# zacharie12/Hypernet-image-captioning

Hardware: AMD Instinct MI355X
Metric: training images/sec at 1/2/4/8 MI355X, Flickr30k GRU+hypernet bs=128 (higher is better)
Workload: dtype f32; 1 GPU; Flickr30k-shaped GRU+additive-attention decoder + hypernet (3 style domains), full training step (fwd, CE, bwd, clip 5.0, Adam); per_gpu_batch=128, global_batch=128, T=20, P=49, D=2048, F=200, E=200, H=200, V=9684, hypernet_params=144906720, parallelism=dp1, launch=eager, next_theta_in_adam_pass=True, next_precompute_beside_adam=True, spinup_steps=0, deterministic_gradients=True

## Files before the change

hypernet-image-captioning_amd/caphn/_lib.py:

```python
import ctypes as C
import os

import torch

_HERE = os.path.dirname(os.path.abspath(__file__))
LIB_PATH = os.environ.get("CAPHN_LIB_PATH") or os.path.join(_HERE, "libcaphn.so")
MAX_HEADS = 8

c_fp = C.c_void_p


class HyperDesc(C.Structure):
    _fields_ = [("he", C.c_int), ("n_heads", C.c_int),
                ("k", C.c_int * MAX_HEADS), ("w", C.c_int * MAX_HEADS),
                ("base_w0", c_fp), ("base_b0", c_fp), ("base_w2", c_fp), ("base_b2", c_fp),
                ("w1", c_fp * MAX_HEADS), ("b1", c_fp * MAX_HEADS),
                ("w2", c_fp * MAX_HEADS), ("b2", c_fp * MAX_HEADS),
                ("d_in", C.c_int), ("d_mid", C.c_int)]


class HyperGrads(C.Structure):
    _fields_ = [("g_base_w0", c_fp), ("g_base_b0", c_fp), ("g_base_w2", c_fp), ("g_base_b2", c_fp),
                ("g_w1", c_fp * MAX_HEADS), ("g_b1", c_fp * MAX_HEADS),
                ("g_w2", c_fp * MAX_HEADS), ("g_b2", c_fp * MAX_HEADS),
# ... 31 lines not shown


class PairPack(C.Structure):
    _fields_ = [("wp", c_fp), ("H", C.c_int), ("HA", C.c_int), ("pitch", C.c_int), ("hrows", C.c_int)]


MAX_LAYERS = 4


class PlainDims(C.Structure):
    _fields_ = [(n, C.c_int) for n in ("B", "T", "E", "H", "V", "L", "cell")]


class AttnDims(C.Structure):
    _fields_ = [(n, C.c_int) for n in ("bs", "nh", "dh", "tq", "tk", "q_ldt", "q_ldb", "k_ldt", "k_ldb", "v_ldt", "v_ldb",
                                       "o_ldt", "o_ldb")] + [("scale", C.c_float), ("dropout_p", C.c_float),
                                                             ("seed", C.c_uint64)]


class PlainParams(C.Structure):
    _fields_ = [("embed_w", c_fp), ("out_w", c_fp), ("out_b", c_fp),
                ("w_ih", c_fp * MAX_LAYERS), ("w_hh", c_fp * MAX_LAYERS), ("b_ih", c_fp * MAX_LAYERS), ("b_hh", c_fp * MAX_LAYERS)]


class PlainGrads(C.Structure):
    _fields_ = [("embed_w", c_fp), ("out_w", c_fp), ("out_b", c_fp),
                ("w_ih", c_fp * MAX_LAYERS), ("w_hh", c_fp * MAX_LAYERS), ("b_ih", c_fp * MAX_LAYERS), ("b_hh", c_fp * MAX_LAYERS),
                ("features", c_fp)]


class SearchCfg(C.Structure):
    _fields_ = [("n_images", C.c_int), ("beam", C.c_int), ("max_steps", C.c_int), ("zero_pad_rule", C.c_int),
                ("lookup_first", C.c_int), ("first_token", C.c_int64), ("end_token", C.c_int64)]


SIGNATURES = {
    "caphn_abi_version": (C.c_int, []),
    "caphn_device_arch": (C.c_int, [C.c_char_p, C.c_int]),
    "caphn_device_error": (C.c_int, [C.c_int]),
    "caphn_gemm_f32": (C.c_int, [C.c_int, C.c_int, C.c_int, C.c_int, C.c_int, c_fp, C.c_int, c_fp, C.c_int,
                                 c_fp, C.c_int, c_fp, c_fp, C.c_int, C.c_int, C.c_int, c_fp]),
    "caphn_split3_bf16": (C.c_int, [c_fp, C.c_int, C.c_int, C.c_int, c_fp, C.c_int, C.c_size_t, C.c_int, c_fp]),
    "caphn_gemm_planes_f32": (C.c_int, [C.c_int, C.c_int, C.c_int, C.c_int, C.c_int, c_fp, C.c_int, c_fp, C.c_int, C.c_size_t,
                                        c_fp, C.c_int, c_fp, C.c_int, C.c_size_t, c_fp, C.c_int, c_fp, c_fp, C.c_int, C.c_int,
                                        C.c_int, C.c_int, c_fp]),
    "caphn_zero_f32": (C.c_int, [c_fp, C.c_size_t, c_fp]),
    "caphn_lrelu_bwd_f32": (C.c_int, [C.c_size_t, c_fp, c_fp, c_fp, c_fp]),
    "caphn_axpy_f32": (C.c_int, [C.c_size_t, C.c_float, c_fp, c_fp, c_fp]),
    "caphn_scale_f32": (C.c_int, [C.c_size_t, c_fp, c_fp, c_fp, c_fp]),
    "caphn_add_dropout_f32": (C.c_int, [C.c_size_t, c_fp, c_fp, C.c_float, C.c_uint64, C.c_uint64, c_fp, c_fp]),
    "caphn_dropout_f32": (C.c_int, [C.c_size_t, C.c_float, C.c_uint64, C.c_uint64, c_fp, c_fp, c_fp]),
    "caphn_colsum_workspace_bytes": (C.c_size_t, [C.c_int, C.c_int]),
    "caphn_linear_wgrad_f32": (C.c_int, [C.c_int, C.c_int, C.c_int, c_fp, C.c_int, c_fp, C.c_int, c_fp, C.c_int, c_fp, c_fp, c_fp]),
    "caphn_colsum_f32": (C.c_int, [C.c_int, C.c_int, c_fp, C.c_int, c_fp, c_fp, c_fp]),
    "caphn_hyper_acts_floats": (C.c_int, [C.POINTER(HyperDesc)]),
    "caphn_hyper_forward": (C.c_int, [C.POINTER(HyperDesc), c_fp, c_fp, c_fp, c_fp]),
    "caphn_hyper_backward_workspace_bytes": (C.c_size_t, [C.POINTER(HyperDesc)]),
    "caphn_hyper_backward": (C.c_int, [C.POINTER(HyperDesc), c_fp, c_fp, C.POINTER(HyperGrads), c_fp, c_fp]),
    "caphn_decoder_workspace_bytes": (C.c_size_t, [C.POINTER(DecoderDims)]),
    "caphn_decoder_forward": (C.c_int, [C.POINTER(DecoderDims), C.POINTER(DecoderParams), c_fp, c_fp,
                                        c_fp, c_fp, c_fp, c_fp]),
    "caphn_decoder_pair_prep": (C.c_int, [C.POINTER(DecoderDims), C.POINTER(DecoderParams), c_fp, c_fp]),
    "caphn_decoder_pair_pack_desc": (C.c_int, [C.POINTER(DecoderDims), c_fp, C.POINTER(PairPack)]),
    "caphn_decoder_precompute": (C.c_int, [C.POINTER(DecoderDims), C.POINTER(DecoderParams), c_fp, c_fp, c_fp, c_fp]),
    "caphn_decoder_inputs": (C.c_int, [C.POINTER(DecoderDims), C.POINTER(DecoderParams), c_fp, c_fp, c_fp]),
    "caphn_decoder_lookup": (C.c_int, [C.POINTER(DecoderDims), C.POINTER(DecoderParams), c_fp, c_fp, c_fp]),
    "caphn_decoder_prepare_rows": (C.c_int, [C.POINTER(DecoderDims), c_fp, C.c_int64, c_fp, c_fp]),
    "caphn_decoder_forward_sampled": (C.c_int, [C.POINTER(DecoderDims), C.POINTER(DecoderParams), c_fp, c_fp,
                                                C.c_char_p, c_fp, c_fp, c_fp, c_fp]),
    "caphn_decoder_forward_sampled_train": (C.c_int, [C.POINTER(DecoderDims), C.POINTER(DecoderParams), c_fp, c_fp,
                                                      C.c_char_p, c_fp, c_fp, c_fp, c_fp]),
    "caphn_decoder_backward": (C.c_int, [C.POINTER(DecoderDims), C.POINTER(DecoderParams), c_fp, c_fp,
                                         c_fp, c_fp, C.POINTER(DecoderGrads), c_fp, c_fp]),
    "caphn_decoder_hyper_backward": (C.c_int, [C.POINTER(DecoderDims), C.POINTER(DecoderParams), c_fp, c_fp,
                                               c_fp, c_fp, C.POINTER(DecoderGrads), c_fp,
                                               C.POINTER(HyperDesc), c_fp, C.POINTER(HyperGrads), c_fp, c_fp]),
    "caphn_decoder_backward_milestone": (C.c_int, [C.c_int, c_fp]),
    "caphn_decoder_search_workspace_bytes": (C.c_size_t, [C.POINTER(DecoderDims), C.POINTER(SearchCfg)]),
    "caphn_decoder_search_begin": (C.c_int, [C.POINTER(DecoderDims), C.POINTER(DecoderParams), C.POINTER(SearchCfg),
                                             c_fp, c_fp, c_fp, c_fp]),
    "caphn_decoder_search_steps": (C.c_int, [C.POINTER(DecoderDims), C.POINTER(DecoderParams), C.POINTER(SearchCfg),
                                             C.c_int, C.c_int, c_fp, c_fp, c_fp, c_fp]),
    "caphn_decoder_search_result": (C.c_int, [C.POINTER(DecoderDims), C.POINTER(SearchCfg), C.c_int, c_fp, c_fp,
                                              c_fp, c_fp, c_fp, c_fp, c_fp, c_fp]),
    "caphn_plain_workspace_bytes": (C.c_size_t, [C.POINTER(PlainDims)]),
    "caphn_plain_forward": (C.c_int, [C.POINTER(PlainDims), C.POINTER(PlainParams), c_fp, c_fp, c_fp, c_fp, c_fp, c_fp, c_fp]),
    "caphn_bahdanau_fwd": (C.c_int, [C.c_int] * 4 + [c_fp] * 8),
    "caphn_bahdanau_bwd": (C.c_int, [C.c_int] * 4 + [c_fp] * 12),
    "caphn_plain_forward_sampled": (C.c_int, [C.POINTER(PlainDims), C.POINTER(PlainParams), c_fp, c_fp, c_fp, C.c_uint64, c_fp, c_fp,
                                               c_fp, c_fp]),
    "caphn_plain_backward": (C.c_int, [C.POINTER(PlainDims), C.POINTER(PlainParams), c_fp, c_fp, c_fp, c_fp, c_fp,
                                       C.POINTER(PlainGrads), c_fp, c_fp]),
    "caphn_layernorm_fwd": (C.c_int, [C.c_int, C.c_int, c_fp, c_fp, c_fp, C.c_float, c_fp, c_fp, c_fp, c_fp]),
    "caphn_layernorm_bwd_workspace_bytes": (C.c_size_t, [C.c_int, C.c_int]),
    "caphn_layernorm_bwd": (C.c_int, [C.c_int, C.c_int, c_fp, c_fp, c_fp, c_fp, c_fp, c_fp, c_fp, c_fp, c_fp, c_fp]),
    "caphn_attention_supported": (C.c_int, [C.POINTER(AttnDims)]),
    "caphn_attention_fwd": (C.c_int, [C.POINTER(AttnDims), c_fp, c_fp, c_fp, c_fp, c_fp, c_fp, c_fp, c_fp]),
    "caphn_attention_bwd": (C.c_int, [C.POINTER(AttnDims), c_fp, c_fp, c_fp, c_fp, c_fp, c_fp, c_fp, c_fp, c_fp, c_fp, c_fp, c_fp]),
    "caphn_ce_workspace_bytes": (C.c_size_t, [C.c_int]),
    "caphn_cross_entropy_rows": (C.c_int, [C.c_int, C.c_int, c_fp, c_fp, C.c_int64, c_fp, C.c_int, c_fp, c_fp, c_fp]),
    "caphn_cross_entropy_rows_ld": (C.c_int, [C.c_int, C.c_int, C.c_int, c_fp, c_fp, C.c_int64, c_fp, C.c_int, c_fp, c_fp, c_fp]),
    "caphn_cross_entropy_finish": (C.c_int, [C.c_int, c_fp, c_fp, c_fp, c_fp]),
    "caphn_decoder_profile_ptr": (C.c_void_p, [C.POINTER(DecoderDims), c_fp]),
    "caphn_decoder_rowcount_ptr": (C.c_void_p, [C.POINTER(DecoderDims), c_fp]),
    "caphn_cross_entropy_fwd_bwd": (C.c_int, [C.c_int, C.c_int, c_fp, c_fp, C.c_int64, c_fp, c_fp, C.c_int, c_fp, c_fp]),
    "caphn_embedding_gather": (C.c_int, [C.c_int, C.c_int, c_fp, c_fp, c_fp, c_fp]),
# ... 85 lines not shown
```

hypernet-image-captioning_amd/caphn/ops.py:

```python
import ctypes as C
from dataclasses import dataclass
from typing import Dict, List, Optional, Sequence, Tuple

import torch

from . import _lib as L

GEMM_BIAS, GEMM_RELU, GEMM_ACCUM, GEMM_MASK, GEMM_LRELU = 1, 2, 4, 8, 16


def _f32(*shape, device):
    return torch.empty(*shape, dtype=torch.float32, device=device)


def gemm(a: torch.Tensor, b: torch.Tensor, ta: bool = False, tb: bool = False,
         bias: Optional[torch.Tensor] = None, relu: bool = False, out: Optional[torch.Tensor] = None,
         accumulate: bool = False, mask: Optional[torch.Tensor] = None, splitk: int = 1, lrelu: bool = False) -> torch.Tensor:
    lib = L.load()
    assert a.dim() == 2 and b.dim() == 2 and a.stride(1) == 1 and b.stride(1) == 1
    M, K = (a.shape[1], a.shape[0]) if ta else (a.shape[0], a.shape[1])
    N, Kb = (b.shape[0], b.shape[1]) if tb else (b.shape[1], b.shape[0])
    if K != Kb:
        raise L.CaphnError(f"gemm inner dims differ: {K} vs {Kb}")
    if out is None:
# ... 48 lines not shown
            "caphn_gemm_planes_f32")
    return out


def zero_(t: torch.Tensor) -> torch.Tensor:
    lib = L.load()
    L.check(lib.caphn_zero_f32(L.ptr(t), t.numel(), L.stream_ptr()), "caphn_zero_f32")
    return t


def add_dropout(x: torch.Tensor, branch: torch.Tensor, p: float = 0.0, seed: int = 0) -> torch.Tensor:
    lib = L.load()
    x, branch = x.contiguous(), branch.contiguous()
    assert x.shape == branch.shape
    out = torch.empty_like(x)
    L.check(lib.caphn_add_dropout_f32(x.numel(), L.ptr(x), L.ptr(branch), float(p), int(seed) & (2 ** 64 - 1), 0, L.ptr(out),
                                      L.stream_ptr()), "caphn_add_dropout_f32")
    return out


def scale_(x: torch.Tensor, scale_dev: torch.Tensor) -> torch.Tensor:
    lib = L.load()
    L.check(lib.caphn_scale_f32(x.numel(), L.ptr(x), L.ptr(scale_dev.reshape(-1)[:1].contiguous()), L.ptr(x), L.stream_ptr()),
            "caphn_scale_f32")
    return x


def lrelu_bwd(dy: torch.Tensor, post: torch.Tensor, out: Optional[torch.Tensor] = None) -> torch.Tensor:
    lib = L.load()
    assert dy.numel() == post.numel() and dy.is_contiguous() and post.is_contiguous()
    if out is None:
        out = torch.empty_like(dy)
    L.check(lib.caphn_lrelu_bwd_f32(dy.numel(), L.ptr(dy), L.ptr(post), L.ptr(out), L.stream_ptr()), "caphn_lrelu_bwd_f32")
    return out


def axpy_(y: torch.Tensor, x: torch.Tensor, alpha: float = 1.0) -> torch.Tensor:
    lib = L.load()
    assert x.numel() == y.numel() and x.is_contiguous() and y.is_contiguous()
    L.check(lib.caphn_axpy_f32(y.numel(), float(alpha), L.ptr(x), L.ptr(y), L.stream_ptr()), "caphn_axpy_f32")
    return y


def linear_wgrad(dy: torch.Tensor, x: torch.Tensor):
    lib = L.load()
    K, M = dy.shape
    N = x.shape[1]
    assert x.shape[0] == K and dy.stride(1) == 1 and x.stride(1) == 1
    dw, db = _f32(M, N, device=dy.device), _f32(M, device=dy.device)
    ws = torch.empty(lib.caphn_colsum_workspace_bytes(K, M), dtype=torch.uint8, device=dy.device)
    L.check(lib.caphn_linear_wgrad_f32(M, N, K, L.ptr(dy), dy.stride(0), L.ptr(x), x.stride(0), L.ptr(dw), N, L.ptr(db),
                                       C.c_void_p(ws.data_ptr()), L.stream_ptr()), "caphn_linear_wgrad_f32")
    return dw, db


def bahdanau_fwd(f: torch.Tensor, waf: torch.Tensor, uah: torch.Tensor, v_a: torch.Tensor, b_va: torch.Tensor):
    lib = L.load()
    B, P, Fd = f.shape
    H = uah.shape[1]
    ctx, alpha = _f32(B, Fd, device=f.device), _f32(B, P, device=f.device)
    L.check(lib.caphn_bahdanau_fwd(B, P, Fd, H, L.ptr(f), L.ptr(waf), L.ptr(uah), L.ptr(v_a), L.ptr(b_va), L.ptr(ctx), L.ptr(alpha),
                                   L.stream_ptr()), "caphn_bahdanau_fwd")
    return ctx, alpha


def bahdanau_bwd(f, waf, uah, v_a, alpha, dctx, dalpha, want_df: bool):
    lib = L.load()
    B, P, Fd = f.shape
    H = uah.shape[1]
    dwaf, duah, part = _f32(B, P, H, device=f.device), _f32(B, H, device=f.device), _f32(B, H + 1, device=f.device)
    df = _f32(B, P, Fd, device=f.device) if want_df else None
    L.check(lib.caphn_bahdanau_bwd(B, P, Fd, H, L.ptr(f), L.ptr(waf), L.ptr(uah), L.ptr(v_a), L.ptr(alpha), L.ptr(dctx),
                                   L.ptr(dalpha, allow_none=True), L.ptr(dwaf), L.ptr(duah), L.ptr(part),
                                   L.ptr(df, allow_none=True), L.stream_ptr()), "caphn_bahdanau_bwd")
    return dwaf, duah, part, df


def colsum(a: torch.Tensor, out: Optional[torch.Tensor] = None) -> torch.Tensor:
    lib = L.load()
    M, N = a.shape
    ws = torch.empty(lib.caphn_colsum_workspace_bytes(M, N), dtype=torch.uint8, device=a.device)
    if out is None:
        out = _f32(N, device=a.device)
    L.check(lib.caphn_colsum_f32(M, N, L.ptr(a), a.stride(0), L.ptr(out), C.c_void_p(ws.data_ptr()), L.stream_ptr()),
            "caphn_colsum_f32")
    return out


HYPER_NAMES = ("hn_base.0.weight", "hn_base.0.bias", "hn_base.2.weight", "hn_base.2.bias")


@dataclass
class HyperShape:
    he: int
    heads: List[Tuple[int, int]]
    d_in: int = 0
    d_mid: int = 0

    @property
    def din(self) -> int:
        return self.d_in or self.he

    @property
    def dmid(self) -> int:
        return self.d_mid or self.he

# ... 883 lines not shown
```

hypernet-image-captioning_amd/csrc/decoder.hip:

```cpp
#include "common.h"
#include "decoder_internal.h"
#include "gemm_internal.h"
#include <algorithm>
#include <initializer_list>
#include <mutex>

int g_tune_deterministic = 0;
int g_tune_rec_pair = 1;
int g_tune_rec_rotate = 1;
int g_tune_vocab_order = 1;
int g_tune_branch_mask = 7;
int g_tune_splitk_target = 1280;
int g_tune_chain_main = 0;
int g_tune_hops = 0;
int g_tune_fork = 4;
int g_tune_join_chain = 0;
int g_tune_sk_dhs = 0, g_tune_sk_vocab_w = 0;
#define RUN(x) do { int _rc = (x); if (_rc != CAPHN_OK) return _rc; } while (0)

namespace {

struct Side {
    hipStream_t st[3];
    enum { D_FORK = 0, D_JOIN = 1, D_X = 4, D_MS = 10, D_PRE_F = 14, D_PRE_ALL = 15, D_COUNT = 16 };
    struct Dep { hipEvent_t ev; unsigned seq = 0; bool by_value = false; };
    Dep deps[D_COUNT];
    unsigned* vals = nullptr;
    unsigned counter = 0;
    bool values = false;
    bool pre_valid = false;
    const void* pre_ws = nullptr;
    bool ready = false, on = false;
    bool forked[3] = {false, false, false};
    hipStream_t main = nullptr;
    int init() {
        if (ready) return CAPHN_OK;
        static std::mutex mu;
        std::lock_guard<std::mutex> lock(mu);
        if (ready) return CAPHN_OK;
        for (auto& s : st) if (hipStreamCreateWithFlags(&s, hipStreamNonBlocking) != hipSuccess) return CAPHN_ELAUNCH;
        for (auto& d : deps) if (hipEventCreateWithFlags(&d.ev, hipEventDisableTiming) != hipSuccess) return CAPHN_ELAUNCH;
        void* p = nullptr;
        if (hipMalloc(&p, sizeof(unsigned) * D_COUNT) == hipSuccess && hipMemset(p, 0, sizeof(unsigned) * D_COUNT) == hipSuccess)
            vals = static_cast<unsigned*>(p);
        else (void)hipGetLastError();
        ready = true;
        return CAPHN_OK;
    }
    int post(int slot, hipStream_t from) {
        Dep& d = deps[slot];
        if (values) {
            d.seq = ++counter; d.by_value = true;
            return hipStreamWriteValue32(from, vals + slot, d.seq, 0) == hipSuccess ? CAPHN_OK : CAPHN_ELAUNCH;
        }
        d.by_value = false;
        return hipEventRecord(d.ev, from) == hipSuccess ? CAPHN_OK : CAPHN_ELAUNCH;
    }
    int await(int slot, hipStream_t to) {
        Dep& d = deps[slot];
        if (d.by_value)
            return hipStreamWaitValue32(to, vals + slot, d.seq, hipStreamWaitValueGte, 0xffffffffu) == hipSuccess ? CAPHN_OK : CAPHN_ELAUNCH;
        return hipStreamWaitEvent(to, d.ev, 0) == hipSuccess ? CAPHN_OK : CAPHN_ELAUNCH;
    }
    int milestone(int k, hipStream_t from) {
        if (init() != CAPHN_OK) return CAPHN_ELAUNCH;
        return post(D_MS + k, from);
    }
    int begin(hipStream_t m, bool enable) {
        main = m; on = enable;
// ... 14 lines not shown
        if (!on) return CAPHN_OK;
        if (post(D_FORK, main) != CAPHN_OK) return CAPHN_ELAUNCH;
        for (int i : ids) {
            if (!((g_tune_branch_mask >> i) & 1)) continue;
            if (await(D_FORK, st[i]) != CAPHN_OK) return CAPHN_ELAUNCH;
            forked[i] = true;
        }
        return CAPHN_OK;
    }
    int jointo(int i) {
        if (!on || !((g_tune_branch_mask >> i) & 1)) return CAPHN_OK;
        forked[i] = false;
        if (post(D_JOIN + i, st[i]) != CAPHN_OK) return CAPHN_ELAUNCH;
        return await(D_JOIN + i, main);
    }
    int join_into(int i, int j) {
        if (!on || !((g_tune_branch_mask >> i) & 1)) return CAPHN_OK;
        if (!((g_tune_branch_mask >> j) & 1)) return jointo(i);
        forked[i] = false;
        if (post(D_JOIN + i, st[i]) != CAPHN_OK) return CAPHN_ELAUNCH;
        return await(D_JOIN + i, st[j]);
    }
    struct Scope {
        Side& s;
        explicit Scope(Side& side) : s(side) {}
        ~Scope() { for (int i = 0; i < 3; ++i) if (s.on && s.forked[i]) (void)s.jointo(i); }
    };
    hipStream_t xfrom[6] = {nullptr, nullptr, nullptr, nullptr, nullptr, nullptr};
    int record(int k, hipStream_t from) {
        if (!on) return CAPHN_OK;
        xfrom[k] = from;
        return post(D_X + k, from);
    }
    int wait(int k, hipStream_t to) {
        if (!on || xfrom[k] == to) return CAPHN_OK;
        return await(D_X + k, to);
    }
    int dep(hipStream_t from, hipStream_t to, int k) {
        if (!on || from == to) return CAPHN_OK;
        if (post(D_X + k, from) != CAPHN_OK) return CAPHN_ELAUNCH;
        return await(D_X + k, to);
    }
};
constexpr int MAX_DEVICES = 64;
Side g_sides[MAX_DEVICES];
inline Side* side_here() {
    int dev = 0;
    if (hipGetDevice(&dev) != hipSuccess || dev < 0 || dev >= MAX_DEVICES) return nullptr;
    return &g_sides[dev];
}

struct Ws {
    size_t Y1, f, meanf, h0, c0, Waf, G, Xe, Xg, Hs, Hprev, gates, hn, Cs, Cprev, uah, alphas, idx;
    size_t dHs, dgi, dgh, duah, de, dh0, dc0, ctx, dctx, dXe, dWaf, dmeanf, df, dY1, apart, vtmp, colws, colws_s[3], prof, rowmap;
    size_t xch, xch_floats;
    size_t wp;
    size_t H0s, dH0, h0L, dcarry, tgi, tgh, tmpA, tmpB;
    size_t Lin[CAPHN_MAX_DEC_LAYERS - 1], Lgates[CAPHN_MAX_DEC_LAYERS - 1], Lhn[CAPHN_MAX_DEC_LAYERS - 1],
           Ldgi[CAPHN_MAX_DEC_LAYERS - 1], Ldgh[CAPHN_MAX_DEC_LAYERS - 1];
    int L1;
    size_t total;
    int npc, pchunk, NG, arows;
};
inline bool use_pair(const caphn_decoder_dims* d) {
    const int NG = d->cell == CAPHN_CELL_LSTM ? 4 : 3;
    return g_tune_rec_pair && d->T > 1 && d->layers <= 1 && caphn_rec_pair_resident_gates(d->P, d->H, NG) >= 0;
}

inline size_t up4(size_t v) { return (v + 3) & ~(size_t)3; }

inline Ws layout(const caphn_decoder_dims* d) {
    Ws w;
    const size_t B = d->B, T = d->T, P = d->P, F = d->F, E = d->E, H = d->H, V = d->V, D = d->D;
    const bool lstm = d->cell == CAPHN_CELL_LSTM, raw = d->raw_features != 0;
    const size_t NG = lstm ? 4 : 3;
    w.NG = (int)NG;
    size_t o = 0;
    auto take = [&](size_t n) { size_t r = o; o += up4(n); return r; };
    w.Y1 = take(raw ? 0 : B * P * F); w.f = take(raw ? 0 : B * P * F); w.meanf = take(B * F); w.h0 = take(B * H);
    w.c0 = take(lstm ? B * H : 0);
    w.Waf = take(B * P * H); w.G = take(B * P * NG * H); w.Xe = take(B * T * (E + F)); w.Xg = take(B * T * NG * H);
    w.Hs = take(B * T * H); w.Hprev = take(B * T * H); w.gates = take(B * T * NG * H); w.hn = take(lstm ? 0 : B * T * H);
    w.Cs = take(lstm ? B * T * H : 0); w.Cprev = take(lstm ? B * T * H : 0);
    w.uah = take(B * T * H); w.alphas = take(B * T * P); w.idx = take(2 * B * T);
    w.dHs = take(B * T * H); w.dgi = take(B * T * NG * H); w.dgh = take(lstm ? 0 : B * T * NG * H); w.duah = take(B * T * H);
    w.de = take(B * T * P); w.dh0 = take(B * H); w.dc0 = take(lstm ? B * H : 0);
    w.ctx = w.Xe + E; w.dctx = take(raw ? 0 : B * T * F);
    w.dXe = take(B * T * E); w.dWaf = take(B * P * H); w.dmeanf = take(raw ? 0 : 2 * B * F); w.df = take(raw ? 0 : B * P * F);
    w.dY1 = take(raw ? 0 : B * P * F);
    w.pchunk = 1; w.npc = (int)((P + w.pchunk - 1) / w.pchunk);
    const size_t arows = std::max<size_t>(std::max<size_t>(w.npc, (size_t)caphn_rec_bwd_groups((int)P, (int)H)),
                                          (size_t)caphn_rec_pair_bwd_groups((int)P, (int)H));
    w.arows = (int)arows;
    w.apart = take(B * arows * (H + 1)); w.vtmp = take(H + 1);
    size_t cs = 0;
    auto need = [&](size_t M, size_t N) { cs = std::max(cs, caphn_colsum_workspace_bytes((int)M, (int)N) / sizeof(float)); };
    need(B * T, V); need(B * T, NG * H); need(B * T, H); need(B * P, H); need(B * P, F); need(B, H);
    need(B * arows, H + 1);
    if (d->layers > 1) need(B * (T + 1), 3 * H);
    w.colws = take(cs);
    {
        size_t c2 = 0;
        auto need2 = [&](size_t M, size_t N) { c2 = std::max(c2, caphn_colsum_workspace_bytes((int)M, (int)N) / sizeof(float)); };
        need2(B * T, NG * H); need2(B * T, H); need2(B * P, H); need2(B * P, F); need2(B, H); need2(B * arows, H + 1);
        if (d->layers > 1) need2(B * (T + 1), 3 * H);
        for (int i = 0; i < 3; ++i) w.colws_s[i] = take(c2);
    }
    w.prof = take(64);
    w.rowmap = take(B * T + 4);
    w.xch_floats = caphn_rec_pair_xch_bytes((int)B, (int)P, (int)H) / sizeof(float);
    w.xch = take(2 * w.xch_floats);
    o = (o + 31) & ~(size_t)31;
    w.wp = take(caphn_rec_pair_wp_floats((int)H, (int)NG));
    w.L1 = d->layers > 1 ? d->layers - 1 : 0;
    {
        const size_t on = w.L1 > 0 ? 1 : 0, S = T + 1;
        w.H0s = take(on * B * T * H); w.dH0 = take(on * B * T * H); w.h0L = take(on * B * H); w.dcarry = take(on * B * H);
        w.tgi = take(on * B * 3 * H); w.tgh = take(on * B * 3 * H); w.tmpA = take(on * B * H); w.tmpB = take(on * B * H);
        for (int l = 0; l < CAPHN_MAX_DEC_LAYERS - 1; ++l) {
            const size_t u = l < w.L1 ? 1 : 0;
            w.Lin[l] = take(u * B * S * H); w.Lgates[l] = take(u * B * S * 3 * H); w.Lhn[l] = take(u * B * S * H);
            w.Ldgi[l] = take(u * B * S * 3 * H); w.Ldgh[l] = take(u * B * S * 3 * H);
        }
    }
    w.total = o;
    (void)D;
    return w;
}

__global__ __launch_bounds__(1024) void valid_rows_kernel(int n, const int64_t* __restrict__ tgt, int64_t ignore, int* __restrict__ map) {
    __shared__ int wsum[16];
    __shared__ int base_s;
    const int tid = threadIdx.x, lane = tid & 63, wave = tid >> 6;
    if (tid == 0) base_s = 0;
    __syncthreads();
    for (int c0 = 0; c0 < n; c0 += 1024) {
        const int i = c0 + tid;
        const int v = (i < n && tgt[i] != ignore) ? 1 : 0;
        const unsigned long long ball = __ballot(v);
        const int before = __popcll(ball & ((1ull << lane) - 1ull));
        if (lane == 0) wsum[wave] = __popcll(ball);
// ... 419 lines not shown
    if (!late && !wg_first) {
        if (!(d->precomputed & 32) && sd.s(0) != s && sd.s(2) != s) {
            RUN(sd.fork_many({0, 2}));
            RUN(caphn_launch_ctx(B, T, P, F, ws + w.alphas, f, ws + w.ctx, EF, sd.s(2)));
            RUN(sd.record(5, sd.s(2)));
            ctx_side = true;
        } else
        RUN(sd.forkto(0));
        RUN(wgrad_bias(V, H, BT, dlogits, LV, ws + w.Hs, H, g->out_w, H, g->out_b, rmap, cws, sd.s(0), gz));
        RUN(sd.milestone(CAPHN_MS_VOCAB, sd.s(0)));
    }

    RecBwdArgs a;
    a.B = B; a.T = T; a.P = P; a.H = H; a.RG = RG;
    a.Waf = ws + w.Waf; a.G = ws + w.G; a.W_hh = p->w_hh; a.U_a = p->Ua_w; a.v_a = p->va_w;
    a.Hprev = ws + w.Hprev; a.alphas = ws + w.alphas; a.gates = ws + w.gates; a.hn = ws + w.hn; a.uah = ws + w.uah;
    a.Cs = ws + w.Cs; a.Cprev = ws + w.Cprev;
    a.dHs = ws + w.dHs; a.dalphas = dalphas;
    a.dgi = dgi; a.dgh = dgh; a.duah = ws + w.duah; a.de = ws + w.de; a.dh0 = ws + w.dh0; a.dc0 = ws + w.dc0;
    a.vecW = (H % 4 == 0) && caphn_aligned16(p->w_hh) && caphn_aligned16(p->Ua_w);
    a.vecS = (H % 4 == 0) && caphn_aligned16(ws);
    a.prof = reinterpret_cast<unsigned long long*>(ws + w.prof) + 8;
    a.rotate = g_tune_rec_rotate;
    a.drop_p = d->dropout_p; a.drop_seed = d->dropout_seed;
    const int ang = w.L1 > 0 ? 0 : pair ? caphn_rec_pair_bwd_groups(P, H) : caphn_rec_bwd_groups(P, H);
    if (ang > 0) { a.dWaf = ws + w.dWaf; a.apart = ws + w.apart; }
    if (w.L1 > 0) {
        RUN(caphn_zero_f32(ws + w.dcarry, (size_t)B * H, s));
        a.dHs = ws + w.dH0; a.dh0 = ws + w.dcarry; a.drop_p = 0.f;
        for (int t = T - 1; t >= 0; --t) {
            RUN(layers_backward(d, p, w, ws, t + 1, ws + w.dHs + (size_t)t * H, T * H, ws + w.dcarry, ws + w.dH0 + (size_t)t * H, T * H, s));
            a.t0 = t; a.t1 = t + 1;
            RUN(caphn_launch_rec_bwd(a, lstm, s));
        }
        RUN(layers_backward(d, p, w, ws, 0, ws + w.dcarry, H, nullptr, ws + w.dh0, H, s));
    } else if (pair) {
        a.xch = reinterpret_cast<unsigned long long*>(ws + w.xch) + w.xch_floats * sizeof(float) / sizeof(unsigned long long);
        a.apart_rows = ang;
        a.WP = ws + w.wp; a.wp_pitch = caphn_rec_pair_pitch(H);
        if (!raw) { a.inith_w = p->inith_w; a.initc_w = lstm ? p->initc_w : nullptr; a.dmean_part = ws + w.dmeanf; a.F = F; }
        RUN(caphn_launch_rec_pair_bwd(a, lstm, s));
    } else
    RUN(caphn_launch_rec_bwd(a, lstm, s));

    hipStream_t b0 = sd.s(0), b1 = sd.s(1), b2 = sd.s(2);
    const bool t_main = hook != nullptr && g_tune_chain_main != 0;
    hipStream_t sT = t_main ? s : b1, sF = t_main ? b1 : s;
    const bool hold_big = late && !raw && fork_mode == 3;
    RUN(sd.fork_many({0, 1, 2}));
    if (late && !hold_big) {
        RUN(wgrad_bias(V, H, BT, dlogits, LV, ws + w.Hs, H, g->out_w, H, g->out_b, rmap, cws, b0, gz));
        RUN(sd.milestone(CAPHN_MS_VOCAB, b0));
    }
    if (ctx_side) RUN(sd.wait(5, sT));
    else if (!(d->precomputed & 32)) RUN(caphn_launch_ctx(B, T, P, F, ws + w.alphas, f, ws + w.ctx, EF, sT));
    if (lstm) RUN(gemm_auto(1, 0, GH, EF, BT, dgi, GH, ws + w.Xe, EF, g->w_ih, EF, nullptr, 0, sT, nullptr, 0, gz));
    else RUN(wgrad_bias(GH, EF, BT, dgi, GH, ws + w.Xe, EF, g->w_ih, EF, g->b_ih, nullptr, cw1, sT, gz));
    RUN(wgrad_bias(GH, H, BT, dgh, GH, ws + w.Hprev, H, g->w_hh, H, g->b_hh, nullptr, cw2, b2, gz));
    if (lstm) RUN(caphn_colsum_f32(BT, GH, dgi, GH, g->b_ih, cw2, b2));
    RUN(sd.record(3, b2));
    hipStream_t se = late ? b2 : b0;
    RUN(caphn_gemm_f32(0, 0, BT, E, GH, dgi, GH, p->w_ih, EF, ws + w.dXe, E, nullptr, nullptr, 0, 0, 1, se));
    if (!gz) RUN(caphn_zero_f32(g->embed_w, (size_t)V * E, se));
    RUN(caphn_embedding_scatter_add_v(BT, E, V, ws + w.dXe, idx, g->embed_w, se));
    RUN(sd.milestone(CAPHN_MS_EMBED, se));
    RUN(sd.wait(3, sT));
    RUN(sd.milestone(CAPHN_MS_DTHETA, sT));
    if (hook && !hold_big) {
        RUN(caphn_hyper_backward(hook->hd, g->w_ih, hook->acts, hook->hg, hook->ws, sT));
    }
    if (!hold_big) RUN(sd.milestone(CAPHN_MS_HYPER, sT));
    if (!raw) {
        RUN(caphn_gemm_f32(0, 0, BT, F, GH, dgi, GH, p->w_ih + E, EF, ws + w.dctx, F, nullptr, nullptr, 0, 0, 1, sF));
        if (!pair)
            RUN(caphn_launch_dmean(B, H, F, ws + w.dh0, p->inith_w, lstm ? ws + w.dc0 : nullptr, lstm ? p->initc_w : nullptr,
                                   ws + w.dmeanf, sF));
    }
    AttnGradArgs ag;
    ag.T = T; ag.P = P; ag.H = H; ag.pchunk = w.pchunk;
    ag.Waf = ws + w.Waf; ag.uah = ws + w.uah; ag.de = ws + w.de; ag.v_a = p->va_w;
    ag.dWaf = ws + w.dWaf; ag.part = ws + w.apart;
    if (ang == 0) RUN(caphn_launch_attn_param_grads(ag, B, w.npc, sF));
    RUN(sd.record(2, sF));
    RUN(wgrad_bias(H, H, BT, ws + w.duah, H, ws + w.Hprev, H, g->Ua_w, H, g->Ua_b, nullptr, cws, b0, gz));
    for (int l = 0; l < w.L1; ++l) {
        const int BS = B * (T + 1), G3 = 3 * H;
        RUN(wgrad_bias(G3, H, BS, ws + w.Ldgi[l], G3, ws + w.Lin[l], H, g->lw_ih[l], H, g->lb_ih[l], nullptr, cws, b0, gz));
        RUN(wgrad_bias(G3, H, BS, ws + w.Ldgh[l], G3, ws + w.Lin[l], H, g->lw_hh[l], H, g->lb_hh[l], nullptr, cws, b0, gz));
    }
    RUN(wgrad_bias(H, F, B, ws + w.dh0, H, ws + w.meanf, F, g->inith_w, F, g->inith_b, nullptr, cws, b0, gz));
    if (lstm) RUN(wgrad_bias(H, F, B, ws + w.dc0, H, ws + w.meanf, F, g->initc_w, F, g->initc_b, nullptr, cws, b0, gz));
    if (!raw) {
        RUN(caphn_launch_df(B, T, P, F, ws + w.alphas, ws + w.dctx, ws + w.dmeanf, ws + w.df, sF, pair ? ws + w.dmeanf + (size_t)B * F : nullptr));
        RUN(caphn_gemm_f32(0, 0, BP, F, H, ws + w.dWaf, H, p->Wa_w, F, ws + w.df, F, nullptr, nullptr, 0, CAPHN_GEMM_ACCUM, 1, sF));
        RUN(sd.record(4, sF));
        if (hold_big) {
            RUN(sd.wait(4, b0));
            RUN(wgrad_bias(V, H, BT, dlogits, LV, ws + w.Hs, H, g->out_w, H, g->out_b, rmap, cws, b0, gz));
            RUN(sd.milestone(CAPHN_MS_VOCAB, b0));
            if (hook) {
                RUN(sd.wait(4, sT));
                RUN(caphn_hyper_backward(hook->hd, g->w_ih, hook->acts, hook->hg, hook->ws, sT));
            }
            RUN(sd.milestone(CAPHN_MS_HYPER, sT));
        }
        RUN(caphn_gemm_f32(0, 0, BP, F, F, ws + w.df, F, p->fc2_w, F, ws + w.dY1, F, nullptr, ws + w.Y1, F, CAPHN_GEMM_MASK, 1, sF));
        RUN(wgrad_bias(F, D, BP, ws + w.dY1, F, features, D, g->fc0_w, D, g->fc0_b, nullptr, cw0, sF, gz));
    }
    RUN(sd.wait(2, b2));
    RUN(caphn_colsum_f32(B * (ang > 0 ? ang : w.npc), H + 1, ws + w.apart, H + 1, ws + w.vtmp, cw2, b2));
    hipLaunchKernelGGL(copy2_kernel, dim3((H + 256) / 256), dim3(256), 0, b2, ws + w.vtmp, H, g->va_w, g->va_b);
    RUN(wgrad_bias(H, F, BP, ws + w.dWaf, H, f, F, g->Wa_w, F, g->Wa_b, nullptr, cw2, b2, gz));
    if (!raw) {
        RUN(sd.wait(4, b2));
        RUN(wgrad_bias(F, F, BP, ws + w.df, F, ws + w.Y1, F, g->fc2_w, F, g->fc2_b, nullptr, cw2, b2, gz));
    }
    if (g_tune_join_chain) { RUN(sd.join_into(0, 1)); RUN(sd.join_into(2, 1)); RUN(sd.jointo(1)); }
    else { RUN(sd.jointo(0)); RUN(sd.jointo(1)); RUN(sd.jointo(2)); }
    (void)captions;
    return caphn_launch_status();
}

extern "C" int caphn_decoder_backward_milestone(int which, caphn_stream_t waiter) {
    if (which < 0 || which >= CAPHN_MS_COUNT) return CAPHN_EINVAL;
    Side* sd = side_here();
    if (!sd) return CAPHN_ELAUNCH;
    if (!sd->ready) return CAPHN_OK;
    return sd->await(Side::D_MS + which, static_cast<hipStream_t>(waiter));
}

extern "C" int caphn_decoder_forward_sampled(const caphn_decoder_dims* d, const caphn_decoder_params* p,
                                             const float* features, const int64_t* captions,
                                             const unsigned char* use_sampling,
                                             float* logits, float* alphas, void* ws_, caphn_stream_t stream) {
    if (!dims_ok(d) || !p || !features || !captions || !use_sampling || !logits || !ws_ || d->logits_ld != 0) return CAPHN_EINVAL;
    if (d->dropout_p > 0.f) return CAPHN_EINVAL;
    hipStream_t s = static_cast<hipStream_t>(stream);
    const Ws w = layout(d);
    float* ws = static_cast<float*>(ws_);
    const int B = d->B, T = d->T, P = d->P, E = d->E, F = d->F, H = d->H, V = d->V;
    const bool lstm = d->cell == CAPHN_CELL_LSTM;
    const int GH = w.NG * H, EF = E + F;
    const int RG = caphn_rec_resident_gates(P, H, w.NG);
    if (RG < 0) return CAPHN_ELIMIT;
    if (lstm && (!p->initc_w || !p->initc_b)) return CAPHN_EINVAL;
    const float* f = nullptr;
    if (!layer_params_ok(d, p)) return CAPHN_EINVAL;
    RUN(decoder_precompute(d, p, w, ws, features, &f, s));
    if (w.L1 > 0) RUN(layers_forward(d, p, w, ws, 0, ws + w.h0, H, ws + w.h0L, H, s));
    int64_t* idx = reinterpret_cast<int64_t*>(ws + w.idx);
    int src_mode = 0, src_col = 0;
    for (int t = 0; t < T; ++t) {
        const bool samp = t > 0 && use_sampling[t] != 0;
        if (!samp) {
            if (t < 2) { src_mode = 0; } else { src_mode = 1; src_col = t - 1; }
// ... 146 lines not shown
    const SearchArgs a = search_args(d, c, w, ws, static_cast<char*>(sws_));
    return caphn_launch_search_init(a, ws + (w.L1 > 0 ? w.h0L : w.h0), c->first_token, c->lookup_first, s);
}

extern "C" int caphn_decoder_search_steps(const caphn_decoder_dims* d, const caphn_decoder_params* p, const caphn_search_cfg* c,
                                          int step0, int nsteps, float* alphas, void* ws_, void* sws_, caphn_stream_t stream) {
    if (!search_ok(d, c) || !p || !ws_ || !sws_ || step0 < 1 || nsteps < 0 || step0 + nsteps - 1 > c->max_steps) return CAPHN_EINVAL;
    if (!layer_params_ok(d, p)) return CAPHN_EINVAL;
    if (alphas && c->beam != 1) return CAPHN_EINVAL;
    hipStream_t s = static_cast<hipStream_t>(stream);
    const Ws w = layout(d);
    float* ws = static_cast<float*>(ws_);
    char* sw = static_cast<char*>(sws_);
    const SearchWs q = search_layout(d, c);
    const SearchArgs sa = search_args(d, c, w, ws, sw);
    const int R = d->B, P = d->P, E = d->E, F = d->F, H = d->H, V = d->V, GH = w.NG * H, EF = E + F;
    const int RG = caphn_rec_resident_gates(P, H, w.NG);
    if (RG < 0) return CAPHN_ELIMIT;
    float* logits = reinterpret_cast<float*>(sw + q.logits);
    for (int step = step0; step < step0 + nsteps; ++step) {
        RUN(caphn_embedding_gather(R, E, p->embed_w, sa.idx, ws + w.Xe, s));
        RUN(caphn_gemm_f32(0, 1, R, GH, E, ws + w.Xe, E, p->w_ih, EF, ws + w.Xg, GH, p->b_ih, nullptr, 0, CAPHN_GEMM_BIAS, 1, s));
        RecFwdArgs a;
        a.B = R; a.T = 1; a.P = P; a.H = H; a.RG = RG; a.slab_div = c->beam;
        a.Waf = ws + w.Waf; a.G = ws + w.G; a.Xg = ws + w.Xg; a.h0 = sa.h_cur; a.c0 = nullptr;
        a.W_hh = p->w_hh; a.b_hh = p->b_hh; a.U_a = p->Ua_w; a.b_Ua = p->Ua_b; a.v_a = p->va_w; a.b_va = p->va_b;
        a.Hs = ws + w.Hs; a.Hprev = ws + w.Hprev; a.alphas = ws + w.alphas; a.gates = ws + w.gates; a.hn = ws + w.hn;
        a.Cs = nullptr; a.Cprev = nullptr; a.uah = ws + w.uah; a.prof = nullptr; a.rotate = 0;
        a.vecW = (H % 4 == 0) && caphn_aligned16(p->w_hh) && caphn_aligned16(p->Ua_w);
        a.vecS = (H % 4 == 0) && caphn_aligned16(ws);
        if (w.L1 > 0) a.Hs = ws + w.H0s;
        RUN(caphn_launch_rec_fwd(a, false, s));
        if (w.L1 > 0) RUN(layers_forward(d, p, w, ws, 1, ws + w.H0s, H, ws + w.Hs, H, s));
        RUN(caphn_gemm_f32(0, 1, R, V, H, ws + w.Hs, H, p->out_w, H, logits, V, p->out_b, nullptr, 0, CAPHN_GEMM_BIAS, 1, s));
        if (alphas)
            if (hipMemcpy2DAsync(alphas + (size_t)(step - 1) * P, sizeof(float) * (size_t)c->max_steps * P, ws + w.alphas,
                                 sizeof(float) * P, sizeof(float) * P, R, hipMemcpyDeviceToDevice, s) != hipSuccess) return CAPHN_ELAUNCH;
        RUN(caphn_launch_row_topk(R, V, c->beam, logits, sa.score, const_cast<float*>(sa.cand_val), const_cast<int*>(sa.cand_idx), s));
        RUN(caphn_launch_beam_merge(sa, step, s));
    }
    return caphn_launch_status();
}

extern "C" int caphn_decoder_search_result(const caphn_decoder_dims* d, const caphn_search_cfg* c, int steps_done, void* ws_, void* sws_,
                                           int64_t* seqs, int* lengths, float* scores, int* finished, int* n_active,
                                           caphn_stream_t stream) {
    if (!search_ok(d, c) || !ws_ || !sws_ || !seqs || !lengths || !scores || !finished || !n_active || steps_done < 0 ||
        steps_done > c->max_steps) return CAPHN_EINVAL;
    const Ws w = layout(d);
    const SearchArgs sa = search_args(d, c, w, static_cast<float*>(ws_), static_cast<char*>(sws_));
    return caphn_launch_search_result(sa, steps_done, seqs, lengths, scores, finished, n_active, static_cast<hipStream_t>(stream));
}

extern "C" int caphn_linear_wgrad_f32(int M, int N, int K, const float* dY, int ldy, const float* X, int ldx, float* dW, int ldw,
                                      float* db, void* ws, caphn_stream_t stream) {
    if (M <= 0 || N <= 0 || K <= 0 || !dY || !X || !dW || !db || !ws) return CAPHN_EINVAL;
    return caphn_gemm_tn_colsum(M, N, K, dY, ldy, X, ldx, dW, ldw, db, pick_splitk(M, N, K), nullptr, ws, false,
                                static_cast<hipStream_t>(stream));
}
```

hypernet-image-captioning_amd/csrc/decoder_internal.h:

```cpp
#pragma once
#include "common.h"

struct RecFwdArgs {
    int B, T, P, H;
    int RG;
    const float* Waf;
    const float* G;
    const float* Xg;
    const float* h0;
    const float* c0;
    const float* W_hh; const float* b_hh;
    const float* U_a; const float* b_Ua;
    const float* v_a; const float* b_va;
    float* Hs; float* Hprev;
    float* alphas;
    float* gates;
    float* hn;
    float* Cs; float* Cprev;
    float* uah;
    unsigned long long* prof;
    int vecW, vecS, rotate;
    int slab_div = 1;
    unsigned long long* xch = nullptr;
    const float* WP = nullptr; int wp_pitch = 0;
// ... 25 lines not shown
    const float* WP = nullptr; int wp_pitch = 0;
    int apart_rows = 0;
    float drop_p = 0.f; unsigned long long drop_seed = 0;
    unsigned epoch = 0; int* err = nullptr; long long xlimit = 0;
    const float* inith_w = nullptr; const float* initc_w = nullptr; float* dmean_part = nullptr; int F = 0;
    int part_rows = 0, wc_rows = 0;
    int t0 = 0, t1 = 0;
};
struct AttnGradArgs {
    int T, P, H, pchunk;
    const float* Waf; const float* uah; const float* de; const float* v_a;
    float* dWaf;
    float* part;
};

struct LayerFwdArgs {
    int B, H, S, slot;
    const float* gi; const float* gh;
    const float* hin; int hin_ld;
    float* hout; int hout_ld;
    float* sin; float* sgates; float* shn;
    float drop_p = 0.f; unsigned long long drop_seed = 0; int T = 1, t = 0;
};
struct LayerBwdArgs {
    int B, H, S, slot;
    const float* d1; int d1_ld; const float* d2;
    const float* sin; const float* sgates; const float* shn;
    float* dgi; float* dgh;
    float* dout; int dout_ld;
    float drop_p = 0.f; unsigned long long drop_seed = 0; int T = 1, t = 0;
};
int caphn_launch_layer_gru_fwd(const LayerFwdArgs& a, hipStream_t s);
int caphn_launch_layer_gru_bwd(const LayerBwdArgs& a, hipStream_t s);

size_t caphn_rec_fwd_lds_bytes(int P, int H, int NG, int RG);
size_t caphn_rec_bwd_lds_bytes(int P, int H, int NG, int RG);
int caphn_rec_resident_gates(int P, int H, int NG);
int caphn_launch_rec_fwd(const RecFwdArgs& a, bool lstm, hipStream_t s);
int caphn_launch_rec_bwd(const RecBwdArgs& a, bool lstm, hipStream_t s);
bool caphn_rec_pair_ok(int P, int H, int NG, int RG);
int caphn_rec_pair_resident_gates(int P, int H, int NG);
size_t caphn_rec_pair_xch_bytes(int B, int P, int H);
int caphn_rec_pair_bwd_groups(int P, int H);
int caphn_rec_pair_pitch(int H);
int caphn_rec_pair_half_a(int H);
size_t caphn_rec_pair_wp_floats(int H, int NG);
int caphn_launch_rec_pair_prep(unsigned long long* xch, size_t nxch, const float* U_a, const float* W_hh, int H, int NG, float* WP,
                               float* zbuf, size_t nz, hipStream_t s);
int caphn_launch_rec_pair_fwd(const RecFwdArgs& a, bool lstm, hipStream_t s);
int caphn_launch_rec_pair_bwd(const RecBwdArgs& a, bool lstm, hipStream_t s);
int caphn_rec_bwd_groups(int P, int H);
int caphn_launch_attn_param_grads(const AttnGradArgs& a, int B, int npc, hipStream_t s);
int caphn_launch_ctx(int B, int T, int P, int F, const float* alphas, const float* f, float* ctx, int ldc, hipStream_t s);
int caphn_launch_df(int B, int T, int P, int F, const float* alphas, const float* dctx, const float* dmean, float* df, hipStream_t s,
                    const float* dmean2 = nullptr);
int caphn_launch_dmean(int B, int H, int F, const float* dh0, const float* Wh, const float* dc0, const float* Wc, float* out, hipStream_t s);
int caphn_launch_init_state(int B, int P, int F, int H, const float* f, const float* Wh, const float* bh, const float* Wc,
                            const float* bc, float* meanf, float* h0, float* c0, hipStream_t s);
int caphn_embedding_gather_strided(int rows, int E, const float* table, const int64_t* idx, int istride, float* out, int ostride, hipStream_t s);
int caphn_launch_mean_p(int B, int P, int F, const float* f, float* out, hipStream_t s);

constexpr int SEARCH_MAX_BEAM = 8;
struct SearchArgs {
    int n_images, beam, max_steps, H;
    int zero_pad_rule;
    int64_t end_token;
    float* h_cur; const float* h_new;
    float* score;
    int64_t* idx;
    const float* cand_val; const int* cand_idx;
    int* k_alive; int* n_comp;
    int64_t* seqs[2];
    int64_t* comp_seqs; int* comp_len; float* comp_score;
};
int caphn_launch_row_topk(int R, int V, int k, const float* logits, const float* score, float* cand_val, int* cand_idx, hipStream_t s);
int caphn_launch_beam_merge(const SearchArgs& a, int step, hipStream_t s);
int caphn_launch_search_init(const SearchArgs& a, const float* h0, int64_t first_token, int lookup_first, hipStream_t s);
int caphn_launch_search_result(const SearchArgs& a, int steps_done, int64_t* out_seq, int* out_len, float* out_score, int* finished,
                               int* n_active, hipStream_t s);
```

hypernet-image-captioning_amd/csrc/gemm_bf16x3.hip:

```cpp
#include "common.h"
#include "gemm_internal.h"
#include "split3.h"
#include <type_traits>

#ifdef CAPHN_GEMM_PROFILE
__device__ unsigned long long d_gemm_prof[10];
__device__ unsigned long long d_gemm_wgt[2 * 8192];
extern "C" int caphn_debug_gemm_wgtimes(unsigned long long* out, int n) {
    return hipMemcpyFromSymbol(out, HIP_SYMBOL(d_gemm_wgt), sizeof(unsigned long long) * 2 * (n < 8192 ? n : 8192)) == hipSuccess ? 0 : -1;
}
#define GSTAMP(i) do { if (gprof) { unsigned long long _n = clock64(); gpc[i] += _n - glast; glast = _n; } } while (0)
extern "C" int caphn_debug_gemm_prof(unsigned long long* out, int reset) {
    if (out && hipMemcpyFromSymbol(out, HIP_SYMBOL(d_gemm_prof), sizeof(unsigned long long) * 10) != hipSuccess) return -1;
    if (reset) { unsigned long long z[10] = {0, 0, 0, 0, 0, 0, 0, 0, 0, 0}; if (hipMemcpyToSymbol(HIP_SYMBOL(d_gemm_prof), z, sizeof(z)) != hipSuccess) return -1; }
    return 0;
}
#else
#define GSTAMP(i) do { } while (0)
#endif

extern int g_tune_gemm_waves;
namespace {

constexpr int BK = 32;
constexpr int PITCH = 32;
__device__ __forceinline__ int kc_off(int row, int k) { return row * PITCH + ((((k >> 3) ^ (row >> 2)) & 3) << 3) + (k & 7); }

template <int BMN, bool KC>
struct TileS {
    static constexpr int NV = BMN / 32;
    static constexpr int PITCHM = BMN + 32;
    static constexpr int PLANE = KC ? BMN * PITCH : BK * PITCHM;
    static constexpr int ELEMS = 3 * PLANE;

    __device__ static __forceinline__ void phys_rows(int (&pr)[NV], int rows, int r0, int tid, const int* __restrict__ rmap,
                                                     bool clamp) {
#pragma unroll
        for (int i = 0; i < NV; ++i) {
            int row = r0 + ((tid + 256 * i) >> 3);
            if (clamp) row = min(row, rows - 1);
            pr[i] = (rmap && row < rows) ? rmap[row] : row;
        }
    }
    __device__ static __forceinline__ void load(f32x4 (&r)[NV], const float* __restrict__ G, int ld,
                                                int rows, int K, int r0, int k0, int vec, int tid,
                                                const int (&pr)[NV], const int* __restrict__ kmap) {
#pragma unroll
        for (int i = 0; i < NV; ++i) {
            f32x4 v = {0.f, 0.f, 0.f, 0.f};
            const int idx = tid + 256 * i;
            if (KC) {
                const int row = r0 + (idx >> 3);
                const int k = k0 + (idx & 7) * 4;
                if (row < rows) {
                    const float* p = G + (size_t)pr[i] * ld + k;
// ... 159 lines not shown
    __device__ static __forceinline__ bf16x8 frag(const __bf16* __restrict__ S, int plane, int row0, int ks, int lane) {
        if (KC) {
            return *reinterpret_cast<const bf16x8*>(S + plane * PLANE + kc_off(row0 + (lane & 31), ks * 16 + (lane >> 5) * 8));
        } else {
            const int g = lane >> 4, i = lane & 15;
            const int col = row0 + 16 * (g & 1) + 4 * (i & 3);
            const int kb = 16 * ks + 8 * (g >> 1) + (i >> 2);
            typedef __attribute__((address_space(3))) bf16x4 lds_bf16x4;
            const __bf16* p = S + plane * PLANE + kb * PITCHM + col;
            const bf16x4 lo4 = __builtin_amdgcn_ds_read_tr16_b64_v4bf16((lds_bf16x4*)(p));
            const bf16x4 hi4 = __builtin_amdgcn_ds_read_tr16_b64_v4bf16((lds_bf16x4*)(p + 4 * PITCHM));
            return __builtin_shufflevector(lo4, hi4, 0, 1, 2, 3, 4, 5, 6, 7);
        }
    }
};

__device__ __forceinline__ float bf16_bits_to_f32(unsigned short b) { return __uint_as_float((unsigned)b << 16); }

template <int BM, int BN, bool TA, bool TB, int MODE>
__device__ __forceinline__ void gemm_bf16x3_body(GemmArgs g) {
    constexpr bool PL = MODE == 1;
    constexpr bool SINGLE = MODE == 2;
    constexpr bool WS = MODE == 5;
    constexpr bool DB = MODE == 3 || WS;
    constexpr bool TWO = MODE == 4;
    using TileA = TileS<BM, !TA>;
    using TileB = TileS<BN, TB>;
    constexpr int WM = BM / 2, WN = BN / 2, TM = WM / 32, TN = WN / 32;
    constexpr int TILE_ELEMS = TileA::ELEMS + TileB::ELEMS;
    extern __shared__ __attribute__((aligned(16))) __bf16 lds[];
    __bf16* As = lds;
    __bf16* Bs = lds + TileA::ELEMS;
    __bf16* As1 = DB ? lds + TILE_ELEMS : As;
    __bf16* Bs1 = DB ? lds + TILE_ELEMS + TileA::ELEMS : Bs;

    const bool producer = WS && threadIdx.x >= 256;
    const int tid = WS ? (threadIdx.x & 255) : threadIdx.x, lane = tid & 63, wave = tid >> 6;
    const int wm = wave >> 1, wn = wave & 1;
    const int li = lane & 31, kh = lane >> 5;
#ifdef CAPHN_GEMM_PROFILE
    const unsigned long long gstart = clock64();
    const unsigned gwg = blockIdx.x + gridDim.x * (blockIdx.y + gridDim.y * blockIdx.z);
    if (tid == 0 && gwg < 8192) d_gemm_wgt[2 * gwg] = wall_clock64();
#endif
    int bx = blockIdx.x, by = blockIdx.y, bz = blockIdx.z;
    if (g.flags & (1 << 20)) {
        const int nx = gridDim.x, ny = gridDim.y, nwg = nx * ny * (int)gridDim.z;
        const int orig = bx + nx * (by + ny * bz);
        const int xcd = orig & 7, q = nwg >> 3, r = nwg & 7;
        const int wgid = (xcd < r ? xcd * (q + 1) : r * (q + 1) + (xcd - r) * q) + (orig >> 3);
        if (g.flags & (1 << 22)) { by = wgid % ny; bx = (wgid / ny) % nx; }
        else { bx = wgid % nx; by = (wgid / nx) % ny; }
        bz = wgid / (nx * ny);
    }
    const int m0 = by * BM, n0 = bx * BN;
    const int* rmapA = nullptr; const int* kmap = nullptr;
    if (g.map_mode == 1) { g.M = min(g.M, g.dev_count[0]); rmapA = g.row_map; if (m0 >= g.M) return; }
    if (g.map_mode == 2) { g.K = min(g.K, g.dev_count[0]); kmap = g.row_map; }

    const int nslab_total = (g.K + BK - 1) / BK;
    int slab0 = 0, slab1 = nslab_total;
    if (g.splitk > 1) {
        const int sps = g.map_mode == 2 ? (nslab_total + g.splitk - 1) / g.splitk : g.slabs_per_split;
        slab0 = bz * sps;
        slab1 = min(nslab_total, slab0 + sps);
        if (slab0 >= slab1) return;
    }

    constexpr bool DUAL = TM * TN == 1;
    f32x16 acc[TM][TN], acc2[DUAL ? TM : 1][DUAL ? TN : 1];
#pragma unroll
    for (int a = 0; a < TM; ++a)
#pragma unroll
        for (int b = 0; b < TN; ++b)
#pragma unroll
            for (int r = 0; r < 16; ++r) { acc[a][b][r] = 0.f; if (DUAL) acc2[a][b][r] = 0.f; }

    f32x4 ra0[TileA::NV], rb0[TileB::NV], ra1[TileA::NV], rb1[TileB::NV];
    int pra[TileA::NV], prb[TileB::NV];
    const int* kl = nullptr;
    const int kbase = slab0 * BK;
    bool fast = !(g.flags & (1 << 21)) && g.vecA && g.vecB && g.M >= 4 && g.N >= 4 && g.K >= 4 && (g.K & 3) == 0 &&
                (!TA || (g.M & 3) == 0) && (TB || (g.N & 3) == 0);
    if (kmap) {
        const int need = (slab1 - slab0) * BK;
        if (fast && TA && !TB && g.kmap_lds >= need) {
            int* kls = reinterpret_cast<int*>(lds + (DB ? 2 : 1) * TILE_ELEMS);
            for (int i = tid; i < need; i += 256) kls[i] = kmap[min(kbase + i, g.K - 1)];
            __syncthreads();
            kl = kls;
        } else fast = false;
    }
    TileA::phys_rows(pra, g.M, m0, tid, rmapA, fast);
    TileB::phys_rows(prb, g.N, n0, tid, nullptr, fast);
    unsigned boa[TileA::NV], bob[TileB::NV];
    if (fast) { TileA::fast_bases(boa, g.lda, g.M, m0, tid, pra); TileB::fast_bases(bob, g.ldb, g.N, n0, tid, prb); }
    else {
#pragma unroll
        for (int i = 0; i < TileA::NV; ++i) boa[i] = 0;
#pragma unroll
        for (int i = 0; i < TileB::NV; ++i) bob[i] = 0;
    }
    auto gload = [&](f32x4 (&ra)[TileA::NV], f32x4 (&rb)[TileB::NV], int slab, auto fast_c) {
        if constexpr (decltype(fast_c)::value) {
            TileA::load_fast_b(ra, g.A, boa, g.lda, g.K, slab * BK, tid, kl, kbase);
            TileB::load_fast_b(rb, g.B, bob, g.ldb, g.K, slab * BK, tid, kl, kbase);
// ... 330 lines not shown
        for (int b = 0; b < TN; ++b) {
            const int col = n0 + wn * WN + b * 32 + li;
            if (col >= g.N) continue;
            const float bv = add_bias ? g.bias[col] : 0.f;
#pragma unroll
            for (int r = 0; r < 16; ++r) {
                const int row = m0 + wm * WM + a * 32 + (r & 3) + 8 * (r >> 2) + 4 * kh;
                if (row >= g.M) continue;
                float v = acc[a][b][r] + bv;
                float* c = g.C + (size_t)(rmapA ? rmapA[row] : row) * g.ldc + col;
                if (atomic) { atomicAdd(c, v); continue; }
                if (g.flags & CAPHN_GEMM_ACCUM) v += *c;
                if (g.flags & CAPHN_GEMM_RELU) v = fmaxf(v, 0.f);
                if (g.flags & CAPHN_GEMM_LRELU) v = v > 0.f ? v : 0.01f * v;
                if (g.flags & CAPHN_GEMM_MASK) v = (g.mask[(size_t)row * g.ldmask + col] > 0.f) ? v : 0.f;
                *c = v;
            }
        }
#ifdef CAPHN_GEMM_PROFILE
    if (tid == 0) {
        __builtin_amdgcn_s_waitcnt(0);
        if (gwg < 8192) d_gemm_wgt[2 * gwg + 1] = wall_clock64();
        if (gwg == 0) atomicAdd(&d_gemm_prof[8], clock64() - gstart);
    }
#endif
}

template <int BM, int BN, bool TA, bool TB, int MODE>
__global__ __launch_bounds__(256) void gemm_bf16x3_kernel(GemmArgs g) { gemm_bf16x3_body<BM, BN, TA, TB, MODE>(g); }
template <int BM, int BN, bool TA, bool TB, int MODE>
__global__ __launch_bounds__(256) __attribute__((amdgpu_waves_per_eu(5, 5))) void gemm_bf16x3_kernel_w5(GemmArgs g) { gemm_bf16x3_body<BM, BN, TA, TB, MODE>(g); }
template <int BM, int BN, bool TA, bool TB, int MODE>
__global__ __launch_bounds__(256) __attribute__((amdgpu_waves_per_eu(6, 6))) void gemm_bf16x3_kernel_w6(GemmArgs g) { gemm_bf16x3_body<BM, BN, TA, TB, MODE>(g); }

template <int BM, int BN, bool TA, bool TB>
__global__ __launch_bounds__(512) void gemm_bf16x3_kernel_ws(GemmArgs g) { gemm_bf16x3_body<BM, BN, TA, TB, 5>(g); }

template <int BM, int BN, bool TA, bool TB, int PL>
int launch_one(const GemmArgs& g, hipStream_t s) {
    using TileA = TileS<BM, !TA>;
    using TileB = TileS<BN, TB>;
    constexpr size_t lds_tiles = sizeof(__bf16) * (TileA::ELEMS + TileB::ELEMS) * ((PL == 3 || PL == 5) ? 2 : 1);
    size_t lds = lds_tiles;
    if (g.kmap_lds > 0) lds += sizeof(int) * (size_t)g.kmap_lds;
    static bool attr_set[64];
    int dev = 0;
    if (hipGetDevice(&dev) != hipSuccess || dev < 0 || dev >= 64) return CAPHN_ELAUNCH;
    if (lds_tiles + 16384 > 48 * 1024 && !attr_set[dev]) {
        const void* fn = PL == 5 ? reinterpret_cast<const void*>(gemm_bf16x3_kernel_ws<BM, BN, TA, TB>)
                                 : reinterpret_cast<const void*>(gemm_bf16x3_kernel<BM, BN, TA, TB, PL == 5 ? 0 : PL>);
        if (hipFuncSetAttribute(fn, hipFuncAttributeMaxDynamicSharedMemorySize, (int)(lds_tiles + 16384)) != hipSuccess) return CAPHN_ELAUNCH;
        attr_set[dev] = true;
    }
    dim3 grid((g.N + BN - 1) / BN, (g.M + BM - 1) / BM, g.splitk > 1 ? g.splitk : 1);
    if constexpr (PL == 5) {
        hipLaunchKernelGGL((gemm_bf16x3_kernel_ws<BM, BN, TA, TB>), grid, dim3(512), lds, s, g);
        return caphn_launch_status();
    } else {
    if constexpr (BM == 64 && PL == 0) {
        if (g_tune_gemm_waves == 5) { hipLaunchKernelGGL((gemm_bf16x3_kernel_w5<BM, BN, TA, TB, PL>), grid, dim3(256), lds, s, g); return caphn_launch_status(); }
        if (g_tune_gemm_waves == 6) { hipLaunchKernelGGL((gemm_bf16x3_kernel_w6<BM, BN, TA, TB, PL>), grid, dim3(256), lds, s, g); return caphn_launch_status(); }
    }
    hipLaunchKernelGGL((gemm_bf16x3_kernel<BM, BN, TA, TB, PL>), grid, dim3(256), lds, s, g);
    return caphn_launch_status();
    }
}
template <int BM, int BN, int PL>
int launch_cfg(const GemmArgs& g, int ta, int tb, hipStream_t s) {
    if (!ta && tb) return launch_one<BM, BN, false, true, PL>(g, s);
    if (!ta && !tb) return launch_one<BM, BN, false, false, PL>(g, s);
    if (ta && !tb) return launch_one<BM, BN, true, false, PL>(g, s);
    if constexpr (PL != 0) return CAPHN_EINVAL;
    else return launch_one<BM, BN, true, true, 0>(g, s);
}

}

extern int g_tune_gemm_planes;
int g_tune_gemm_tile = 0;
int g_tune_gemm_single = 0;
int g_tune_gemm_order = 1;
int g_tune_gemm_xcd = 1;
int g_tune_gemm_waves = 0;
int g_tune_gemm_ws = 0;
int g_tune_gemm_db = 0;
int g_tune_gemm_fast = 1;
bool caphn_gemm_planes_ok(const GemmArgs& g, int ta, int tb) {
    bool pl = g_tune_gemm_planes && g.Ap && g.Bp && !(ta && tb) && (g.K % 8) == 0 && g.K >= 8 && (g.ldap % 8) == 0 && (g.ldbp % 8) == 0 &&
              (g.psa % 8) == 0 && (g.psb % 8) == 0 && caphn_aligned16(g.Ap) && caphn_aligned16(g.Bp);
    if (pl && ta && (((g.M + 7) & ~7) > g.ldap || g.M < 8)) pl = false;
    if (pl && !tb && (((g.N + 7) & ~7) > g.ldbp || g.N < 8)) pl = false;
    if (pl && g.map_mode == 2) {
        const int nslab = (g.K + 31) / 32, sk = g.splitk > 1 ? g.splitk : 1;
        if (!(ta && !tb) || ((nslab + sk - 1) / sk) * 32 > 4096) pl = false;
    }
    return pl;
}
template <int BM, int BN, bool TA, bool TB>
static int occ_one() {
    using TileA = TileS<BM, !TA>;
    using TileB = TileS<BN, TB>;
    int n = 0;
    if (hipOccupancyMaxActiveBlocksPerMultiprocessor(&n, reinterpret_cast<const void*>(gemm_bf16x3_kernel<BM, BN, TA, TB, 0>), 256,
                                                     sizeof(__bf16) * (TileA::ELEMS + TileB::ELEMS)) != hipSuccess) return -1;
    return n;
}
extern "C" int caphn_debug_gemm_occupancy(int ta, int tb, int tile) {
    if (tile == 128) return !ta && tb ? occ_one<128, 128, false, true>() : !ta ? occ_one<128, 128, false, false>() : !tb ? occ_one<128, 128, true, false>() : occ_one<128, 128, true, true>();
    return !ta && tb ? occ_one<64, 64, false, true>() : !ta ? occ_one<64, 64, false, false>() : !tb ? occ_one<64, 64, true, false>() : occ_one<64, 64, true, true>();
}
int caphn_gemm_bf16x3_launch(GemmArgs g, int ta, int tb, hipStream_t s) {
    if (g_tune_gemm_xcd) g.flags |= 1 << 20;
    g.kmap_lds = 0;
    if (g.map_mode == 2 && ta && !tb) {
        const int nslab = (g.K + 31) / 32, sk = g.splitk > 1 ? g.splitk : 1;
        const int ints = ((nslab + sk - 1) / sk) * 32;
        if (ints <= 4096) g.kmap_lds = ints;
    }
    if (!g_tune_gemm_fast) g.flags |= 1 << 21;
    {
        const double ea = ta ? (double)g.K * g.lda : (double)g.M * g.lda, eb = tb ? (double)g.N * g.ldb : (double)g.K * g.ldb;
        if (ea * 4.0 >= 4.0e9 || eb * 4.0 >= 4.0e9) g.flags |= 1 << 21;
    }
    if (g_tune_gemm_order != 0 && g.splitk <= 1) {
        const double abytes = 4.0 * (double)g.M * g.K, bbytes = 4.0 * (double)g.N * g.K, l2 = 3.0 * 1024 * 1024;
        if (g_tune_gemm_order == 2 || (bbytes > l2 && abytes < bbytes)) g.flags |= 1 << 22;
    }
    long tiles128 = (long)((g.M + 127) / 128) * ((g.N + 127) / 128) * g.splitk;
    if (g.K < 512) tiles128 = 0;
    if (g_tune_gemm_tile == 64) tiles128 = 0; else if (g_tune_gemm_tile == 128) tiles128 = 1 << 20;
    const bool pl = caphn_gemm_planes_ok(g, ta, tb);
    if (!pl && g_tune_gemm_single == 0 && g_tune_gemm_tile == 0 && g_tune_gemm_ws == 0) {
        const int rc = caphn_gemm_kres_launch(g, ta, tb, s);
        if (rc != 1) return rc;
    }
    if (pl) {
        if (tiles128 >= 512) return launch_cfg<128, 128, 1>(g, ta, tb, s);
        return launch_cfg<64, 64, 1>(g, ta, tb, s);
    }
    if (g_tune_gemm_single == 1 && !(ta && tb)) {
        if (tiles128 >= 512) return launch_cfg<128, 128, 2>(g, ta, tb, s);
        return launch_cfg<64, 64, 2>(g, ta, tb, s);
    }
    if (g_tune_gemm_single == 2 && !(ta && tb)) {
        if (tiles128 >= 512) return launch_cfg<128, 128, 4>(g, ta, tb, s);
        return launch_cfg<64, 64, 4>(g, ta, tb, s);
    }
    if (g_tune_gemm_ws == 128 && !(ta && tb)) return launch_cfg<128, 128, 5>(g, ta, tb, s);
    if (g_tune_gemm_ws == 64 && !(ta && tb)) return launch_cfg<64, 64, 5>(g, ta, tb, s);
    if (tiles128 >= 512) return launch_cfg<128, 128, 0>(g, ta, tb, s);
    const int lay = (!ta && tb) ? 1 : (!ta && !tb) ? 2 : (ta && !tb) ? 4 : 0;
    if (g_tune_gemm_db & lay) return launch_cfg<64, 64, 3>(g, ta, tb, s);
    return launch_cfg<64, 64, 0>(g, ta, tb, s);
}

namespace {
struct SplitJobs { SplitJob j[8]; int n; long block0[9]; };
__global__ __launch_bounds__(256) void split3_kernel(SplitJobs jobs) {
    int ji = 0;
    for (int i = 1; i < jobs.n; ++i) if ((long)blockIdx.x >= jobs.block0[i]) ji = i;
    const SplitJob& J = jobs.j[ji];
    const int cpr = (J.cols + 7) >> 3;
    const long nchunk = (long)(J.rows + J.zero_rows) * cpr;
    const long stride = (jobs.block0[ji + 1] - jobs.block0[ji]) * 256;
    __bf16* dst = static_cast<__bf16*>(J.dst);
    const bool vec = (J.ld & 3) == 0 && caphn_aligned16_dev(J.src);
    for (long c = ((long)blockIdx.x - jobs.block0[ji]) * 256 + threadIdx.x; c < nchunk; c += stride) {
        const int row = (int)(c / cpr), col = (int)(c % cpr) * 8;
        const float* sp = J.src + (size_t)row * J.ld + col;
        f32x4 v0 = {0.f, 0.f, 0.f, 0.f}, v1 = {0.f, 0.f, 0.f, 0.f};
        if (row >= J.rows) { }
        else if (vec && col + 8 <= J.cols) { v0 = *reinterpret_cast<const f32x4*>(sp); v1 = *reinterpret_cast<const f32x4*>(sp + 4); }
        else {
#pragma unroll
            for (int e = 0; e < 4; ++e) { if (col + e < J.cols) v0[e] = sp[e]; if (col + 4 + e < J.cols) v1[e] = sp[4 + e]; }
        }
        const Split4 a = split3(v0), b = split3(v1);
        __bf16* dp = dst + (size_t)row * J.ldp + col;
        *reinterpret_cast<bf16x8*>(dp) = __builtin_shufflevector(a.hi, b.hi, 0, 1, 2, 3, 4, 5, 6, 7);
        *reinterpret_cast<bf16x8*>(dp + J.ps) = __builtin_shufflevector(a.mid, b.mid, 0, 1, 2, 3, 4, 5, 6, 7);
        *reinterpret_cast<bf16x8*>(dp + 2 * J.ps) = __builtin_shufflevector(a.lo, b.lo, 0, 1, 2, 3, 4, 5, 6, 7);
    }
}
// ... 22 lines not shown
```

hypernet-image-captioning_amd/csrc/gemm_f32.hip:

```cpp
#include "common.h"
#include "gemm_internal.h"

int g_tune_gemm = 1;

namespace {

template <int BMN, bool KC, int BK>
struct Tile {
    static constexpr int KPAD = BK + 4;
    static constexpr int K4 = BK / 4;
    static constexpr int TOTAL = BMN * K4;
    static constexpr int NV = (TOTAL + 255) / 256;
    static constexpr int LDM = BMN + 4;
    static constexpr int FLOATS = KC ? BMN * KPAD : BK * LDM;

    __device__ static __forceinline__ void load(f32x4 (&r)[NV], const float* __restrict__ G, int ld,
                                                int rows, int K, int r0, int k0, int vec, int tid) {
#pragma unroll
        for (int i = 0; i < NV; ++i) {
            f32x4 v = {0.f, 0.f, 0.f, 0.f};
            const int idx = tid + 256 * i;
            if (TOTAL % 256 != 0 && idx >= TOTAL) { r[i] = v; continue; }
            if (KC) {
                int row = r0 + idx / K4;
                int k = k0 + (idx % K4) * 4;
                if (row < rows) {
                    const float* p = G + (size_t)row * ld + k;
                    if (vec && k + 3 < K) v = *reinterpret_cast<const f32x4*>(p);
                    else {
#pragma unroll
                        for (int e = 0; e < 4; ++e) if (k + e < K) v[e] = p[e];
                    }
                }
            } else {
                int m = r0 + (idx % (BMN / 4)) * 4;
                int k = k0 + idx / (BMN / 4);
                if (k < K) {
                    const float* p = G + (size_t)k * ld + m;
                    if (vec && m + 3 < rows) v = *reinterpret_cast<const f32x4*>(p);
                    else {
#pragma unroll
                        for (int e = 0; e < 4; ++e) if (m + e < rows) v[e] = p[e];
                    }
                }
            }
            r[i] = v;
        }
    }
    __device__ static __forceinline__ void store(const f32x4 (&r)[NV], float* __restrict__ S, int tid) {
#pragma unroll
        for (int i = 0; i < NV; ++i) {
            const int idx = tid + 256 * i;
            if (TOTAL % 256 != 0 && idx >= TOTAL) continue;
            if (KC) *reinterpret_cast<f32x4*>(S + (idx / K4) * KPAD + (idx % K4) * 4) = r[i];
            else *reinterpret_cast<f32x4*>(S + (idx / (BMN / 4)) * LDM + (idx % (BMN / 4)) * 4) = r[i];
        }
    }
    __device__ static __forceinline__ f32x4 frag(const float* __restrict__ S, int row, int kq, int kh) {
        if (KC) return *reinterpret_cast<const f32x4*>(S + row * KPAD + kq * 8 + kh * 4);
        f32x4 v;
#pragma unroll
        for (int s = 0; s < 4; ++s) v[s] = S[(kq * 8 + kh * 4 + s) * LDM + row];
        return v;
    }
};

template <int BM, int BN, bool TA, bool TB, int BK>
__global__ __launch_bounds__(256) void gemm_f32_kernel(GemmArgs g) {
    using TileA = Tile<BM, !TA, BK>;
    using TileB = Tile<BN, TB, BK>;
    constexpr int WM = BM / 2, WN = BN / 2, TM = WM / 32, TN = WN / 32;
    __shared__ __attribute__((aligned(16))) float lds[TileA::FLOATS + TileB::FLOATS];
    float* As = lds;
    float* Bs = lds + TileA::FLOATS;

    const int tid = threadIdx.x, lane = tid & 63, wave = tid >> 6;
    const int wm = wave >> 1, wn = wave & 1;
    const int li = lane & 31, kh = lane >> 5;
    const int m0 = blockIdx.y * BM, n0 = blockIdx.x * BN;

    const int nslab_total = (g.K + BK - 1) / BK;
    int slab0 = 0, slab1 = nslab_total;
    if (g.splitk > 1) {
        slab0 = blockIdx.z * g.slabs_per_split;
        slab1 = min(nslab_total, slab0 + g.slabs_per_split);
        if (slab0 >= slab1) return;
    }

    f32x16 acc[TM][TN];
#pragma unroll
    for (int a = 0; a < TM; ++a)
#pragma unroll
        for (int b = 0; b < TN; ++b)
#pragma unroll
            for (int r = 0; r < 16; ++r) acc[a][b][r] = 0.f;

    f32x4 ra[TileA::NV], rb[TileB::NV];
    TileA::load(ra, g.A, g.lda, g.M, g.K, m0, slab0 * BK, g.vecA, tid);
    TileB::load(rb, g.B, g.ldb, g.N, g.K, n0, slab0 * BK, g.vecB, tid);
    TileA::store(ra, As, tid);
    TileB::store(rb, Bs, tid);
    __syncthreads();

    for (int slab = slab0; slab < slab1; ++slab) {
        const bool more = slab + 1 < slab1;
        if (more) {
            TileA::load(ra, g.A, g.lda, g.M, g.K, m0, (slab + 1) * BK, g.vecA, tid);
            TileB::load(rb, g.B, g.ldb, g.N, g.K, n0, (slab + 1) * BK, g.vecB, tid);
        }
#pragma unroll
        for (int kq = 0; kq < BK / 8; ++kq) {
            f32x4 fa[TM], fb[TN];
#pragma unroll
            for (int a = 0; a < TM; ++a) fa[a] = TileA::frag(As, wm * WM + a * 32 + li, kq, kh);
#pragma unroll
            for (int b = 0; b < TN; ++b) fb[b] = TileB::frag(Bs, wn * WN + b * 32 + li, kq, kh);
#pragma unroll
            for (int s = 0; s < 4; ++s)
#pragma unroll
                for (int a = 0; a < TM; ++a)
#pragma unroll
                    for (int b = 0; b < TN; ++b)
                        acc[a][b] = __builtin_amdgcn_mfma_f32_32x32x2f32(fa[a][s], fb[b][s], acc[a][b], 0, 0, 0);
        }
        __syncthreads();
        if (more) {
            TileA::store(ra, As, tid);
            TileB::store(rb, Bs, tid);
            __syncthreads();
        }
    }

    const bool atomic = g.splitk > 1;
    const bool add_bias = (g.flags & CAPHN_GEMM_BIAS) && (!atomic || blockIdx.z == 0);
#pragma unroll
    for (int a = 0; a < TM; ++a)
#pragma unroll
        for (int b = 0; b < TN; ++b) {
            const int col = n0 + wn * WN + b * 32 + li;
            if (col >= g.N) continue;
            const float bv = add_bias ? g.bias[col] : 0.f;
#pragma unroll
            for (int r = 0; r < 16; ++r) {
                const int row = m0 + wm * WM + a * 32 + (r & 3) + 8 * (r >> 2) + 4 * kh;
                if (row >= g.M) continue;
                float v = acc[a][b][r] + bv;
                float* c = g.C + (size_t)row * g.ldc + col;
                if (atomic) { atomicAdd(c, v); continue; }
                if (g.flags & CAPHN_GEMM_ACCUM) v += *c;
                if (g.flags & CAPHN_GEMM_RELU) v = fmaxf(v, 0.f);
                if (g.flags & CAPHN_GEMM_LRELU) v = v > 0.f ? v : 0.01f * v;
                if (g.flags & CAPHN_GEMM_MASK) v = (g.mask[(size_t)row * g.ldmask + col] > 0.f) ? v : 0.f;
                *c = v;
            }
        }
}

template <int BM, int BN, int BK>
int launch_cfg(const GemmArgs& g, int ta, int tb, hipStream_t s) {
    dim3 grid((g.N + BN - 1) / BN, (g.M + BM - 1) / BM, g.splitk > 1 ? g.splitk : 1);
    dim3 block(256);
    if (!ta && tb) hipLaunchKernelGGL((gemm_f32_kernel<BM, BN, false, true, BK>), grid, block, 0, s, g);
    else if (!ta && !tb) hipLaunchKernelGGL((gemm_f32_kernel<BM, BN, false, false, BK>), grid, block, 0, s, g);
    else if (ta && !tb) hipLaunchKernelGGL((gemm_f32_kernel<BM, BN, true, false, BK>), grid, block, 0, s, g);
    else hipLaunchKernelGGL((gemm_f32_kernel<BM, BN, true, true, BK>), grid, block, 0, s, g);
    return caphn_launch_status();
}

}

int caphn_gemm_mapped(int ta, int tb, int M, int N, int K, const float* A, int lda, const float* B, int ldb,
                      float* C, int ldc, const float* bias, int flags, int splitk,
                      const int* row_map, const int* dev_count, int map_mode, hipStream_t s) {
    if (M <= 0 || N <= 0 || K <= 0 || !A || !B || !C || !row_map || !dev_count) return CAPHN_EINVAL;
    if ((flags & CAPHN_GEMM_BIAS) && !bias) return CAPHN_EINVAL;
    if (splitk > 1 && (flags & 0xFFFF & ~CAPHN_GEMM_BIAS)) return CAPHN_EINVAL;
    GemmArgs g;
    g.M = M; g.N = N; g.K = K; g.A = A; g.lda = lda; g.B = B; g.ldb = ldb; g.C = C; g.ldc = ldc;
    g.bias = bias; g.mask = nullptr; g.ldmask = 0; g.flags = flags;
    const int nslab = (K + 31) / 32;
    if (splitk > nslab) splitk = nslab;
    g.splitk = splitk > 1 ? splitk : 1;
    g.slabs_per_split = (nslab + g.splitk - 1) / g.splitk;
    g.vecA = caphn_aligned16(A) && (lda % 4 == 0);
    g.vecB = caphn_aligned16(B) && (ldb % 4 == 0);
    g.row_map = row_map; g.dev_count = dev_count; g.map_mode = map_mode; g.colsum_a = nullptr; g.kmap_lds = 0;
    g.Ap = nullptr; g.Bp = nullptr; g.ldap = g.ldbp = 0; g.psa = g.psb = 0;
    return caphn_gemm_bf16x3_launch(g, ta, tb, s);
}

int caphn_gemm_tn_colsum(int M, int N, int K, const float* A, int lda, const float* B, int ldb, float* C, int ldc,
                         float* colsum_out, int splitk, const int* rowmap, void* cws, bool prezeroed, hipStream_t s) {
    if (M <= 0 || N <= 0 || K <= 0 || !A || !B || !C || !colsum_out) return CAPHN_EINVAL;
    const int nslab = (K + 31) / 32;
    if (splitk > nslab) splitk = nslab;
    if (splitk < 1) splitk = 1;
    if ((splitk > 1 || rowmap) && !prezeroed) {
        if (ldc == N) { int rc = caphn_zero_f32(C, (size_t)M * N, s); if (rc) return rc; }
        else if (hipMemset2DAsync(C, sizeof(float) * ldc, 0, sizeof(float) * N, M, s) != hipSuccess) return CAPHN_ELAUNCH;
    }
    if (g_tune_gemm != 1 && !rowmap) {
        int rc = caphn_gemm_f32(1, 0, M, N, K, A, lda, B, ldb, C, ldc, nullptr, nullptr, 0, 0, splitk, s);
        if (rc) return rc;
        return caphn_colsum_f32(K, M, A, lda, colsum_out, cws, s);
    }
    if (!prezeroed) { int rc = caphn_zero_f32(colsum_out, (size_t)M, s); if (rc) return rc; }
    GemmArgs g;
    g.M = M; g.N = N; g.K = K; g.A = A; g.lda = lda; g.B = B; g.ldb = ldb; g.C = C; g.ldc = ldc;
    g.bias = nullptr; g.mask = nullptr; g.ldmask = 0; g.flags = 0;
    g.splitk = splitk; g.slabs_per_split = (nslab + splitk - 1) / splitk;
    g.vecA = caphn_aligned16(A) && (lda % 4 == 0);
    g.vecB = caphn_aligned16(B) && (ldb % 4 == 0);
    g.row_map = rowmap ? rowmap + 4 : nullptr; g.dev_count = rowmap; g.map_mode = rowmap ? 2 : 0;
    g.colsum_a = colsum_out; g.kmap_lds = 0;
    g.Ap = nullptr; g.Bp = nullptr; g.ldap = g.ldbp = 0; g.psa = g.psb = 0;
    return caphn_gemm_bf16x3_launch(g, 1, 0, s);
}

int caphn_gemm_x(int ta, int tb, int M, int N, int K, const Opnd& A, const Opnd& B, float* C, int ldc, const GemmX& x, hipStream_t s) {
    if (M <= 0 || N <= 0 || K <= 0 || !A.f || !B.f || !C) return CAPHN_EINVAL;
    if ((x.flags & CAPHN_GEMM_BIAS) && !x.bias) return CAPHN_EINVAL;
    if ((x.flags & CAPHN_GEMM_MASK) && !x.mask) return CAPHN_EINVAL;
    if (g_tune_gemm != 1) {
        if (x.rowmap || x.colsum) return CAPHN_EINVAL;
        return caphn_gemm_f32(ta, tb, M, N, K, A.f, A.ld, B.f, B.ld, C, ldc, x.bias, x.mask, x.ldmask, x.flags, x.splitk, s);
    }
    int splitk = x.splitk;
    if (splitk > 1 && (x.flags & 0xFFFF & ~CAPHN_GEMM_BIAS)) return CAPHN_EINVAL;
    GemmArgs g;
    g.M = M; g.N = N; g.K = K; g.A = A.f; g.lda = A.ld; g.B = B.f; g.ldb = B.ld; g.C = C; g.ldc = ldc;
    g.bias = x.bias; g.mask = x.mask; g.ldmask = x.ldmask; g.flags = x.flags;
    const int nslab = (K + 31) / 32;
    if (splitk > nslab) splitk = nslab;
    g.splitk = splitk > 1 ? splitk : 1;
    g.slabs_per_split = (nslab + g.splitk - 1) / g.splitk;
    g.vecA = caphn_aligned16(A.f) && (A.ld % 4 == 0);
    g.vecB = caphn_aligned16(B.f) && (B.ld % 4 == 0);
    g.row_map = x.rowmap ? x.rowmap + 4 : nullptr; g.dev_count = x.rowmap; g.map_mode = x.rowmap ? x.map_mode : 0;
    g.colsum_a = ta ? x.colsum : nullptr; g.kmap_lds = 0;
    const bool both = A.p && B.p;
    g.Ap = both ? A.p : nullptr; g.ldap = A.ldp; g.psa = A.ps;
    g.Bp = both ? B.p : nullptr; g.ldbp = B.ldp; g.psb = B.ps;
    if (both && x.Kp > K) {
        g.K = x.Kp;
        if (!caphn_gemm_planes_ok(g, ta, tb)) g.K = K;
        else {
            const int ns = (g.K + 31) / 32;
            g.slabs_per_split = (ns + g.splitk - 1) / g.splitk;
        }
    }
    if (g.K == K && (K % 8) != 0) { g.Ap = nullptr; g.Bp = nullptr; }
    return caphn_gemm_bf16x3_launch(g, ta, tb, s);
}

extern "C" int caphn_split3_bf16(const float* src, int rows, int cols, int ld, void* planes, int ldp, size_t plane_stride,
                                 int zero_rows, caphn_stream_t stream) {
    if (!src || !planes || rows <= 0 || cols <= 0 || ld < cols || zero_rows < 0) return CAPHN_EINVAL;
    SplitJob j{src, ld, planes, ldp, plane_stride, rows, cols, zero_rows};
    return caphn_split3_launch(&j, 1, static_cast<hipStream_t>(stream));
}
extern "C" int caphn_gemm_planes_f32(int ta, int tb, int M, int N, int K,
                                     const float* A, int lda, const void* Ap, int ldap, size_t psa,
                                     const float* B, int ldb, const void* Bp, int ldbp, size_t psb,
                                     float* C, int ldc, const float* bias, const float* mask, int ldmask, int flags, int splitk,
                                     int Kp, caphn_stream_t stream) {
    GemmX x;
    x.bias = bias; x.mask = mask; x.ldmask = ldmask; x.flags = flags; x.splitk = splitk; x.Kp = Kp;
    return caphn_gemm_x(ta, tb, M, N, K, Opnd(A, lda, Ap, ldap, psa), Opnd(B, ldb, Bp, ldbp, psb), C, ldc, x,
// ... 39 lines not shown
```

hypernet-image-captioning_amd/csrc/gemm_internal.h:

```cpp
#pragma once
#include "common.h"

struct GemmArgs {
    int M, N, K;
    const float* A; int lda;
    const float* B; int ldb;
    float* C; int ldc;
    const float* bias;
    const float* mask; int ldmask;
    int flags;
    int splitk, slabs_per_split;
    int vecA, vecB;
    const int* row_map; const int* dev_count; int map_mode;
    float* colsum_a;
    int kmap_lds;
    const void* Ap; int ldap; size_t psa;
    const void* Bp; int ldbp; size_t psb;
};

struct Opnd {
    const float* f; int ld;
    const void* p; int ldp; size_t ps;
    Opnd() : f(nullptr), ld(0), p(nullptr), ldp(0), ps(0) {}
    Opnd(const float* f_, int ld_) : f(f_), ld(ld_), p(nullptr), ldp(0), ps(0) {}
    Opnd(const float* f_, int ld_, const void* p_, int ldp_, size_t ps_) : f(f_), ld(ld_), p(p_), ldp(ldp_), ps(ps_) {}
    Opnd at(size_t rows, size_t cols) const {
        Opnd o = *this;
        o.f = f + rows * ld + cols;
        if (p) o.p = static_cast<const char*>(p) + 2 * (rows * ldp + cols);
        return o;
    }
};
struct GemmX {
    const float* bias = nullptr; const float* mask = nullptr; int ldmask = 0; int flags = 0; int splitk = 1;
    const int* rowmap = nullptr;
    int map_mode = 0;
    float* colsum = nullptr;
    int Kp = 0;
};
int caphn_gemm_x(int ta, int tb, int M, int N, int K, const Opnd& A, const Opnd& B, float* C, int ldc, const GemmX& x, hipStream_t s);

struct SplitJob { const float* src; int ld; void* dst; int ldp; size_t ps; int rows, cols; int zero_rows; };
int caphn_split3_launch(const SplitJob* jobs, int n, hipStream_t s);

int caphn_gemm_mapped(int ta, int tb, int M, int N, int K, const float* A, int lda, const float* B, int ldb,
                      float* C, int ldc, const float* bias, int flags, int splitk,
                      const int* row_map, const int* dev_count, int map_mode, hipStream_t s);

int caphn_gemm_tn_colsum(int M, int N, int K, const float* A, int lda, const float* B, int ldb, float* C, int ldc,
                         float* colsum_out, int splitk, const int* rowmap, void* cws, bool prezeroed, hipStream_t s);

bool caphn_gemm_planes_ok(const GemmArgs& g, int ta, int tb);
int caphn_gemm_bf16x3_launch(GemmArgs g, int ta, int tb, hipStream_t s);
int caphn_gemm_kres_launch(const GemmArgs& g, int ta, int tb, hipStream_t s);
extern int g_tune_gemm;
```

hypernet-image-captioning_amd/csrc/hyper.hip:

```cpp
#include "common.h"
#include <algorithm>

namespace {

constexpr float LRELU = 0.01f;
__device__ __forceinline__ float lrelu(float v) { return v > 0.f ? v : LRELU * v; }
__device__ __forceinline__ float lrelu_grad(float post) { return post > 0.f ? 1.f : LRELU; }

struct GemvJob {
    const float* W; const float* b; const float* x; float* y;
    int rows, k, act, vec;
    int block0, nblocks;
    float* xcopy;
};
struct GemvJobs { GemvJob j[CAPHN_MAX_HEADS]; int n; };

template <int QMAX, int RB, bool NTL>
__device__ __forceinline__ void gemv_rows_wave(const GemvJob& J, int wave_g, int nwaves, int lane) {
    const int k4 = J.k >> 2;
    const f32x4* x4 = reinterpret_cast<const f32x4*>(J.x);
    f32x4 xr[QMAX];
#pragma unroll
    for (int q = 0; q < QMAX; ++q) {
        int c = lane + 64 * q;
        xr[q] = c < k4 ? x4[c] : f32x4{0.f, 0.f, 0.f, 0.f};
    }
    const int myrow = RB == 8 ? ((lane >> 5) & 1) * 4 + ((lane >> 4) & 1) * 2 + ((lane >> 3) & 1) : lane;
    for (int r0 = wave_g * RB; r0 < J.rows; r0 += nwaves * RB) {
        f32x4 w[RB][QMAX];
#pragma unroll
        for (int i = 0; i < RB; ++i) {
            const f32x4* row = reinterpret_cast<const f32x4*>(J.W + (size_t)(r0 + i) * J.k);
#pragma unroll
            for (int q = 0; q < QMAX; ++q) {
                int c = lane + 64 * q;
                if (r0 + i < J.rows && c < k4) w[i][q] = NTL ? __builtin_nontemporal_load(row + c) : row[c];
                else w[i][q] = f32x4{0.f, 0.f, 0.f, 0.f};
            }
        }
        float v[RB];
#pragma unroll
        for (int i = 0; i < RB; ++i) {
            float s = 0.f;
#pragma unroll
            for (int q = 0; q < QMAX; ++q)
                s += w[i][q][0] * xr[q][0] + w[i][q][1] * xr[q][1] + w[i][q][2] * xr[q][2] + w[i][q][3] * xr[q][3];
            v[i] = s;
        }
        float mine = 0.f;
        if (RB == 8) {
#pragma unroll
            for (int st = 0; st < 3; ++st) {
                const int mask = 32 >> st, half = RB >> (st + 1);
// ... 132 lines not shown
            if (lane == 0) {
                const RowRef rr = locate(r);
                const float v = lrelu(t + rr.b[rr.r]);
                if (out_s) out_s[r] = v;
                if (rr.og) rr.og[rr.r] = v;
            }
        }
    }
}
template <int QMAX>
__global__ __launch_bounds__(1024) void hyper_acts_fused_kernel(ActsFusedArgs a) {
    extern __shared__ __attribute__((aligned(16))) float sm[];
    float* xs = sm;
    float* a0s = xs + ((a.d_in + 3) & ~3);
    float* bs = a0s + ((a.d_mid + 3) & ~3);
    const int tid = threadIdx.x, lane = tid & 63, wave = __builtin_amdgcn_readfirstlane(tid >> 6), wg = blockIdx.x;
    const bool w0g = wg == 0;
    for (int i = tid; i < a.d_in; i += 1024) {
        const float v = a.x[i];
        xs[i] = v;
        if (w0g && a.a_x != a.x) a.a_x[i] = v;
    }
    __syncthreads();
    fused_rows<QMAX>([&](int r) { return RowRef{a.w0, a.b0, w0g ? a.a_a0 : nullptr, r}; }, a.d_mid, a.d_in, xs, wave, 16, a0s, lane);
    __syncthreads();
    fused_rows<QMAX>([&](int r) { return RowRef{a.w2, a.b2, w0g ? a.a_base : nullptr, r}; }, a.he, a.d_mid, a0s, wave, 16, bs, lane);
    __syncthreads();
    fused_rows<QMAX>([&](int r) {
        int i = 0;
        while (i + 1 < a.nh && r >= a.k[i]) { r -= a.k[i]; ++i; }
        return RowRef{a.w1[i], a.b1[i], a.out[i], r};
    }, a.rtot, a.he, bs, wg * 16 + wave, (int)gridDim.x * 16, nullptr, lane);
}
}
int g_tune_gemv = 1;
namespace {
template <int QMAX>
static void launch_gemv_fwd_q(const GemvJobs& jobs, int nblocks, hipStream_t s) {
    if (g_tune_gemv == 0) hipLaunchKernelGGL((gemv_fwd_kernel<4, false, QMAX>), dim3(nblocks), dim3(256), 0, s, jobs);
    else hipLaunchKernelGGL((gemv_fwd_kernel<4, true, QMAX>), dim3(nblocks), dim3(256), 0, s, jobs);
}
static void launch_gemv_fwd(const GemvJobs& jobs, int nblocks, hipStream_t s) {
    int kmax = 0;
    for (int i = 0; i < jobs.n; ++i) if (jobs.j[i].vec && jobs.j[i].k <= 2048) kmax = std::max(kmax, jobs.j[i].k);
    if (kmax <= 256) launch_gemv_fwd_q<1>(jobs, nblocks, s);
    else if (kmax <= 512) launch_gemv_fwd_q<2>(jobs, nblocks, s);
    else if (kmax <= 1024) launch_gemv_fwd_q<4>(jobs, nblocks, s);
    else launch_gemv_fwd_q<8>(jobs, nblocks, s);
}

struct GemvTJob {
    const float* W; const float* d; float* partial;
    int rows, k, vec, block0, nblocks;
};
struct GemvTJobs { GemvTJob j[CAPHN_MAX_HEADS]; int n; unsigned* bar = nullptr; };

template <int QMAX>
__device__ __forceinline__ void gemv_t_wave(const GemvTJob& J, int lb, int tid, float* red ) {
    const int lane = tid & 63, wave = tid >> 6;
    const int k4 = J.k >> 2;
    f32x4 acc[QMAX];
#pragma unroll
    for (int q = 0; q < QMAX; ++q) acc[q] = f32x4{0.f, 0.f, 0.f, 0.f};
    constexpr int RB = 4;
    const int wave_g = lb * 4 + wave, nwaves = J.nblocks * 4;
    for (int r0 = wave_g * RB; r0 < J.rows; r0 += nwaves * RB) {
        f32x4 w[RB][QMAX];
        float dv[RB];
#pragma unroll
        for (int i = 0; i < RB; ++i) {
            const bool ok = r0 + i < J.rows;
            dv[i] = ok ? J.d[r0 + i] : 0.f;
            const f32x4* row = reinterpret_cast<const f32x4*>(J.W + (size_t)(r0 + i) * J.k);
#pragma unroll
            for (int q = 0; q < QMAX; ++q) {
                int c = lane + 64 * q;
                w[i][q] = (ok && c < k4) ? __builtin_nontemporal_load(row + c) : f32x4{0.f, 0.f, 0.f, 0.f};
            }
        }
#pragma unroll
        for (int i = 0; i < RB; ++i)
#pragma unroll
            for (int q = 0; q < QMAX; ++q) acc[q] += w[i][q] * dv[i];
    }
#pragma unroll
    for (int q = 0; q < QMAX; ++q) {
        int c = lane + 64 * q;
        if (c < k4) *reinterpret_cast<f32x4*>(red + wave * J.k + c * 4) = acc[q];
    }
    __syncthreads();
    for (int c = tid; c < J.k; c += 256)
        J.partial[(size_t)lb * J.k + c] = red[c] + red[J.k + c] + red[2 * J.k + c] + red[3 * J.k + c];
}

template <int QMAX>
__global__ __launch_bounds__(256) void gemv_t_partial_kernel(GemvTJobs jobs) {
    extern __shared__ __attribute__((aligned(16))) float red[];
    int ji = 0;
    for (int i = 1; i < jobs.n; ++i) if ((int)blockIdx.x >= jobs.j[i].block0) ji = i;
    const GemvTJob& J = jobs.j[ji];
    const int lb = blockIdx.x - J.block0, tid = threadIdx.x;
    if (jobs.bar && blockIdx.x == 0 && tid < 4) jobs.bar[tid] = 0u;
    if (J.vec && J.k <= 256 * QMAX) {
        gemv_t_wave<QMAX>(J, lb, tid, red);
    } else {
        const int per = (J.rows + J.nblocks - 1) / J.nblocks;
        const int ra = lb * per, rb = min(J.rows, ra + per);
        constexpr int CJ = 8;
        for (int c0 = tid; c0 < J.k; c0 += 256 * CJ) {
            float s[CJ];
#pragma unroll
            for (int j = 0; j < CJ; ++j) s[j] = 0.f;
            const bool full = c0 + 256 * (CJ - 1) < J.k;
            if (full) {
                for (int r = ra; r < rb; ++r) {
                    const float dr = J.d[r];
                    const float* row = J.W + (size_t)r * J.k + c0;
#pragma unroll
                    for (int j = 0; j < CJ; ++j) s[j] += row[256 * j] * dr;
                }
            } else {
                for (int r = ra; r < rb; ++r) {
                    const float dr = J.d[r];
                    const float* row = J.W + (size_t)r * J.k + c0;
#pragma unroll
                    for (int j = 0; j < CJ; ++j) if (c0 + 256 * j < J.k) s[j] += row[256 * j] * dr;
                }
            }
#pragma unroll
            for (int j = 0; j < CJ; ++j) if (c0 + 256 * j < J.k) J.partial[(size_t)lb * J.k + c0 + 256 * j] = s[j];
        }
    }
}

constexpr int RL = 16;
__device__ __forceinline__ float col_reduce_finish(float acc, float (*red)[65]) {
    const int c = threadIdx.x & 63, rl = threadIdx.x >> 6;
    red[rl][c] = acc;
    __syncthreads();
    float s = 0.f;
    if (rl == 0) {
#pragma unroll
        for (int i = 0; i < RL; ++i) s += red[i][c];
    }
    return s;
}

struct ReduceJob { const float* partial; const float* post; float* out0; float* out1; int k, nblocks; };
struct ReduceJobs { ReduceJob j[CAPHN_MAX_HEADS]; int n; };
__global__ __launch_bounds__(1024) void gemv_t_reduce_kernel(ReduceJobs jobs) {
    __shared__ float red[RL][65];
    const ReduceJob& J = jobs.j[blockIdx.y];
    const int c = blockIdx.x * 64 + (threadIdx.x & 63), rl = threadIdx.x >> 6;
    if (blockIdx.x * 64 >= J.k) return;
    float acc = 0.f;
    if (c < J.k)
        for (int b = rl; b < J.nblocks; b += RL) acc += J.partial[(size_t)b * J.k + c];
    float s = col_reduce_finish(acc, red);
    if (rl == 0 && c < J.k) {
        if (J.post) s *= lrelu_grad(J.post[c]);
        if (J.out0) J.out0[c] = s;
        if (J.out1) J.out1[c] = s;
    }
}

struct SmallTJob { const float* W; const float* d; int rows; };
struct SmallTArgs { SmallTJob j[CAPHN_MAX_HEADS]; int n; int k; const float* post; float* out0; float* out1; int acc0 = 0; };
constexpr int STC = 8, STR = 128;
__global__ __launch_bounds__(1024) void gemv_t_small_kernel(SmallTArgs a) {
    __shared__ float red[STR][STC + 1];
    const int cl = threadIdx.x & (STC - 1), rl = threadIdx.x / STC;
    const int c = blockIdx.x * STC + cl;
    float acc = 0.f;
    if (c < a.k)
        for (int i = 0; i < a.n; ++i) {
            const SmallTJob& J = a.j[i];
            for (int r = rl; r < J.rows; r += STR) acc += J.W[(size_t)r * a.k + c] * J.d[r];
        }
    red[rl][cl] = acc;
    __syncthreads();
    if (threadIdx.x < 64 * STC) {
        const int col = threadIdx.x >> 6, lane = threadIdx.x & 63;
        float s = wave_sum(red[lane][col] + red[lane + 64][col]);
        const int cc = blockIdx.x * STC + col;
        if (lane == 0 && cc < a.k) {
            if (a.post) s *= lrelu_grad(a.post[cc]);
            if (a.out0) { if (a.acc0) atomicAdd(a.out0 + cc, s); else a.out0[cc] = s; }
            if (a.out1) a.out1[cc] = s;
        }
    }
}

struct OuterJob { const float* g; const float* a; float* out; int rows, k; long block0; };
struct OuterJobs { OuterJob j[2 * CAPHN_MAX_HEADS]; int n; };
__global__ __launch_bounds__(256) void outer_kernel(OuterJobs jobs) {
    int ji = 0;
    for (int i = 1; i < jobs.n; ++i) if ((long)blockIdx.x >= jobs.j[i].block0) ji = i;
    const OuterJob& J = jobs.j[ji];
    const size_t n = (size_t)J.rows * J.k;
    size_t idx = ((size_t)blockIdx.x - J.block0) * 1024 + threadIdx.x;
#pragma unroll
    for (int i = 0; i < 4; ++i, idx += 256)
        if (idx < n) J.out[idx] = J.g[idx / J.k] * J.a[idx % J.k];
}


int g_tune_vjp_blocks = 512;
int g_tune_hyper_tail = 0;
struct TailHead { const float* partial; const float* post; const float* w1; float* g_b1; float* g_w1; int k, nblocks, dzo; };
struct TailArgs {
    TailHead h[CAPHN_MAX_HEADS]; int nh;
    int he, d_mid, d_in;
    const float* base_act;
    const float* a0_act;
    const float* x_in;
    const float* base_w2; const float* base_w0;
    float* g_base_b2; float* g_base_b0; float* g_base_w2; float* g_base_w0; float* g_x; int x_acc;
    float* dz; float* dzb2; float* dzb0;
    unsigned* bar;
    int* err; long long limit;
};
__device__ __forceinline__ float ld_x(const float* p) {
    return __uint_as_float(__hip_atomic_load(reinterpret_cast<const unsigned*>(p), __ATOMIC_RELAXED, __HIP_MEMORY_SCOPE_AGENT));
}
__device__ __forceinline__ void st_x(float* p, float v) {
    __hip_atomic_store(reinterpret_cast<unsigned*>(p), __float_as_uint(v), __ATOMIC_RELAXED, __HIP_MEMORY_SCOPE_AGENT);
}
__device__ __forceinline__ void tail_barrier(unsigned* cnt, unsigned target, int* err, long long limit) {
    asm volatile("s_waitcnt vmcnt(0)" ::: "memory");
    __syncthreads();
    if (threadIdx.x == 0) {
        __hip_atomic_fetch_add(cnt, 1u, __ATOMIC_RELAXED, __HIP_MEMORY_SCOPE_AGENT);
        const long long t0 = wall_clock64();
        for (int spin = 1; __hip_atomic_load(cnt, __ATOMIC_RELAXED, __HIP_MEMORY_SCOPE_AGENT) < target; ++spin) {
            __builtin_amdgcn_s_sleep(1);
            if ((spin & 255) == 0 && wall_clock64() - t0 > limit) {
                if (err) __hip_atomic_store(err, 1, __ATOMIC_RELAXED, __HIP_MEMORY_SCOPE_SYSTEM);
                break;
            }
        }
    }
    __syncthreads();
}
__device__ __forceinline__ void tail_stage(const float* src, int n, float* dst) {
    for (int i = threadIdx.x; i < n; i += 1024) dst[i] = ld_x(src + i);
    __syncthreads();
}
__device__ __forceinline__ void tail_smallt(const float* W, const float* ds, int rows, int k, const float* post, float* out_x, float* out_g,
                                            int acc_g, int unit, float (*red)[STC + 1]) {
    const int cl = threadIdx.x & (STC - 1), rl = threadIdx.x / STC;
    const int c = unit * STC + cl;
    float acc = 0.f;
    if (c < k) {
        int r = rl;
        for (; r + 3 * STR < rows; r += 4 * STR) {
            const float w0 = W[(size_t)r * k + c], w1 = W[(size_t)(r + STR) * k + c], w2 = W[(size_t)(r + 2 * STR) * k + c],
                        w3 = W[(size_t)(r + 3 * STR) * k + c];
            acc += w0 * ds[r]; acc += w1 * ds[r + STR]; acc += w2 * ds[r + 2 * STR]; acc += w3 * ds[r + 3 * STR];
        }
// ... 184 lines not shown
        GemvJob& J = jobs.j[0];
        J.W = W; J.b = b; J.x = in; J.y = out; J.rows = rows; J.k = k; J.act = act; J.xcopy = xcopy;
        J.vec = vec_ok(W, in, k); J.block0 = 0; J.nblocks = gemv_blocks(rows, k, J.vec);
        launch_gemv_fwd(jobs, J.nblocks, s);
    };
    bool fused = g_tune_acts_fused != 0;
    {
        const int widths[3] = {d_in(d), d_mid(d), d->he};
        for (int wdt : widths) fused = fused && wdt % 4 == 0 && wdt >= 128 && wdt <= 512;
        fused = fused && (long)d_mid(d) * d_in(d) + (long)d->he * d_mid(d) <= 262144 && caphn_aligned16(x) && caphn_aligned16(acts) &&
                caphn_aligned16(d->base_w0) && caphn_aligned16(d->base_w2);
        for (int i = 0; i < d->n_heads; ++i) fused = fused && caphn_aligned16(d->w1[i]);
    }
    if (fused) {
        ActsFusedArgs a;
        a.x = x; a.d_in = d_in(d); a.d_mid = d_mid(d); a.he = d->he; a.nh = d->n_heads; a.rtot = 0;
        a.w0 = d->base_w0; a.b0 = d->base_b0; a.w2 = d->base_w2; a.b2 = d->base_b2;
        for (int i = 0; i < d->n_heads; ++i) { a.w1[i] = d->w1[i]; a.b1[i] = d->b1[i]; a.out[i] = acts + L.a[i]; a.k[i] = d->k[i]; a.rtot += d->k[i]; }
        a.a_x = acts + L.x; a.a_a0 = acts + L.a0; a.a_base = acts + L.base;
        const int nb = std::max(1, std::min(64, (a.rtot + 15) / 16));
        const size_t shm = sizeof(float) * (size_t)(((a.d_in + 3) & ~3) + ((a.d_mid + 3) & ~3) + ((a.he + 3) & ~3));
        const int wmax = std::max(a.d_in, std::max(a.d_mid, a.he));
        if (wmax <= 256) hipLaunchKernelGGL(hyper_acts_fused_kernel<1>, dim3(nb), dim3(1024), shm, s, a);
        else hipLaunchKernelGGL(hyper_acts_fused_kernel<2>, dim3(nb), dim3(1024), shm, s, a);
    } else {
    one(d->base_w0, d->base_b0, x, acts + L.a0, d_mid(d), d_in(d), 1, x == acts + L.x ? nullptr : acts + L.x);
    one(d->base_w2, d->base_b2, acts + L.a0, acts + L.base, d->he, d_mid(d), 1, nullptr);
    {
        GemvJobs jobs; jobs.n = d->n_heads; int b0 = 0;
        for (int i = 0; i < d->n_heads; ++i) {
            GemvJob& J = jobs.j[i];
            J.W = d->w1[i]; J.b = d->b1[i]; J.x = acts + L.base; J.y = acts + L.a[i];
            J.rows = d->k[i]; J.k = d->he; J.act = 1; J.vec = vec_ok(J.W, J.x, J.k); J.xcopy = nullptr;
            J.block0 = b0; J.nblocks = gemv_blocks(J.rows, J.k, J.vec); b0 += J.nblocks;
        }
        launch_gemv_fwd(jobs, b0, s);
    }
    }
    if (theta) {
        GemvJobs jobs; jobs.n = d->n_heads; int b0 = 0; size_t off = 0;
        for (int i = 0; i < d->n_heads; ++i) {
            GemvJob& J = jobs.j[i];
            J.W = d->w2[i]; J.b = d->b2[i]; J.x = acts + L.a[i]; J.y = theta + off; off += d->w[i];
            J.rows = d->w[i]; J.k = d->k[i]; J.act = 0; J.vec = vec_ok(J.W, J.x, J.k); J.xcopy = nullptr;
            J.block0 = b0; J.nblocks = gemv_blocks(J.rows, J.k, J.vec); b0 += J.nblocks;
        }
        launch_gemv_fwd(jobs, b0, s);
    }
    return caphn_launch_status();
}

namespace {
struct BwdWs { size_t partial[CAPHN_MAX_HEADS]; int nblocks[CAPHN_MAX_HEADS]; size_t dz[CAPHN_MAX_HEADS];
               size_t dzb2, dzb0, bar, total; };
constexpr int VJP_BLOCKS_MAX = 4096;
inline BwdWs bwd_ws(const caphn_hyper_desc* d) {
    BwdWs w; size_t o = 0;
    for (int i = 0; i < d->n_heads; ++i) {
        const long want = ((long)d->w[i] + 15) / 16;
        int nb = (int)std::min<long>(g_tune_vjp_blocks, want);
        if (nb < 1) nb = 1;
        w.nblocks[i] = nb;
        w.partial[i] = o; o += caphn_align_up((size_t)std::max<long>(1, std::min<long>(VJP_BLOCKS_MAX, want)) * d->k[i], 4);
    }
    for (int i = 0; i < d->n_heads; ++i) { w.dz[i] = o; o += caphn_align_up(d->k[i], 4); }
    w.dzb2 = o; o += caphn_align_up(d->he, 4);
    w.dzb0 = o; o += caphn_align_up(d_mid(d), 4);
    o = caphn_align_up(o, 32);
    w.bar = o; o += 32;
    w.total = o;
    return w;
}
}

extern "C" size_t caphn_hyper_backward_workspace_bytes(const caphn_hyper_desc* d) {
    if (!d || d->n_heads <= 0 || d->n_heads > CAPHN_MAX_HEADS) return 0;
    return bwd_ws(d).total * sizeof(float);
}

extern "C" int caphn_hyper_backward(const caphn_hyper_desc* d, const float* dtheta, const float* acts,
                                    const caphn_hyper_grads* g, void* ws_, caphn_stream_t stream) {
    if (!desc_ok(d) || !dtheta || !acts || !g || !ws_) return CAPHN_EINVAL;
    hipStream_t s = static_cast<hipStream_t>(stream);
    const ActsLayout L = acts_layout(d);
    const BwdWs W = bwd_ws(d);
    float* ws = static_cast<float*>(ws_);
    const int nh = d->n_heads;
    size_t toff[CAPHN_MAX_HEADS]; { size_t o = 0; for (int i = 0; i < nh; ++i) { toff[i] = o; o += d->w[i]; } }

    for (int i = 0; i < nh; ++i)
        if (g->g_b2[i] && g->g_b2[i] != dtheta + toff[i])
            if (hipMemcpyAsync(g->g_b2[i], dtheta + toff[i], sizeof(float) * d->w[i], hipMemcpyDeviceToDevice, s) != hipSuccess)
                return CAPHN_ELAUNCH;

    {
        GemvTJobs jobs; jobs.n = nh; int b0 = 0; int kmax = 0;
        for (int i = 0; i < nh; ++i) {
            GemvTJob& J = jobs.j[i];
            J.W = d->w2[i]; J.d = dtheta + toff[i]; J.partial = ws + W.partial[i];
            J.rows = d->w[i]; J.k = d->k[i]; J.vec = (J.k % 4 == 0) && caphn_aligned16(J.W);
            J.block0 = b0; J.nblocks = W.nblocks[i]; b0 += J.nblocks;
            kmax = std::max(kmax, J.k);
        }
        size_t vec_floats = std::max(d->he, d_mid(d));
        { size_t kt = 0; for (int i = 0; i < nh; ++i) kt += caphn_align_up(d->k[i], 4); vec_floats = std::max(vec_floats, kt); }
        const bool fused_tail = g_tune_hyper_tail != 0 && vec_floats * sizeof(float) <= 64 * 1024;
        if (fused_tail) jobs.bar = reinterpret_cast<unsigned*>(ws + W.bar);
        int kv = 0;
        for (int i = 0; i < nh; ++i) if (jobs.j[i].vec && jobs.j[i].k <= 2048) kv = std::max(kv, jobs.j[i].k);
        const size_t shm = sizeof(float) * 4 * (kv > 0 ? kv : 1);
        if (kv <= 256) hipLaunchKernelGGL(gemv_t_partial_kernel<1>, dim3(b0), dim3(256), shm, s, jobs);
        else if (kv <= 512) hipLaunchKernelGGL(gemv_t_partial_kernel<2>, dim3(b0), dim3(256), shm, s, jobs);
        else if (kv <= 1024) hipLaunchKernelGGL(gemv_t_partial_kernel<4>, dim3(b0), dim3(256), shm, s, jobs);
        else hipLaunchKernelGGL(gemv_t_partial_kernel<8>, dim3(b0), dim3(256), shm, s, jobs);
        if (fused_tail) {
            TailArgs a;
            a.nh = nh; a.he = d->he; a.d_mid = d_mid(d); a.d_in = d_in(d);
            a.base_act = acts + L.base; a.a0_act = acts + L.a0; a.x_in = acts + L.x;
            a.base_w2 = d->base_w2; a.base_w0 = d->base_w0;
            a.g_base_b2 = g->g_base_b2; a.g_base_b0 = g->g_base_b0; a.g_base_w2 = g->g_base_w2; a.g_base_w0 = g->g_base_w0;
            a.g_x = g->g_x; a.x_acc = g->x_accumulate;
            a.dz = ws + W.dz[0]; a.dzb2 = ws + W.dzb2; a.dzb0 = ws + W.dzb0;
            a.bar = reinterpret_cast<unsigned*>(ws + W.bar);
            a.err = caphn_errword(); a.limit = g_tune_xch_timeout;
            int units = (d->he + STC - 1) / STC, p1 = 0, outer = 0;
            for (int i = 0; i < nh; ++i) {
                TailHead& H = a.h[i];
                H.partial = ws + W.partial[i]; H.post = acts + L.a[i]; H.w1 = d->w1[i]; H.g_b1 = g->g_b1[i]; H.g_w1 = g->g_w1[i];
                H.k = d->k[i]; H.nblocks = W.nblocks[i]; H.dzo = (int)(W.dz[i] - W.dz[0]);
                p1 += (H.k + 63) / 64;
                if (H.g_w1) outer += (int)(((size_t)H.k * d->he + 4095) / 4096);
            }
            units = std::max(units + outer, std::max(p1, std::max((d_mid(d) + STC - 1) / STC, (d_in(d) + STC - 1) / STC)));
            const int nb = std::max(1, std::min(64, units));
            hipLaunchKernelGGL(hyper_tail_kernel, dim3(nb), dim3(1024), vec_floats * sizeof(float), s, a);
            for (int i = 0; i < nh; ++i)
                if (g->g_w2[i]) {
                    OuterJobs o2; o2.n = 1;
                    OuterJob& J = o2.j[0];
                    J.g = dtheta + toff[i]; J.a = acts + L.a[i]; J.out = g->g_w2[i]; J.rows = d->w[i]; J.k = d->k[i]; J.block0 = 0;
                    long nbo = ((long)J.rows * J.k + 1023) / 1024;
                    hipLaunchKernelGGL(outer_kernel, dim3((unsigned)nbo), dim3(256), 0, s, o2);
                }
            return caphn_launch_status();
        }
        ReduceJobs rj; rj.n = nh;
        for (int i = 0; i < nh; ++i) {
            ReduceJob& R = rj.j[i];
            R.partial = ws + W.partial[i]; R.post = acts + L.a[i]; R.out0 = ws + W.dz[i]; R.out1 = g->g_b1[i];
            R.k = d->k[i]; R.nblocks = W.nblocks[i];
        }
        hipLaunchKernelGGL(gemv_t_reduce_kernel, dim3((kmax + 63) / 64, nh), dim3(1024), 0, s, rj);
    }
    {
        SmallTArgs a; a.n = nh; a.k = d->he; a.post = acts + L.base; a.out0 = ws + W.dzb2; a.out1 = g->g_base_b2;
        for (int i = 0; i < nh; ++i) { a.j[i].W = d->w1[i]; a.j[i].d = ws + W.dz[i]; a.j[i].rows = d->k[i]; }
        hipLaunchKernelGGL(gemv_t_small_kernel, dim3((d->he + STC - 1) / STC), dim3(1024), 0, s, a);
    }
    {
        SmallTArgs a; a.n = 1; a.k = d_mid(d); a.post = acts + L.a0; a.out0 = ws + W.dzb0; a.out1 = g->g_base_b0;
        a.j[0].W = d->base_w2; a.j[0].d = ws + W.dzb2; a.j[0].rows = d->he;
        hipLaunchKernelGGL(gemv_t_small_kernel, dim3((d_mid(d) + STC - 1) / STC), dim3(1024), 0, s, a);
    }
    if (g->g_x) {
        SmallTArgs a; a.n = 1; a.k = d_in(d); a.post = nullptr; a.out0 = g->g_x; a.out1 = nullptr; a.acc0 = g->x_accumulate;
        a.j[0].W = d->base_w0; a.j[0].d = ws + W.dzb0; a.j[0].rows = d_mid(d);
        hipLaunchKernelGGL(gemv_t_small_kernel, dim3((d_in(d) + STC - 1) / STC), dim3(1024), 0, s, a);
    }
    {
        OuterJobs oj; oj.n = 0; long b0 = 0;
        auto add = [&](const float* gv, const float* av, float* out, int rows, int k) {
            if (!out) return;
            OuterJob& J = oj.j[oj.n++];
            J.g = gv; J.a = av; J.out = out; J.rows = rows; J.k = k; J.block0 = b0;
            b0 += ((long)rows * k + 1023) / 1024;
        };
        add(ws + W.dzb0, acts + L.x, g->g_base_w0, d_mid(d), d_in(d));
        add(ws + W.dzb2, acts + L.a0, g->g_base_w2, d->he, d_mid(d));
        for (int i = 0; i < nh; ++i) add(ws + W.dz[i], acts + L.base, g->g_w1[i], d->k[i], d->he);
        if (oj.n) hipLaunchKernelGGL(outer_kernel, dim3((unsigned)b0), dim3(256), 0, s, oj);
        for (int i = 0; i < nh; ++i)
            if (g->g_w2[i]) {
                OuterJobs o2; o2.n = 1;
                OuterJob& J = o2.j[0];
                J.g = dtheta + toff[i]; J.a = acts + L.a[i]; J.out = g->g_w2[i]; J.rows = d->w[i]; J.k = d->k[i]; J.block0 = 0;
                long nb = ((long)J.rows * J.k + 1023) / 1024;
                hipLaunchKernelGGL(outer_kernel, dim3((unsigned)nb), dim3(256), 0, s, o2);
            }
    }
    return caphn_launch_status();
}

extern "C" int caphn_outer_f32(int rows, int k, const float* gv, const float* av, float* out, caphn_stream_t stream) {
    if (rows <= 0 || k <= 0 || !gv || !av || !out) return CAPHN_EINVAL;
    OuterJobs o2; o2.n = 1;
    OuterJob& J = o2.j[0];
    J.g = gv; J.a = av; J.out = out; J.rows = rows; J.k = k; J.block0 = 0;
    long nb = ((long)rows * k + 1023) / 1024;
    hipLaunchKernelGGL(outer_kernel, dim3((unsigned)nb), dim3(256), 0, static_cast<hipStream_t>(stream), o2);
    return caphn_launch_status();
}

extern int g_tune_adam;
extern int g_tune_gemm;
extern int g_tune_rec_rotate;
extern int g_tune_fork;
extern int g_tune_gemm_xcd;
extern int g_tune_gemm_fast;
extern int g_tune_gemm_planes;
extern int g_tune_rec_pair;
extern int g_tune_gemm_single;
extern int g_tune_gemm_tile;
extern int g_tune_deterministic;
extern int g_tune_adam_cap;
extern int g_tune_chain_main;
extern int g_tune_rec_cache;
extern int g_tune_splitk_target;
extern int g_tune_gemm_order;
extern int g_tune_branch_mask;
extern int g_tune_gemm_db;
extern int g_tune_gemm_ws;
extern int g_tune_adam_dense_cap;
extern int g_tune_sk_dhs, g_tune_sk_vocab_w;
extern int g_tune_join_chain;
extern int g_tune_gemm_kres;
extern int g_tune_gemm_waves;
extern int g_tune_hops;
extern int g_tune_vocab_order;
extern int g_det_vocab;
int caphn_rec_pair_debug_skip(int v);
int caphn_rec_pair_debug_opts(int v);
extern "C" int caphn_tune(int key, int value) {
    if (key == 0) { g_tune_gemv = value; return CAPHN_OK; }
    if (key == 1) { g_tune_adam = value; return CAPHN_OK; }
    if (key == 2) { g_tune_gemm = value; return CAPHN_OK; }
    if (key == 3) { g_tune_rec_rotate = value; return CAPHN_OK; }
    if (key == 4) { g_tune_fork = value; return CAPHN_OK; }
    if (key == 6) { g_tune_gemm_xcd = value; return CAPHN_OK; }
    if (key == 7) { g_tune_gemm_fast = value; return CAPHN_OK; }
    if (key == 8) { g_tune_gemm_planes = value; return CAPHN_OK; }
    if (key == 9) { g_tune_rec_pair = value; return CAPHN_OK; }
    if (key == 10) return caphn_rec_pair_debug_skip(value);
    if (key == 11) { g_tune_gemm_single = value; return CAPHN_OK; }
    if (key == 12) { g_tune_gemm_tile = value; return CAPHN_OK; }
    if (key == 13) { g_tune_deterministic = value > 0; g_det_vocab = value; return CAPHN_OK; }
    if (key == 21) { g_tune_vocab_order = value != 0; return CAPHN_OK; }
    if (key == 20) { if (value < 0 || value > 7) return CAPHN_EINVAL; g_tune_branch_mask = value; return CAPHN_OK; }
    if (key == 18) { if (value < 0 || value > 2) return CAPHN_EINVAL; g_tune_gemm_order = value; return CAPHN_OK; }
    if (key == 17) { if (value < 1 || value > 65536) return CAPHN_EINVAL; g_tune_splitk_target = value; return CAPHN_OK; }
    if (key == 16) { if (value < 0 || value > 2) return CAPHN_EINVAL; g_tune_rec_cache = value; return CAPHN_OK; }
    if (key == 15) { g_tune_chain_main = value != 0; return CAPHN_OK; }
    if (key == 26) { g_tune_hops = value != 0; return CAPHN_OK; }
    if (key == 27) { g_tune_hyper_tail = value != 0; return CAPHN_OK; }
    if (key == 28) { g_tune_acts_fused = value != 0; return CAPHN_OK; }
    if (key == 36) { g_tune_gemm_kres = value != 0; return CAPHN_OK; }
    if (key == 35) { g_tune_join_chain = value != 0; return CAPHN_OK; }
    if (key == 33) { if (value < 0 || value > 64) return CAPHN_EINVAL; g_tune_sk_dhs = value; return CAPHN_OK; }
    if (key == 34) { if (value < 0 || value > 64) return CAPHN_EINVAL; g_tune_sk_vocab_w = value; return CAPHN_OK; }
    if (key == 30) { if (value < 64 || value > 4096) return CAPHN_EINVAL; g_tune_vjp_blocks = value; return CAPHN_OK; }
    if (key == 31) { if (value < 64 || value > 65535) return CAPHN_EINVAL; g_tune_adam_dense_cap = value; return CAPHN_OK; }
    if (key == 29) { if (value != 0 && value != 64 && value != 128) return CAPHN_EINVAL; g_tune_gemm_ws = value; return CAPHN_OK; }
    if (key == 25) { if (value != 0 && value != 5 && value != 6) return CAPHN_EINVAL; g_tune_gemm_waves = value; return CAPHN_OK; }
    if (key == 24) return caphn_rec_pair_debug_opts(value);
    if (key == 23) { if (value < 0 || value > 7) return CAPHN_EINVAL; g_tune_gemm_db = value; return CAPHN_OK; }
    if (key == 22) { if (value < 1) return CAPHN_EINVAL; g_tune_xch_timeout = 100ll * value; return CAPHN_OK; }
    if (key == 14) { if (value < 64 || value > 65535) return CAPHN_EINVAL; g_tune_adam_cap = value; return CAPHN_OK; }
    return CAPHN_EINVAL;
}
```

hypernet-image-captioning_amd/csrc/misc.hip:

```cpp
#include "common.h"
#include "gemm_internal.h"
#include <math.h>

namespace {
constexpr int RMAX = 8;


__global__ __launch_bounds__(256) void ce_count_kernel(int rows, const int64_t* __restrict__ tgt, int64_t ignore, float* nvalid) {
    __shared__ int cnt[4];
    int c = 0;
    for (int i = threadIdx.x; i < rows; i += 256) c += (tgt[i] != ignore);
    float cf = wave_sum((float)c);
    if ((threadIdx.x & 63) == 0) cnt[threadIdx.x >> 6] = (int)cf;
    __syncthreads();
    if (threadIdx.x == 0) nvalid[0] = (float)(cnt[0] + cnt[1] + cnt[2] + cnt[3]);
}

__global__ __launch_bounds__(256) void ce_row_kernel(int V, int ld, const float* logits, const int64_t* __restrict__ tgt,
                                                     int64_t ignore, const float* __restrict__ nvalid, const int* __restrict__ nvi,
                                                     float* dlogits, float* __restrict__ row_loss, int vec) {
    __shared__ float red[4];
    __shared__ float bc[2];
    const int row = blockIdx.x, tid = threadIdx.x;
    const float* x = logits + (size_t)row * ld;
// ... 142 lines not shown
        out[i] = x[i] + branch[i] * (p > 0.f ? caphn_keep_scale(seed, offset + i, p, inv_keep) : 1.f);
}

__global__ __launch_bounds__(256) void scale_kernel(size_t n, const float* __restrict__ x, const float* __restrict__ scale, float* __restrict__ out) {
    const float c = scale[0];
    const size_t stride = (size_t)gridDim.x * 256;
    for (size_t i = (size_t)blockIdx.x * 256 + threadIdx.x; i < n; i += stride) out[i] = x[i] * c;
}

__global__ __launch_bounds__(256) void lrelu_bwd_kernel(size_t n, const float* __restrict__ dy, const float* __restrict__ post, float* __restrict__ dx) {
    for (size_t i = (size_t)blockIdx.x * 256 + threadIdx.x; i < n; i += (size_t)gridDim.x * 256) dx[i] = dy[i] * (post[i] > 0.f ? 1.f : 0.01f);
}
__global__ __launch_bounds__(256) void axpy_kernel(size_t n, float alpha, const float* __restrict__ x, float* __restrict__ y) {
    const size_t stride = (size_t)gridDim.x * 256;
    for (size_t i = (size_t)blockIdx.x * 256 + threadIdx.x; i < n; i += stride) y[i] = fmaf(alpha, x[i], y[i]);
}

__global__ __launch_bounds__(256) void colsum_kernel(int M, int N, const float* __restrict__ A, int lda,
                                                     float* __restrict__ out, int rows_per) {
    __shared__ float red[4][65];
    const int c = threadIdx.x & 63, rl = threadIdx.x >> 6;
    const int n = blockIdx.x * 64 + c;
    const int m0 = blockIdx.y * rows_per, m1 = min(M, m0 + rows_per);
    float s0 = 0.f, s1 = 0.f;
    if (n < N) {
        int m = m0 + rl;
        for (; m + 4 < m1; m += 8) { s0 += A[(size_t)m * lda + n]; s1 += A[(size_t)(m + 4) * lda + n]; }
        if (m < m1) s0 += A[(size_t)m * lda + n];
    }
    red[rl][c] = s0 + s1;
    __syncthreads();
    if (rl == 0 && n < N) out[(size_t)blockIdx.y * N + n] = (red[0][c] + red[1][c]) + (red[2][c] + red[3][c]);
}
inline int colsum_slices(int M, int N) {
    const int colblocks = (N + 63) / 64;
    int S = 2048 / colblocks;
    if (S > (M + 31) / 32) S = (M + 31) / 32;
    if (S > 256) S = 256;
    if (S < 1) S = 1;
    return S;
}

__global__ __launch_bounds__(256) void embed_gather_kernel(int rows, int E, const float* __restrict__ table, const int64_t* __restrict__ idx, float* __restrict__ out) {
    const int r = blockIdx.x;
    const int64_t id = idx[r];
    for (int e = threadIdx.x; e < E; e += 256) out[(size_t)r * E + e] = id < 0 ? 0.f : table[(size_t)id * E + e];
}
__global__ __launch_bounds__(256) void embed_gather_strided_kernel(int rows, int E, const float* __restrict__ table, const int64_t* __restrict__ idx,
                                                                   int istride, float* __restrict__ out, int ostride) {
    const int r = blockIdx.x;
    const int64_t id = idx[(size_t)r * istride];
    for (int e = threadIdx.x; e < E; e += 256) out[(size_t)r * ostride + e] = id < 0 ? 0.f : table[(size_t)id * E + e];
}
__global__ __launch_bounds__(256) void embed_scatter_det_kernel(int rows, int E, int V, const float* __restrict__ g, const int64_t* __restrict__ idx,
                                                                float* __restrict__ tg) {
    const int v = blockIdx.x * 4 + (threadIdx.x >> 6), lane = threadIdx.x & 63;
    if (v >= V) return;
    bool any = false;
    for (int r0 = 0; r0 < rows; r0 += 64) {
        const int r = r0 + lane;
        const bool hit = r < rows && idx[r] == (int64_t)v;
        unsigned long long ball = __ballot(hit);
        while (ball) {
            const int b = __ffsll((long long)ball) - 1;
            ball &= ball - 1;
            const float* src = g + (size_t)(r0 + b) * E;
            for (int e = lane; e < E; e += 64) tg[(size_t)v * E + e] += src[e];
            any = true;
        }
    }
    (void)any;
}
__global__ __launch_bounds__(256) void embed_scatter_kernel(int rows, int E, const float* __restrict__ g, const int64_t* __restrict__ idx, float* __restrict__ tg) {
    const int r = blockIdx.x;
    const int64_t id = idx[r];
    if (id < 0) return;
    for (int e = threadIdx.x; e < E; e += 256) atomicAdd(&tg[(size_t)id * E + e], g[(size_t)r * E + e]);
}

constexpr int SUMSQ_CHUNK = 256 * 4 * 8;
__global__ __launch_bounds__(256) void sumsq_kernel(size_t n, const float* __restrict__ x, double* __restrict__ partial, int vec) {
    __shared__ double red[4];
    const size_t base = (size_t)blockIdx.x * SUMSQ_CHUNK;
    float s = 0.f;
    if (vec && base + SUMSQ_CHUNK <= n) {
        const f32x4* x4 = reinterpret_cast<const f32x4*>(x + base);
#pragma unroll
        for (int i = 0; i < 8; ++i) { f32x4 v = x4[threadIdx.x + 256 * i]; s += v[0] * v[0] + v[1] * v[1] + v[2] * v[2] + v[3] * v[3]; }
    } else {
        for (size_t i = base + threadIdx.x; i < n && i < base + SUMSQ_CHUNK; i += 256) s += x[i] * x[i];
    }
    double d = wave_sum_d((double)s);
    if ((threadIdx.x & 63) == 0) red[threadIdx.x >> 6] = d;
    __syncthreads();
    if (threadIdx.x == 0) partial[blockIdx.x] = red[0] + red[1] + red[2] + red[3];
}

constexpr int GRAM_CHUNKS = 64;
struct GramJob { const float* gfac; size_t ldg; const float* afac; size_t lda; int rows, k; };
struct GramJobs { GramJob j[CAPHN_MAX_HEADS]; int n; };
__global__ __launch_bounds__(256) void rank_gram_kernel(int R, GramJobs jobs, double* __restrict__ ws) {
    __shared__ double red[4];
    const int pair = blockIdx.x, job = blockIdx.y >> 1, which = blockIdx.y & 1;
    const GramJob& J = jobs.j[job];
    const int r = pair / R, s = pair % R;
    const float* u = which ? J.afac + (size_t)r * J.lda : J.gfac + (size_t)r * J.ldg;
    const float* v = which ? J.afac + (size_t)s * J.lda : J.gfac + (size_t)s * J.ldg;
    const int n = which ? J.k : J.rows;
    const int per = (n + GRAM_CHUNKS - 1) / GRAM_CHUNKS;
    const int i0 = blockIdx.z * per, i1 = min(n, i0 + per);
    if (i0 >= i1) return;
    double acc = 0.0;
    for (int i = i0 + threadIdx.x; i < i1; i += 256) acc += (double)u[i] * (double)v[i];
    acc = wave_sum_d(acc);
    if ((threadIdx.x & 63) == 0) red[threadIdx.x >> 6] = acc;
    __syncthreads();
    if (threadIdx.x == 0) atomicAdd(&ws[((size_t)job * 2 + which) * R * R + pair], red[0] + red[1] + red[2] + red[3]);
}
__global__ void rank_gram_finish_kernel(int R, int njobs, const double* __restrict__ ws, double* acc) {
    if (threadIdx.x == 0 && blockIdx.x == 0) {
        double t = 0.0;
        for (int j = 0; j < njobs; ++j)
            for (int i = 0; i < R * R; ++i) t += ws[((size_t)j * 2) * R * R + i] * ws[((size_t)j * 2 + 1) * R * R + i];
        acc[0] += t;
    }
}
__global__ __launch_bounds__(256) void clip_coef_kernel(int nparts, const double* __restrict__ partial, const double* extra,
                                                        double max_norm, double scale, float* coef_out) {
    __shared__ double red[4];
    double s = 0.0;
// ... 596 lines not shown
    if (!in || !out || !(p >= 0.f) || !(p < 1.f)) return CAPHN_EINVAL;
    size_t blocks = (n + 255) / 256;
    if (blocks > 4096) blocks = 4096;
    hipLaunchKernelGGL(dropout_kernel, dim3((unsigned)blocks), dim3(256), 0, static_cast<hipStream_t>(stream), n, p, 1.0f / (1.0f - p), seed,
                       offset, in, out);
    return caphn_launch_status();
}
extern "C" int caphn_add_dropout_f32(size_t n, const float* x, const float* branch, float p, unsigned long long seed,
                                     unsigned long long offset, float* out, caphn_stream_t stream) {
    if (n == 0) return CAPHN_OK;
    if (!x || !branch || !out || !(p >= 0.f) || !(p < 1.f)) return CAPHN_EINVAL;
    size_t blocks = (n + 255) / 256;
    if (blocks > 4096) blocks = 4096;
    hipLaunchKernelGGL(add_dropout_kernel, dim3((unsigned)blocks), dim3(256), 0, static_cast<hipStream_t>(stream), n, p, 1.0f / (1.0f - p), seed,
                       offset, x, branch, out);
    return caphn_launch_status();
}
extern "C" int caphn_scale_f32(size_t n, const float* x, const float* scale_dev, float* out, caphn_stream_t stream) {
    if (n == 0) return CAPHN_OK;
    if (!x || !scale_dev || !out) return CAPHN_EINVAL;
    size_t blocks = (n + 255) / 256;
    if (blocks > 4096) blocks = 4096;
    hipLaunchKernelGGL(scale_kernel, dim3((unsigned)blocks), dim3(256), 0, static_cast<hipStream_t>(stream), n, x, scale_dev, out);
    return caphn_launch_status();
}
extern "C" int caphn_lrelu_bwd_f32(size_t n, const float* dy, const float* post, float* dx, caphn_stream_t stream) {
    if (n == 0) return CAPHN_OK;
    if (!dy || !post || !dx) return CAPHN_EINVAL;
    size_t blocks = (n + 255) / 256;
    if (blocks > 1024) blocks = 1024;
    hipLaunchKernelGGL(lrelu_bwd_kernel, dim3((unsigned)blocks), dim3(256), 0, static_cast<hipStream_t>(stream), n, dy, post, dx);
    return caphn_launch_status();
}
extern "C" int caphn_axpy_f32(size_t n, float alpha, const float* x, float* y, caphn_stream_t stream) {
    if (n == 0) return CAPHN_OK;
    if (!x || !y) return CAPHN_EINVAL;
    size_t blocks = (n + 255) / 256;
    if (blocks > 2048) blocks = 2048;
    hipLaunchKernelGGL(axpy_kernel, dim3((unsigned)blocks), dim3(256), 0, static_cast<hipStream_t>(stream), n, alpha, x, y);
    return caphn_launch_status();
}
extern "C" int caphn_embedding_gather(int rows, int E, const float* table, const int64_t* idx, float* out, caphn_stream_t stream) {
    if (rows <= 0 || E <= 0 || !table || !idx || !out) return CAPHN_EINVAL;
    hipLaunchKernelGGL(embed_gather_kernel, dim3(rows), dim3(256), 0, static_cast<hipStream_t>(stream), rows, E, table, idx, out);
    return caphn_launch_status();
}
int caphn_embedding_gather_strided(int rows, int E, const float* table, const int64_t* idx, int istride, float* out, int ostride, hipStream_t s) {
    if (rows <= 0 || E <= 0 || !table || !idx || !out) return CAPHN_EINVAL;
    hipLaunchKernelGGL(embed_gather_strided_kernel, dim3(rows), dim3(256), 0, s, rows, E, table, idx, istride, out, ostride);
    return caphn_launch_status();
}
extern int g_tune_deterministic;
int g_det_vocab = 0;
extern "C" int caphn_embedding_scatter_add_v(int rows, int E, int V, const float* g, const int64_t* idx, float* table_grad,
                                             caphn_stream_t stream) {
    if (rows <= 0 || E <= 0 || V <= 0 || !g || !idx || !table_grad) return CAPHN_EINVAL;
    if (g_tune_deterministic && rows > 1) {
        hipLaunchKernelGGL(embed_scatter_det_kernel, dim3((V + 3) / 4), dim3(256), 0, static_cast<hipStream_t>(stream), rows, E,
                           V, g, idx, table_grad);
        return caphn_launch_status();
    }
    hipLaunchKernelGGL(embed_scatter_kernel, dim3(rows), dim3(256), 0, static_cast<hipStream_t>(stream), rows, E, g, idx, table_grad);
    return caphn_launch_status();
}
extern "C" int caphn_embedding_scatter_add(int rows, int E, const float* g, const int64_t* idx, float* table_grad, caphn_stream_t stream) {
    if (rows <= 0 || E <= 0 || !g || !idx || !table_grad) return CAPHN_EINVAL;
    if (g_tune_deterministic && g_det_vocab > 0 && rows > 1) return caphn_embedding_scatter_add_v(rows, E, g_det_vocab, g, idx, table_grad, stream);
    hipLaunchKernelGGL(embed_scatter_kernel, dim3(rows), dim3(256), 0, static_cast<hipStream_t>(stream), rows, E, g, idx, table_grad);
    return caphn_launch_status();
}

extern "C" int caphn_sumsq_blocks(size_t n) { return (int)((n + SUMSQ_CHUNK - 1) / SUMSQ_CHUNK); }
extern "C" int caphn_sumsq_f32(size_t n, const float* x, double* partial, caphn_stream_t stream) {
    if (n == 0 || !x || !partial) return CAPHN_EINVAL;
    const int nb = caphn_sumsq_blocks(n);
    hipLaunchKernelGGL(sumsq_kernel, dim3(nb), dim3(256), 0, static_cast<hipStream_t>(stream), n, x, partial, (int)caphn_aligned16(x));
    return caphn_launch_status();
}
extern "C" int caphn_rank_sumsq_f32(int R, int rows, int k, const float* gfac, size_t ldg, const float* afac, size_t lda,
                                    double* acc, double* ws, caphn_stream_t stream) {
    if (R <= 0 || R > RMAX || rows <= 0 || k <= 0 || !gfac || !afac || !acc || !ws) return CAPHN_EINVAL;
    hipStream_t s = static_cast<hipStream_t>(stream);
    GramJobs jobs; jobs.n = 1;
    jobs.j[0] = GramJob{gfac, ldg, afac, lda, rows, k};
    if (hipMemsetAsync(ws, 0, sizeof(double) * 2 * R * R, s) != hipSuccess) return CAPHN_ELAUNCH;
    hipLaunchKernelGGL(rank_gram_kernel, dim3(R * R, 2, GRAM_CHUNKS), dim3(256), 0, s, R, jobs, ws);
    hipLaunchKernelGGL(rank_gram_finish_kernel, dim3(1), dim3(64), 0, s, R, 1, ws, acc);
    return caphn_launch_status();
}
extern "C" int caphn_rank_sumsq_multi_f32(int R, int n, const int* rows, const int* k, const float* const* gfac, const size_t* ldg,
                                          const float* const* afac, const size_t* lda, double* acc, double* ws,
                                          caphn_stream_t stream) {
    if (R <= 0 || R > RMAX || n <= 0 || n > CAPHN_MAX_HEADS || !rows || !k || !gfac || !ldg || !afac || !lda || !acc || !ws)
        return CAPHN_EINVAL;
    hipStream_t s = static_cast<hipStream_t>(stream);
    GramJobs jobs; jobs.n = n;
    for (int i = 0; i < n; ++i) {
        if (rows[i] <= 0 || k[i] <= 0 || !gfac[i] || !afac[i]) return CAPHN_EINVAL;
        jobs.j[i] = GramJob{gfac[i], ldg[i], afac[i], lda[i], rows[i], k[i]};
    }
    if (hipMemsetAsync(ws, 0, sizeof(double) * 2 * R * R * n, s) != hipSuccess) return CAPHN_ELAUNCH;
    hipLaunchKernelGGL(rank_gram_kernel, dim3(R * R, 2 * n, GRAM_CHUNKS), dim3(256), 0, s, R, jobs, ws);
    hipLaunchKernelGGL(rank_gram_finish_kernel, dim3(1), dim3(64), 0, s, R, n, ws, acc);
    return caphn_launch_status();
}
extern "C" size_t caphn_grad_norm_workspace_bytes(size_t n, int R, int njobs) {
    if (R <= 0 || R > RMAX || njobs < 0 || njobs > CAPHN_MAX_HEADS) return 0;
    return sizeof(double) * ((size_t)caphn_sumsq_blocks(n) + (size_t)njobs * 2 * R * R * NORM_CHUNKS);
}
extern "C" int caphn_grad_norm_coef(size_t n, const float* x, int R, int njobs, const int* rows, const int* k,
                                    const float* const* gfac, const size_t* ldg, const float* const* afac, const size_t* lda,
                                    double max_norm, double scale, float* coef_out, void* ws, caphn_stream_t stream) {
    if (n == 0 || !x || R <= 0 || R > RMAX || njobs < 0 || njobs > CAPHN_MAX_HEADS || !coef_out || !ws) return CAPHN_EINVAL;
    GramJobs jobs; jobs.n = njobs;
    for (int i = 0; i < njobs; ++i) {
        if (!rows || !k || !gfac || !ldg || !afac || !lda || rows[i] <= 0 || k[i] <= 0 || !gfac[i] || !afac[i]) return CAPHN_EINVAL;
        jobs.j[i] = GramJob{gfac[i], ldg[i], afac[i], lda[i], rows[i], k[i]};
    }
    const int nb_s = caphn_sumsq_blocks(n);
    const unsigned nb = (unsigned)nb_s + (unsigned)(njobs * 2 * R * R * NORM_CHUNKS);
    hipStream_t s = static_cast<hipStream_t>(stream);
// ... 259 lines not shown
```

hypernet-image-captioning_amd/csrc/recurrent_gru.hip:

```cpp
#include "common.h"
#include "decoder_internal.h"

namespace {

constexpr int NT = 1024;
#ifdef CAPHN_REC_PROFILE
#define PSTAMP(i) do { if (prof_on) { unsigned long long _n = clock64(); pc[i] += _n - plast; plast = _n; } } while (0)
#define PDECL const bool prof_on = (b == 0 && tid == 0 && a.prof != nullptr); \
    unsigned long long pc[8] = {0, 0, 0, 0, 0, 0, 0, 0}, plast = prof_on ? clock64() : 0
#define PFLUSH do { if (prof_on) for (int i = 0; i < 8; ++i) a.prof[i] = pc[i]; } while (0)
#else
#define PSTAMP(i) do { } while (0)
#define PDECL do { } while (0)
#define PFLUSH do { } while (0)
#endif

__device__ __forceinline__ void copy_to_lds(float* dst, const float* __restrict__ src, int n, int vec, int tid) {
    if (vec) {
        const f32x4* s4 = reinterpret_cast<const f32x4*>(src);
        f32x4* d4 = reinterpret_cast<f32x4*>(dst);
        for (int i = tid; i < (n >> 2); i += NT) d4[i] = s4[i];
    } else {
        for (int i = tid; i < n; i += NT) dst[i] = src[i];
    }
// ... 421 lines not shown
                dv += de * tv;
            }
            a.dWaf[((size_t)b * P + p) * H + k] = s * vk;
        }
        a.part[blk * (H + 1) + k] = dv;
    }
    if (threadIdx.x == 0) {
        float s = 0.f;
        for (int p = p0; p < p1; ++p)
            for (int t = 0; t < T; ++t) s += a.de[((size_t)b * T + t) * P + p];
        a.part[blk * (H + 1) + H] = s;
    }
}

__global__ __launch_bounds__(256) void dmean_kernel(int H, int F, const float* __restrict__ dh0, const float* __restrict__ Wh,
                                                    const float* __restrict__ dc0, const float* __restrict__ Wc, float* __restrict__ out) {
    extern __shared__ float dv[];
    const int b = blockIdx.x;
    for (int j = threadIdx.x; j < H; j += 256) { dv[j] = dh0[(size_t)b * H + j]; dv[H + j] = dc0 ? dc0[(size_t)b * H + j] : 0.f; }
    __syncthreads();
    for (int k = threadIdx.x; k < F; k += 256) {
        float s0 = 0.f, s1 = 0.f;
        int j = 0;
        for (; j + 8 <= H; j += 8) {
            float w[8], c[8];
#pragma unroll
            for (int u = 0; u < 8; ++u) { w[u] = Wh[(size_t)(j + u) * F + k]; c[u] = dc0 ? Wc[(size_t)(j + u) * F + k] : 0.f; }
#pragma unroll
            for (int u = 0; u < 8; ++u) { s0 += dv[j + u] * w[u]; s1 += dv[H + j + u] * c[u]; }
        }
        for (; j < H; ++j) { s0 += dv[j] * Wh[(size_t)j * F + k]; if (dc0) s1 += dv[H + j] * Wc[(size_t)j * F + k]; }
        out[(size_t)b * F + k] = s0 + s1;
    }
}

__global__ void ctx_kernel(int P, int F, int T, const float* __restrict__ alphas, const float* __restrict__ f, float* __restrict__ ctx,
                           int ldc) {
    const int b = blockIdx.x, t = blockIdx.y;
    const float* al = alphas + ((size_t)b * T + t) * P;
    for (int k = threadIdx.x; k < F; k += blockDim.x) {
        float s = 0.f;
        int p = 0;
        for (; p + 8 <= P; p += 8) {
            float v[8];
#pragma unroll
            for (int u = 0; u < 8; ++u) v[u] = f[((size_t)b * P + p + u) * F + k];
#pragma unroll
            for (int u = 0; u < 8; ++u) s += al[p + u] * v[u];
        }
        for (; p < P; ++p) s += al[p] * f[((size_t)b * P + p) * F + k];
        ctx[((size_t)b * T + t) * ldc + k] = s;
    }
}
__global__ void df_kernel(int P, int F, int T, const float* __restrict__ alphas, const float* __restrict__ dctx,
                          const float* __restrict__ dmean, const float* __restrict__ dmean2, float* __restrict__ df) {
    const int b = blockIdx.x, p = blockIdx.y;
    const float invP = 1.0f / (float)P;
    for (int k = threadIdx.x; k < F; k += blockDim.x) {
        float s = (dmean2 ? dmean[(size_t)b * F + k] + dmean2[(size_t)b * F + k] : dmean[(size_t)b * F + k]) * invP;
        int t = 0;
        for (; t + 8 <= T; t += 8) {
            float a[8], v[8];
#pragma unroll
            for (int u = 0; u < 8; ++u) { a[u] = alphas[((size_t)b * T + t + u) * P + p]; v[u] = dctx[((size_t)b * T + t + u) * F + k]; }
#pragma unroll
            for (int u = 0; u < 8; ++u) s += a[u] * v[u];
        }
        for (; t < T; ++t) s += alphas[((size_t)b * T + t) * P + p] * dctx[((size_t)b * T + t) * F + k];
        df[((size_t)b * P + p) * F + k] = s;
    }
}
__global__ __launch_bounds__(1024) void init_state_kernel(int P, int F, int H, const float* __restrict__ f,
                                                          const float* __restrict__ Wh, const float* __restrict__ bh,
                                                          const float* __restrict__ Wc, const float* __restrict__ bc,
                                                          float* __restrict__ meanf, float* __restrict__ h0, float* __restrict__ c0) {
    extern __shared__ float sm[];
    const int b = blockIdx.x, tid = threadIdx.x, lane = tid & 63, wave = tid >> 6;
    const int Fp = (F + 255) & ~255;
    for (int k0 = 0; k0 < F; k0 += 256) {
        const int k = k0 + (tid & 255), pl = tid >> 8;
        float s = 0.f;
        if (k < F) for (int p = pl; p < P; p += 4) s += f[((size_t)b * P + p) * F + k];
        sm[pl * Fp + k0 + (tid & 255)] = s;
    }
    __syncthreads();
    const float invP = 1.0f / (float)P;
    for (int k = tid; k < F; k += 1024) {
        const float m = ((sm[k] + sm[Fp + k]) + (sm[2 * Fp + k] + sm[3 * Fp + k])) * invP;
        sm[4 * Fp + k] = m;
        meanf[(size_t)b * F + k] = m;
    }
    __syncthreads();
    const float* mean = sm + 4 * Fp;
    for (int j = wave; j < H; j += 16) {
        float sh = 0.f, sc = 0.f;
        for (int k = lane; k < F; k += 64) {
            const float m = mean[k];
            sh += Wh[(size_t)j * F + k] * m;
            if (Wc) sc += Wc[(size_t)j * F + k] * m;
        }
        sh = wave_sum(sh);
        if (Wc) sc = wave_sum(sc);
        if (lane == 0) {
            h0[(size_t)b * H + j] = sh + bh[j];
            if (Wc) c0[(size_t)b * H + j] = sc + bc[j];
        }
    }
}
__global__ void mean_p_kernel(int P, int F, const float* __restrict__ f, float* __restrict__ out) {
    const int b = blockIdx.x;
    const float invP = 1.0f / (float)P;
    for (int k = threadIdx.x; k < F; k += blockDim.x) {
        float s = 0.f;
        for (int p = 0; p < P; ++p) s += f[((size_t)b * P + p) * F + k];
        out[(size_t)b * F + k] = s * invP;
    }
}

constexpr size_t LDS_LIMIT = 160 * 1024;
bool g_attr_set[64];
int ensure_lds_attr() {
// ... 16 lines not shown
    return sizeof(float) * ((size_t)RG * P * H + 4 * (size_t)H + (size_t)NG * H + Ppad + (size_t)kg_groups(H) * NG * H);
}
size_t caphn_rec_bwd_lds_bytes(int P, int H, int NG, int RG) {
    const size_t Ppad = (P + 63) & ~63;
    const int CH = (H % 4 == 0) ? 4 : 1;
    const int nch = (H + CH - 1) / CH;
    const int nch_eff = nch < NT ? nch : NT;
    int nsl = NT / nch_eff;
    if (kg_groups(H) > nsl) nsl = kg_groups(H);
    const int nsl1 = NT / (H < NT ? H : NT);
    if (nsl1 > nsl) nsl = nsl1;
    return sizeof(float) * ((size_t)RG * P * H + 5 * (size_t)H + 2 * (size_t)NG * H + 2 * Ppad + (size_t)nsl * H);
}
int caphn_rec_resident_gates(int P, int H, int NG) {
    for (int rg = NG; rg >= 0; --rg)
        if (caphn_rec_fwd_lds_bytes(P, H, NG, rg) <= LDS_LIMIT && caphn_rec_bwd_lds_bytes(P, H, NG, rg) <= LDS_LIMIT) return rg;
    return -1;
}

int caphn_launch_rec_fwd(const RecFwdArgs& a, bool lstm, hipStream_t s) {
    const size_t lds = caphn_rec_fwd_lds_bytes(a.P, a.H, lstm ? 4 : 3, a.RG);
    if (lds > LDS_LIMIT) return CAPHN_ELIMIT;
    int rc = ensure_lds_attr(); if (rc) return rc;
    if (lstm) hipLaunchKernelGGL(rec_attn_fwd_kernel<true>, dim3(a.B), dim3(NT), lds, s, a);
    else hipLaunchKernelGGL(rec_attn_fwd_kernel<false>, dim3(a.B), dim3(NT), lds, s, a);
    return caphn_launch_status();
}
int caphn_rec_bwd_groups(int P, int H) {
    if (H > NT) return 0;
    const int ng = NT / H;
    return (P + ng - 1) / ng <= PGM ? ng : 0;
}
int caphn_launch_rec_bwd(const RecBwdArgs& a, bool lstm, hipStream_t s) {
    if (a.dWaf && (!a.apart || caphn_rec_bwd_groups(a.P, a.H) == 0)) return CAPHN_EINVAL;
    const size_t lds = caphn_rec_bwd_lds_bytes(a.P, a.H, lstm ? 4 : 3, a.RG);
    if (lds > LDS_LIMIT) return CAPHN_ELIMIT;
    int rc = ensure_lds_attr(); if (rc) return rc;
    if (lstm) hipLaunchKernelGGL(rec_attn_bwd_kernel<true>, dim3(a.B), dim3(NT), lds, s, a);
    else hipLaunchKernelGGL(rec_attn_bwd_kernel<false>, dim3(a.B), dim3(NT), lds, s, a);
    return caphn_launch_status();
}
int caphn_launch_attn_param_grads(const AttnGradArgs& a, int B, int npc, hipStream_t s) {
    hipLaunchKernelGGL(attn_param_grads_kernel, dim3(B, npc), dim3(a.H >= 192 ? 256 : 64), 0, s, a);
    return caphn_launch_status();
}
int caphn_launch_dmean(int B, int H, int F, const float* dh0, const float* Wh, const float* dc0, const float* Wc, float* out, hipStream_t s) {
    hipLaunchKernelGGL(dmean_kernel, dim3(B), dim3(256), sizeof(float) * 2 * H, s, H, F, dh0, Wh, dc0, Wc, out);
    return caphn_launch_status();
}
int caphn_launch_ctx(int B, int T, int P, int F, const float* alphas, const float* f, float* ctx, int ldc, hipStream_t s) {
    hipLaunchKernelGGL(ctx_kernel, dim3(B, T), dim3(F >= 192 ? 256 : 64), 0, s, P, F, T, alphas, f, ctx, ldc);
    return caphn_launch_status();
}
int caphn_launch_df(int B, int T, int P, int F, const float* alphas, const float* dctx, const float* dmean, float* df, hipStream_t s,
                    const float* dmean2) {
    hipLaunchKernelGGL(df_kernel, dim3(B, P), dim3(F >= 192 ? 256 : 64), 0, s, P, F, T, alphas, dctx, dmean, dmean2, df);
    return caphn_launch_status();
}
int caphn_launch_init_state(int B, int P, int F, int H, const float* f, const float* Wh, const float* bh, const float* Wc,
                            const float* bc, float* meanf, float* h0, float* c0, hipStream_t s) {
    const int Fp = (F + 255) & ~255;
    hipLaunchKernelGGL(init_state_kernel, dim3(B), dim3(1024), sizeof(float) * (4 * Fp + F), s, P, F, H, f, Wh, bh, Wc, bc, meanf, h0, c0);
    return caphn_launch_status();
}
int caphn_launch_mean_p(int B, int P, int F, const float* f, float* out, hipStream_t s) {
    hipLaunchKernelGGL(mean_p_kernel, dim3(B), dim3(F >= 192 ? 256 : 64), 0, s, P, F, f, out);
    return caphn_launch_status();
}
```

include/caphn.h:

```cpp
#ifndef CAPHN_H
#define CAPHN_H
#include <stdint.h>
#include <stddef.h>

#ifdef __cplusplus
extern "C" {
#endif

typedef void* caphn_stream_t;

#define CAPHN_OK 0
#define CAPHN_EINVAL (-1)
#define CAPHN_ELAUNCH (-2)
#define CAPHN_ELIMIT (-3)
#define CAPHN_ETIMEOUT (-4)

int caphn_abi_version(void);
int caphn_device_error(int clear);
int caphn_device_arch(char* buf, int buflen);

#define CAPHN_GEMM_BIAS 1
#define CAPHN_GEMM_RELU 2
#define CAPHN_GEMM_ACCUM 4
#define CAPHN_GEMM_MASK 8
#define CAPHN_GEMM_LRELU 16
int caphn_gemm_f32(int ta, int tb, int M, int N, int K,
                   const float* A, int lda, const float* B, int ldb,
                   float* C, int ldc, const float* bias,
                   const float* mask, int ldmask, int flags, int splitk,
                   caphn_stream_t stream);

int caphn_split3_bf16(const float* src, int rows, int cols, int ld, void* planes, int ldp, size_t plane_stride, int zero_rows,
                      caphn_stream_t stream);
int caphn_gemm_planes_f32(int ta, int tb, int M, int N, int K,
                          const float* A, int lda, const void* Ap, int ldap, size_t psa,
                          const float* B, int ldb, const void* Bp, int ldbp, size_t psb,
                          float* C, int ldc, const float* bias, const float* mask, int ldmask, int flags, int splitk,
                          int Kp, caphn_stream_t stream);

int caphn_zero_f32(float* p, size_t n, caphn_stream_t stream);
int caphn_dropout_f32(size_t n, float p, unsigned long long seed, unsigned long long offset, const float* in, float* out,
                      caphn_stream_t stream);
int caphn_add_dropout_f32(size_t n, const float* x, const float* branch, float p, unsigned long long seed,
                          unsigned long long offset, float* out, caphn_stream_t stream);
int caphn_scale_f32(size_t n, const float* x, const float* scale_dev, float* out, caphn_stream_t stream);
int caphn_lrelu_bwd_f32(size_t n, const float* dy, const float* post, float* dx, caphn_stream_t stream);
int caphn_axpy_f32(size_t n, float alpha, const float* x, float* y, caphn_stream_t stream);
int caphn_linear_wgrad_f32(int M, int N, int K, const float* dY, int ldy, const float* X, int ldx, float* dW, int ldw,
                           float* db, void* ws, caphn_stream_t stream);
size_t caphn_colsum_workspace_bytes(int M, int N);
int caphn_colsum_f32(int M, int N, const float* A, int lda, float* out, void* ws, caphn_stream_t stream);

#define CAPHN_MAX_HEADS 8
typedef struct caphn_hyper_desc {
    int he;
    int n_heads;
    int k[CAPHN_MAX_HEADS];
    int w[CAPHN_MAX_HEADS];
    const float* base_w0; const float* base_b0;
    const float* base_w2; const float* base_b2;
    const float* w1[CAPHN_MAX_HEADS]; const float* b1[CAPHN_MAX_HEADS];
    const float* w2[CAPHN_MAX_HEADS]; const float* b2[CAPHN_MAX_HEADS];
    int d_in, d_mid;
} caphn_hyper_desc;

int caphn_hyper_acts_floats(const caphn_hyper_desc* d);
int caphn_hyper_forward(const caphn_hyper_desc* d, const float* x, float* theta, float* acts,
                        caphn_stream_t stream);

int caphn_hyper_forward_acts(const caphn_hyper_desc* d, const float* x, float* acts, caphn_stream_t stream);

typedef struct caphn_hyper_grads {
    float* g_base_w0; float* g_base_b0; float* g_base_w2; float* g_base_b2;
    float* g_w1[CAPHN_MAX_HEADS]; float* g_b1[CAPHN_MAX_HEADS];
    float* g_w2[CAPHN_MAX_HEADS]; float* g_b2[CAPHN_MAX_HEADS];
    float* g_x;
    int x_accumulate;
} caphn_hyper_grads;
size_t caphn_hyper_backward_workspace_bytes(const caphn_hyper_desc* d);
int caphn_hyper_backward(const caphn_hyper_desc* d, const float* dtheta, const float* acts,
                         const caphn_hyper_grads* g, void* ws, caphn_stream_t stream);

#define CAPHN_CELL_GRU 0
#define CAPHN_CELL_LSTM 1
typedef struct caphn_decoder_dims {
    int B, T, P;
    int D, F, E, H, V;
    int cell;
    int raw_features;
    int row_subset;
    int grads_zeroed;
    int precomputed;
    int layers;
    float dropout_p;
    unsigned long long dropout_seed;
    int logits_ld;
} caphn_decoder_dims;

#define CAPHN_MAX_DEC_LAYERS 4
typedef struct caphn_decoder_params {
    const float* fc0_w; const float* fc0_b;
    const float* fc2_w; const float* fc2_b;
// ... 209 lines not shown
```

Baseline: 82400 images/s.

## Merge shared-input weight-gradient GEMMs into multi-panel launches and fuse dXe/dctx GEMM

Adds a multi-panel TN GEMM+colsum path so weight gradients that share the same input (W_hh and Ua from Hprev) run as one launch, with each block choosing its panel. The dXe and dctx input-gradient GEMMs are fused into a single GEMM over E+F columns by giving them an interleaved layout, and the embed scatter and df kernels now take a leading dimension. The hyper backward is split into a prepare step issued early and a run step. This cuts kernel launches and repeated reads of the shared operand, but it changes the stream placement and the dependencies between streams.

```diff
diff --git a/hypernet-image-captioning_amd/caphn/_lib.py b/hypernet-image-captioning_amd/caphn/_lib.py
--- a/hypernet-image-captioning_amd/caphn/_lib.py
+++ b/hypernet-image-captioning_amd/caphn/_lib.py
@@ -107,6 +107,9 @@
     "caphn_dropout_f32": (C.c_int, [C.c_size_t, C.c_float, C.c_uint64, C.c_uint64, c_fp, c_fp, c_fp]),
     "caphn_colsum_workspace_bytes": (C.c_size_t, [C.c_int, C.c_int]),
     "caphn_linear_wgrad_f32": (C.c_int, [C.c_int, C.c_int, C.c_int, c_fp, C.c_int, c_fp, C.c_int, c_fp, C.c_int, c_fp, c_fp, c_fp]),
+    "caphn_linear_wgrad_panels_f32": (C.c_int, [C.c_int, C.POINTER(C.c_int), C.c_int, C.c_int, C.POINTER(C.c_void_p), C.POINTER(C.c_int),
+                                                c_fp, C.c_int, C.POINTER(C.c_void_p), C.POINTER(C.c_int), C.POINTER(C.c_void_p), C.c_int,
+                                                c_fp, c_fp]),
     "caphn_colsum_f32": (C.c_int, [C.c_int, C.c_int, c_fp, C.c_int, c_fp, c_fp, c_fp]),
     "caphn_hyper_acts_floats": (C.c_int, [C.POINTER(HyperDesc)]),
     "caphn_hyper_forward": (C.c_int, [C.POINTER(HyperDesc), c_fp, c_fp, c_fp, c_fp]),
diff --git a/hypernet-image-captioning_amd/caphn/ops.py b/hypernet-image-captioning_amd/caphn/ops.py
--- a/hypernet-image-captioning_amd/caphn/ops.py
+++ b/hypernet-image-captioning_amd/caphn/ops.py
@@ -124,6 +124,20 @@
     L.check(lib.caphn_linear_wgrad_f32(M, N, K, L.ptr(dy), dy.stride(0), L.ptr(x), x.stride(0), L.ptr(dw), N, L.ptr(db),
                                        C.c_void_p(ws.data_ptr()), L.stream_ptr()), "caphn_linear_wgrad_f32")
     return dw, db
+
+
+def linear_wgrad_panels(dys, x: torch.Tensor, splitk: int = 1):
+    lib = L.load()
+    n, (K, N) = len(dys), x.shape
+    assert all(dy.shape[0] == K and dy.stride(1) == 1 for dy in dys) and x.stride(1) == 1
+    outs = [(_f32(dy.shape[1], N, device=x.device), _f32(dy.shape[1], device=x.device)) for dy in dys]
+    ws = torch.empty(lib.caphn_colsum_workspace_bytes(K, max(dy.shape[1] for dy in dys)), dtype=torch.uint8, device=x.device)
+    ints = lambda v: (C.c_int * n)(*v)
+    ptrs = lambda ts: (C.c_void_p * n)(*[t.data_ptr() for t in ts])
+    L.check(lib.caphn_linear_wgrad_panels_f32(n, ints([dy.shape[1] for dy in dys]), N, K, ptrs(dys), ints([dy.stride(0) for dy in dys]),
+                                              L.ptr(x), x.stride(0), ptrs([o[0] for o in outs]), ints([N] * n), ptrs([o[1] for o in outs]),
+                                              int(splitk), C.c_void_p(ws.data_ptr()), L.stream_ptr()), "caphn_linear_wgrad_panels_f32")
+    return outs
 
 
 def bahdanau_fwd(f: torch.Tensor, waf: torch.Tensor, uah: torch.Tensor, v_a: torch.Tensor, b_va: torch.Tensor):
diff --git a/hypernet-image-captioning_amd/csrc/decoder.hip b/hypernet-image-captioning_amd/csrc/decoder.hip
--- a/hypernet-image-captioning_amd/csrc/decoder.hip
+++ b/hypernet-image-captioning_amd/csrc/decoder.hip
@@ -15,6 +15,7 @@
 int g_tune_hops = 0;
 int g_tune_fork = 4;
 int g_tune_join_chain = 0;
+int g_tune_post_merge = 1;
 int g_tune_sk_dhs = 0, g_tune_sk_vocab_w = 0;
 #define RUN(x) do { int _rc = (x); if (_rc != CAPHN_OK) return _rc; } while (0)
 
@@ -135,7 +136,7 @@
 
 struct Ws {
     size_t Y1, f, meanf, h0, c0, Waf, G, Xe, Xg, Hs, Hprev, gates, hn, Cs, Cprev, uah, alphas, idx;
-    size_t dHs, dgi, dgh, duah, de, dh0, dc0, ctx, dctx, dXe, dWaf, dmeanf, df, dY1, apart, vtmp, colws, colws_s[3], prof, rowmap;
+    size_t dHs, dgi, dgh, duah, de, dh0, dc0, ctx, dctx, dXe, ldx, dWaf, dmeanf, df, dY1, apart, vtmp, colws, colws_s[3], prof, rowmap;
     size_t xch, xch_floats;
     size_t wp;
     size_t H0s, dH0, h0L, dcarry, tgi, tgh, tmpA, tmpB;
@@ -168,8 +169,8 @@
     w.uah = take(B * T * H); w.alphas = take(B * T * P); w.idx = take(2 * B * T);
     w.dHs = take(B * T * H); w.dgi = take(B * T * NG * H); w.dgh = take(lstm ? 0 : B * T * NG * H); w.duah = take(B * T * H);
     w.de = take(B * T * P); w.dh0 = take(B * H); w.dc0 = take(lstm ? B * H : 0);
-    w.ctx = w.Xe + E; w.dctx = take(raw ? 0 : B * T * F);
-    w.dXe = take(B * T * E); w.dWaf = take(B * P * H); w.dmeanf = take(raw ? 0 : 2 * B * F); w.df = take(raw ? 0 : B * P * F);
+    w.ctx = w.Xe + E; w.ldx = raw ? E : E + F;
+    w.dXe = take(B * T * w.ldx); w.dctx = w.dXe + E; w.dWaf = take(B * P * H); w.dmeanf = take(raw ? 0 : 2 * B * F); w.df = take(raw ? 0 : B * P * F);
     w.dY1 = take(raw ? 0 : B * P * F);
     w.pchunk = 1; w.npc = (int)((P + w.pchunk - 1) / w.pchunk);
     const size_t arows = std::max<size_t>(std::max<size_t>(w.npc, (size_t)caphn_rec_bwd_groups((int)P, (int)H)),
@@ -695,26 +696,41 @@
         RUN(wgrad_bias(V, H, BT, dlogits, LV, ws + w.Hs, H, g->out_w, H, g->out_b, rmap, cws, b0, gz));
         RUN(sd.milestone(CAPHN_MS_VOCAB, b0));
     }
+    if (hook) RUN(caphn_hyper_backward_prepare(hook->hd, hook->ws, sT));
     if (ctx_side) RUN(sd.wait(5, sT));
     else if (!(d->precomputed & 32)) RUN(caphn_launch_ctx(B, T, P, F, ws + w.alphas, f, ws + w.ctx, EF, sT));
     if (lstm) RUN(gemm_auto(1, 0, GH, EF, BT, dgi, GH, ws + w.Xe, EF, g->w_ih, EF, nullptr, 0, sT, nullptr, 0, gz));
     else RUN(wgrad_bias(GH, EF, BT, dgi, GH, ws + w.Xe, EF, g->w_ih, EF, g->b_ih, nullptr, cw1, sT, gz));
+    const bool merge = g_tune_post_merge != 0;
+    if (merge) {
+        const TnPanel pn[2] = {{dgh, GH, GH, g->w_hh, H, g->b_hh, pick_splitk(GH, H, BT)},
+                               {ws + w.duah, H, H, g->Ua_w, H, g->Ua_b, pick_splitk(H, H, BT)}};
+        RUN(caphn_gemm_tn_colsum_panels(2, pn, H, BT, ws + w.Hprev, H, nullptr, cw2, gz, b2));
+    } else
     RUN(wgrad_bias(GH, H, BT, dgh, GH, ws + w.Hprev, H, g->w_hh, H, g->b_hh, nullptr, cw2, b2, gz));
     if (lstm) RUN(caphn_colsum_f32(BT, GH, dgi, GH, g->b_ih, cw2, b2));
     RUN(sd.record(3, b2));
     hipStream_t se = late ? b2 : b0;
-    RUN(caphn_gemm_f32(0, 0, BT, E, GH, dgi, GH, p->w_ih, EF, ws + w.dXe, E, nullptr, nullptr, 0, 0, 1, se));
+    const int ldx = (int)w.ldx;
+    const bool xmerge = merge && !raw && caphn_gemm_bf16x3_tile(BT, EF, GH, 1) == caphn_gemm_bf16x3_tile(BT, E, GH, 1) &&
+                        caphn_gemm_bf16x3_tile(BT, EF, GH, 1) == caphn_gemm_bf16x3_tile(BT, F, GH, 1);
+    if (xmerge) {
+        RUN(caphn_gemm_f32(0, 0, BT, EF, GH, dgi, GH, p->w_ih, EF, ws + w.dXe, ldx, nullptr, nullptr, 0, 0, 1, sF));
+        RUN(sd.record(0, sF));
+    } else
+    RUN(caphn_gemm_f32(0, 0, BT, E, GH, dgi, GH, p->w_ih, EF, ws + w.dXe, ldx, nullptr, nullptr, 0, 0, 1, se));
     if (!gz) RUN(caphn_zero_f32(g->embed_w, (size_t)V * E, se));
-    RUN(caphn_embedding_scatter_add_v(BT, E, V, ws + w.dXe, idx, g->embed_w, se));
+    if (xmerge) RUN(sd.wait(0, se));
+    RUN(caphn_launch_embed_scatter(BT, E, V, ws + w.dXe, ldx, idx, g->embed_w, se));
     RUN(sd.milestone(CAPHN_MS_EMBED, se));
     RUN(sd.wait(3, sT));
     RUN(sd.milestone(CAPHN_MS_DTHETA, sT));
     if (hook && !hold_big) {
-        RUN(caphn_hyper_backward(hook->hd, g->w_ih, hook->acts, hook->hg, hook->ws, sT));
+        RUN(caphn_hyper_backward_run(hook->hd, g->w_ih, hook->acts, hook->hg, hook->ws, sT));
     }
     if (!hold_big) RUN(sd.milestone(CAPHN_MS_HYPER, sT));
     if (!raw) {
-        RUN(caphn_gemm_f32(0, 0, BT, F, GH, dgi, GH, p->w_ih + E, EF, ws + w.dctx, F, nullptr, nullptr, 0, 0, 1, sF));
+        if (!xmerge) RUN(caphn_gemm_f32(0, 0, BT, F, GH, dgi, GH, p->w_ih + E, EF, ws + w.dctx, ldx, nullptr, nullptr, 0, 0, 1, sF));
         if (!pair)
             RUN(caphn_launch_dmean(B, H, F, ws + w.dh0, p->inith_w, lstm ? ws + w.dc0 : nullptr, lstm ? p->initc_w : nullptr,
                                    ws + w.dmeanf, sF));
@@ -725,7 +741,7 @@
     ag.dWaf = ws + w.dWaf; ag.part = ws + w.apart;
     if (ang == 0) RUN(caphn_launch_attn_param_grads(ag, B, w.npc, sF));
     RUN(sd.record(2, sF));
-    RUN(wgrad_bias(H, H, BT, ws + w.duah, H, ws + w.Hprev, H, g->Ua_w, H, g->Ua_b, nullptr, cws, b0, gz));
+    if (!merge) RUN(wgrad_bias(H, H, BT, ws + w.duah, H, ws + w.Hprev, H, g->Ua_w, H, g->Ua_b, nullptr, cws, b0, gz));
     for (int l = 0; l < w.L1; ++l) {
         const int BS = B * (T + 1), G3 = 3 * H;
         RUN(wgrad_bias(G3, H, BS, ws + w.Ldgi[l], G3, ws + w.Lin[l], H, g->lw_ih[l], H, g->lb_ih[l], nullptr, cws, b0, gz));
@@ -734,7 +750,7 @@
     RUN(wgrad_bias(H, F, B, ws + w.dh0, H, ws + w.meanf, F, g->inith_w, F, g->inith_b, nullptr, cws, b0, gz));
     if (lstm) RUN(wgrad_bias(H, F, B, ws + w.dc0, H, ws + w.meanf, F, g->initc_w, F, g->initc_b, nullptr, cws, b0, gz));
     if (!raw) {
-        RUN(caphn_launch_df(B, T, P, F, ws + w.alphas, ws + w.dctx, ws + w.dmeanf, ws + w.df, sF, pair ? ws + w.dmeanf + (size_t)B * F : nullptr));
+        RUN(caphn_launch_df(B, T, P, F, ws + w.alphas, ws + w.dctx, ldx, ws + w.dmeanf, ws + w.df, sF, pair ? ws + w.dmeanf + (size_t)B * F : nullptr));
         RUN(caphn_gemm_f32(0, 0, BP, F, H, ws + w.dWaf, H, p->Wa_w, F, ws + w.df, F, nullptr, nullptr, 0, CAPHN_GEMM_ACCUM, 1, sF));
         RUN(sd.record(4, sF));
         if (hold_big) {
@@ -743,7 +759,7 @@
             RUN(sd.milestone(CAPHN_MS_VOCAB, b0));
             if (hook) {
                 RUN(sd.wait(4, sT));
-                RUN(caphn_hyper_backward(hook->hd, g->w_ih, hook->acts, hook->hg, hook->ws, sT));
+                RUN(caphn_hyper_backward_run(hook->hd, g->w_ih, hook->acts, hook->hg, hook->ws, sT));
             }
             RUN(sd.milestone(CAPHN_MS_HYPER, sT));
         }
@@ -996,6 +1012,16 @@
     return caphn_launch_search_result(sa, steps_done, seqs, lengths, scores, finished, n_active, static_cast<hipStream_t>(stream));
 }
 
+extern "C" int caphn_linear_wgrad_panels_f32(int n, const int* M, int N, int K, const float* const* dY, const int* ldy, const float* X, int ldx,
+                                             float* const* dW, const int* ldw, float* const* db, int splitk, void* ws, caphn_stream_t stream) {
+    if (n < 1 || n > CAPHN_MAX_HEADS || !M || N <= 0 || K <= 0 || !dY || !ldy || !X || !dW || !ldw || !db || !ws || splitk < 1) return CAPHN_EINVAL;
+    TnPanel pn[CAPHN_MAX_HEADS];
+    for (int i = 0; i < n; ++i) {
+        if (M[i] <= 0 || !dY[i] || !dW[i] || !db[i]) return CAPHN_EINVAL;
+        pn[i] = TnPanel{dY[i], ldy[i], M[i], dW[i], ldw[i], db[i], splitk};
+    }
+    return caphn_gemm_tn_colsum_panels(n, pn, N, K, X, ldx, nullptr, ws, false, static_cast<hipStream_t>(stream));
+}
 extern "C" int caphn_linear_wgrad_f32(int M, int N, int K, const float* dY, int ldy, const float* X, int ldx, float* dW, int ldw,
                                       float* db, void* ws, caphn_stream_t stream) {
     if (M <= 0 || N <= 0 || K <= 0 || !dY || !X || !dW || !db || !ws) return CAPHN_EINVAL;
diff --git a/hypernet-image-captioning_amd/csrc/decoder_internal.h b/hypernet-image-captioning_amd/csrc/decoder_internal.h
--- a/hypernet-image-captioning_amd/csrc/decoder_internal.h
+++ b/hypernet-image-captioning_amd/csrc/decoder_internal.h
@@ -101,8 +101,11 @@
 int caphn_rec_bwd_groups(int P, int H);
 int caphn_launch_attn_param_grads(const AttnGradArgs& a, int B, int npc, hipStream_t s);
 int caphn_launch_ctx(int B, int T, int P, int F, const float* alphas, const float* f, float* ctx, int ldc, hipStream_t s);
-int caphn_launch_df(int B, int T, int P, int F, const float* alphas, const float* dctx, const float* dmean, float* df, hipStream_t s,
+int caphn_launch_df(int B, int T, int P, int F, const float* alphas, const float* dctx, int ldd, const float* dmean, float* df, hipStream_t s,
                     const float* dmean2 = nullptr);
+int caphn_launch_embed_scatter(int rows, int E, int V, const float* g, int ldg, const int64_t* idx, float* table_grad, hipStream_t s);
+int caphn_hyper_backward_prepare(const caphn_hyper_desc* d, void* ws, hipStream_t s);
+int caphn_hyper_backward_run(const caphn_hyper_desc* d, const float* dtheta, const float* acts, const caphn_hyper_grads* g, void* ws, hipStream_t s);
 int caphn_launch_dmean(int B, int H, int F, const float* dh0, const float* Wh, const float* dc0, const float* Wc, float* out, hipStream_t s);
 int caphn_launch_init_state(int B, int P, int F, int H, const float* f, const float* Wh, const float* bh, const float* Wc,
                             const float* bc, float* meanf, float* h0, float* c0, hipStream_t s);
diff --git a/hypernet-image-captioning_amd/csrc/gemm_bf16x3.hip b/hypernet-image-captioning_amd/csrc/gemm_bf16x3.hip
--- a/hypernet-image-captioning_amd/csrc/gemm_bf16x3.hip
+++ b/hypernet-image-captioning_amd/csrc/gemm_bf16x3.hip
@@ -1,6 +1,7 @@
 #include "common.h"
 #include "gemm_internal.h"
 #include "split3.h"
+#include <algorithm>
 #include <type_traits>
 
 #ifdef CAPHN_GEMM_PROFILE
@@ -266,6 +267,9 @@
         if (g.flags & (1 << 22)) { by = wgid % ny; bx = (wgid / ny) % nx; }
         else { bx = wgid % nx; by = (wgid / nx) % ny; }
         bz = wgid / (nx * ny);
+    }
+    if constexpr (TA && !TB) {
+        if (!gemm_pick_panel(g, by, bz)) return;
     }
     const int m0 = by * BM, n0 = bx * BN;
     const int* rmapA = nullptr; const int* kmap = nullptr;
@@ -702,7 +706,7 @@
         if (hipFuncSetAttribute(fn, hipFuncAttributeMaxDynamicSharedMemorySize, (int)(lds_tiles + 16384)) != hipSuccess) return CAPHN_ELAUNCH;
         attr_set[dev] = true;
     }
-    dim3 grid((g.N + BN - 1) / BN, (g.M + BM - 1) / BM, g.splitk > 1 ? g.splitk : 1);
+    dim3 grid((g.N + BN - 1) / BN, g.npanels > 1 ? g.ptiles : (g.M + BM - 1) / BM, g.splitk > 1 ? g.splitk : 1);
     if constexpr (PL == 5) {
         hipLaunchKernelGGL((gemm_bf16x3_kernel_ws<BM, BN, TA, TB>), grid, dim3(512), lds, s, g);
         return caphn_launch_status();
@@ -759,11 +763,19 @@
     if (tile == 128) return !ta && tb ? occ_one<128, 128, false, true>() : !ta ? occ_one<128, 128, false, false>() : !tb ? occ_one<128, 128, true, false>() : occ_one<128, 128, true, true>();
     return !ta && tb ? occ_one<64, 64, false, true>() : !ta ? occ_one<64, 64, false, false>() : !tb ? occ_one<64, 64, true, false>() : occ_one<64, 64, true, true>();
 }
+int caphn_gemm_bf16x3_tile(int M, int N, int K, int splitk) {
+    long tiles128 = (long)((M + 127) / 128) * ((N + 127) / 128) * (splitk > 1 ? splitk : 1);
+    if (K < 512) tiles128 = 0;
+    if (g_tune_gemm_tile == 64) tiles128 = 0; else if (g_tune_gemm_tile == 128) tiles128 = 1 << 20;
+    return tiles128 >= 512 ? 128 : 64;
+}
 int caphn_gemm_bf16x3_launch(GemmArgs g, int ta, int tb, hipStream_t s) {
     if (g_tune_gemm_xcd) g.flags |= 1 << 20;
     g.kmap_lds = 0;
     if (g.map_mode == 2 && ta && !tb) {
-        const int nslab = (g.K + 31) / 32, sk = g.splitk > 1 ? g.splitk : 1;
+        int skmin = g.splitk;
+        for (int i = 0; i < g.npanels; ++i) skmin = std::min(skmin, g.panel[i].splitk);
+        const int nslab = (g.K + 31) / 32, sk = skmin > 1 ? skmin : 1;
         const int ints = ((nslab + sk - 1) / sk) * 32;
         if (ints <= 4096) g.kmap_lds = ints;
     }
@@ -776,9 +788,21 @@
         const double abytes = 4.0 * (double)g.M * g.K, bbytes = 4.0 * (double)g.N * g.K, l2 = 3.0 * 1024 * 1024;
         if (g_tune_gemm_order == 2 || (bbytes > l2 && abytes < bbytes)) g.flags |= 1 << 22;
     }
-    long tiles128 = (long)((g.M + 127) / 128) * ((g.N + 127) / 128) * g.splitk;
-    if (g.K < 512) tiles128 = 0;
-    if (g_tune_gemm_tile == 64) tiles128 = 0; else if (g_tune_gemm_tile == 128) tiles128 = 1 << 20;
+    long tiles128 = 0;
+    if (g.npanels > 1) {
+        if (!ta || tb || g.npanels > CAPHN_MAX_HEADS || g.map_mode == 1) return CAPHN_EINVAL;
+        const int tile = caphn_gemm_bf16x3_tile(g.panel[0].M, g.N, g.K, g.panel[0].splitk);
+        int t0 = 0, skmax = 1;
+        for (int i = 0; i < g.npanels; ++i) {
+            GemmPanel& P = g.panel[i];
+            if (caphn_gemm_bf16x3_tile(P.M, g.N, g.K, P.splitk) != tile) return CAPHN_EINVAL;
+            P.tile0 = t0; t0 += (P.M + tile - 1) / tile;
+            skmax = std::max(skmax, P.splitk);
+        }
+        g.ptiles = t0; g.splitk = skmax; g.Ap = nullptr; g.Bp = nullptr;
+        tiles128 = tile == 128 ? 1 << 20 : 0;
+    } else
+    tiles128 = caphn_gemm_bf16x3_tile(g.M, g.N, g.K, g.splitk) == 128 ? 1 << 20 : 0;
     const bool pl = caphn_gemm_planes_ok(g, ta, tb);
     if (!pl && g_tune_gemm_single == 0 && g_tune_gemm_tile == 0 && g_tune_gemm_ws == 0) {
         const int rc = caphn_gemm_kres_launch(g, ta, tb, s);
diff --git a/hypernet-image-captioning_amd/csrc/gemm_f32.hip b/hypernet-image-captioning_amd/csrc/gemm_f32.hip
--- a/hypernet-image-captioning_amd/csrc/gemm_f32.hip
+++ b/hypernet-image-captioning_amd/csrc/gemm_f32.hip
@@ -1,5 +1,6 @@
 #include "common.h"
 #include "gemm_internal.h"
+#include <algorithm>
 
 int g_tune_gemm = 1;
 
@@ -77,7 +78,11 @@
     const int tid = threadIdx.x, lane = tid & 63, wave = tid >> 6;
     const int wm = wave >> 1, wn = wave & 1;
     const int li = lane & 31, kh = lane >> 5;
-    const int m0 = blockIdx.y * BM, n0 = blockIdx.x * BN;
+    int by = blockIdx.y;
+    if constexpr (TA && !TB) {
+        if (!gemm_pick_panel(g, by, blockIdx.z)) return;
+    }
+    const int m0 = by * BM, n0 = blockIdx.x * BN;
 
     const int nslab_total = (g.K + BK - 1) / BK;
     int slab0 = 0, slab1 = nslab_total;
@@ -158,7 +163,7 @@
 
 template <int BM, int BN, int BK>
 int launch_cfg(const GemmArgs& g, int ta, int tb, hipStream_t s) {
-    dim3 grid((g.N + BN - 1) / BN, (g.M + BM - 1) / BM, g.splitk > 1 ? g.splitk : 1);
+    dim3 grid((g.N + BN - 1) / BN, g.npanels > 1 ? g.ptiles : (g.M + BM - 1) / BM, g.splitk > 1 ? g.splitk : 1);
     dim3 block(256);
     if (!ta && tb) hipLaunchKernelGGL((gemm_f32_kernel<BM, BN, false, true, BK>), grid, block, 0, s, g);
     else if (!ta && !tb) hipLaunchKernelGGL((gemm_f32_kernel<BM, BN, false, false, BK>), grid, block, 0, s, g);
@@ -214,6 +219,75 @@
     g.row_map = rowmap ? rowmap + 4 : nullptr; g.dev_count = rowmap; g.map_mode = rowmap ? 2 : 0;
     g.colsum_a = colsum_out; g.kmap_lds = 0;
     g.Ap = nullptr; g.Bp = nullptr; g.ldap = g.ldbp = 0; g.psa = g.psb = 0;
+    return caphn_gemm_bf16x3_launch(g, 1, 0, s);
+}
+
+int caphn_gemm_f32_panels(GemmArgs g, hipStream_t s) {
+    if (g.npanels < 2 || g.npanels > CAPHN_MAX_HEADS) return CAPHN_EINVAL;
+    const int BK = (g.K % 40 == 0 && g.K % 32 != 0) ? 40 : 32;
+    const int nslab = (g.K + BK - 1) / BK;
+    long t128 = 0; int skmax = 1;
+    for (int i = 0; i < g.npanels; ++i) {
+        GemmPanel& P = g.panel[i];
+        if (P.splitk > nslab) P.splitk = nslab;
+        if (P.splitk < 1) P.splitk = 1;
+        P.slabs_per_split = (nslab + P.splitk - 1) / P.splitk;
+        t128 += (long)((P.M + 127) / 128) * ((g.N + 127) / 128) * P.splitk;
+        skmax = std::max(skmax, P.splitk);
+    }
+    const int tile = t128 >= 1024 ? 128 : 64;
+    int t0 = 0;
+    for (int i = 0; i < g.npanels; ++i) { g.panel[i].tile0 = t0; t0 += (g.panel[i].M + tile - 1) / tile; }
+    g.ptiles = t0; g.splitk = skmax;
+    if (tile == 128) return BK == 40 ? launch_cfg<128, 128, 40>(g, 1, 0, s) : launch_cfg<128, 128, 32>(g, 1, 0, s);
+    return BK == 40 ? launch_cfg<64, 64, 40>(g, 1, 0, s) : launch_cfg<64, 64, 32>(g, 1, 0, s);
+}
+
+int caphn_gemm_tn_colsum_panels(int np, const TnPanel* p, int N, int K, const float* B, int ldb, const int* rowmap, void* cws,
+                                bool prezeroed, hipStream_t s) {
+    if (np < 1 || np > CAPHN_MAX_HEADS || !p || N <= 0 || K <= 0 || !B) return CAPHN_EINVAL;
+    for (int i = 0; i < np; ++i) if (p[i].rows <= 0 || !p[i].A || !p[i].dW || !p[i].db) return CAPHN_EINVAL;
+    const int nslab = (K + 31) / 32;
+    const bool f32 = g_tune_gemm != 1 && !rowmap;
+    int sk[CAPHN_MAX_HEADS];
+    bool one = np > 1;
+    for (int i = 0; i < np; ++i) {
+        sk[i] = std::max(1, std::min(p[i].splitk, nslab));
+        if (!f32 && caphn_gemm_bf16x3_tile(p[i].rows, N, K, sk[i]) != caphn_gemm_bf16x3_tile(p[0].rows, N, K, sk[0])) one = false;
+    }
+    if (!one) {
+        for (int i = 0; i < np; ++i) {
+            const int rc = caphn_gemm_tn_colsum(p[i].rows, N, K, p[i].A, p[i].lda, B, ldb, p[i].dW, p[i].ldc, p[i].db, p[i].splitk, rowmap, cws, prezeroed, s);
+            if (rc) return rc;
+        }
+        return CAPHN_OK;
+    }
+    GemmArgs g;
+    g.M = p[0].rows; g.N = N; g.K = K; g.A = p[0].A; g.lda = p[0].lda; g.B = B; g.ldb = ldb; g.C = p[0].dW; g.ldc = p[0].ldc;
+    g.bias = nullptr; g.mask = nullptr; g.ldmask = 0; g.flags = 0;
+    g.splitk = sk[0]; g.slabs_per_split = (nslab + sk[0] - 1) / sk[0];
+    g.vecA = caphn_aligned16(p[0].A) && (p[0].lda % 4 == 0);
+    g.vecB = caphn_aligned16(B) && (ldb % 4 == 0);
+    g.row_map = rowmap ? rowmap + 4 : nullptr; g.dev_count = rowmap; g.map_mode = rowmap ? 2 : 0;
+    g.colsum_a = f32 ? nullptr : p[0].db; g.kmap_lds = 0;
+    g.Ap = nullptr; g.Bp = nullptr; g.ldap = g.ldbp = 0; g.psa = g.psb = 0;
+    g.npanels = np;
+    for (int i = 0; i < np; ++i) {
+        GemmPanel& P = g.panel[i];
+        P.A = p[i].A; P.C = p[i].dW; P.colsum_a = f32 ? nullptr : p[i].db; P.lda = p[i].lda; P.M = p[i].rows; P.ldc = p[i].ldc; P.tile0 = 0;
+        P.splitk = sk[i]; P.slabs_per_split = (nslab + sk[i] - 1) / sk[i];
+        P.vecA = caphn_aligned16(p[i].A) && (p[i].lda % 4 == 0);
+        if ((sk[i] > 1 || rowmap) && !prezeroed) {
+            if (P.ldc == N) { int rc = caphn_zero_f32(P.C, (size_t)P.M * N, s); if (rc) return rc; }
+            else if (hipMemset2DAsync(P.C, sizeof(float) * P.ldc, 0, sizeof(float) * N, P.M, s) != hipSuccess) return CAPHN_ELAUNCH;
+        }
+        if (!f32 && !prezeroed) { int rc = caphn_zero_f32(P.colsum_a, (size_t)P.M, s); if (rc) return rc; }
+    }
+    if (f32) {
+        int rc = caphn_gemm_f32_panels(g, s);
+        for (int i = 0; i < np && !rc; ++i) rc = caphn_colsum_f32(K, p[i].rows, p[i].A, p[i].lda, p[i].db, cws, s);
+        return rc;
+    }
     return caphn_gemm_bf16x3_launch(g, 1, 0, s);
 }
 
diff --git a/hypernet-image-captioning_amd/csrc/gemm_internal.h b/hypernet-image-captioning_amd/csrc/gemm_internal.h
--- a/hypernet-image-captioning_amd/csrc/gemm_internal.h
+++ b/hypernet-image-captioning_amd/csrc/gemm_internal.h
@@ -1,5 +1,11 @@
 #pragma once
 #include "common.h"
+
+struct GemmPanel {
+    const float* A; float* C; float* colsum_a;
+    int lda, M, ldc, tile0, splitk, slabs_per_split, vecA;
+};
+struct TnPanel { const float* A; int lda; int rows; float* dW; int ldc; float* db; int splitk; };
 
 struct GemmArgs {
     int M, N, K;
@@ -16,7 +22,23 @@
     int kmap_lds;
     const void* Ap; int ldap; size_t psa;
     const void* Bp; int ldbp; size_t psb;
+    int npanels = 0, ptiles = 0;
+    GemmPanel panel[CAPHN_MAX_HEADS];
 };
+
+#ifdef __HIPCC__
+__device__ __forceinline__ bool gemm_pick_panel(GemmArgs& g, int& by, int bz) {
+    if (g.npanels <= 1) return true;
+    GemmPanel p = g.panel[0];
+#pragma unroll
+    for (int i = 1; i < CAPHN_MAX_HEADS; ++i)
+        if (i < g.npanels && by >= g.panel[i].tile0) p = g.panel[i];
+    g.A = p.A; g.lda = p.lda; g.M = p.M; g.C = p.C; g.ldc = p.ldc; g.colsum_a = p.colsum_a; g.vecA = p.vecA;
+    g.splitk = p.splitk; g.slabs_per_split = p.slabs_per_split;
+    by -= p.tile0;
+    return bz < (p.splitk > 1 ? p.splitk : 1);
+}
+#endif
 
 struct Opnd {
     const float* f; int ld;
@@ -50,6 +72,11 @@
 int caphn_gemm_tn_colsum(int M, int N, int K, const float* A, int lda, const float* B, int ldb, float* C, int ldc,
                          float* colsum_out, int splitk, const int* rowmap, void* cws, bool prezeroed, hipStream_t s);
 
+int caphn_gemm_tn_colsum_panels(int np, const TnPanel* p, int N, int K, const float* B, int ldb, const int* rowmap, void* cws,
+                                bool prezeroed, hipStream_t s);
+int caphn_gemm_f32_panels(GemmArgs g, hipStream_t s);
+int caphn_gemm_bf16x3_tile(int M, int N, int K, int splitk);
+
 bool caphn_gemm_planes_ok(const GemmArgs& g, int ta, int tb);
 int caphn_gemm_bf16x3_launch(GemmArgs g, int ta, int tb, hipStream_t s);
 int caphn_gemm_kres_launch(const GemmArgs& g, int ta, int tb, hipStream_t s);
diff --git a/hypernet-image-captioning_amd/csrc/hyper.hip b/hypernet-image-captioning_amd/csrc/hyper.hip
--- a/hypernet-image-captioning_amd/csrc/hyper.hip
+++ b/hypernet-image-captioning_amd/csrc/hyper.hip
@@ -1,4 +1,5 @@
 #include "common.h"
+#include "decoder_internal.h"
 #include <algorithm>
 
 namespace {
@@ -237,6 +238,7 @@
 struct GemvTJob {
     const float* W; const float* d; float* partial;
     int rows, k, vec, block0, nblocks;
+    unsigned* ticket; const float* post; float* out0; float* out1;
 };
 struct GemvTJobs { GemvTJob j[CAPHN_MAX_HEADS]; int n; unsigned* bar = nullptr; };
 
@@ -276,6 +278,43 @@
     __syncthreads();
     for (int c = tid; c < J.k; c += 256)
         J.partial[(size_t)lb * J.k + c] = red[c] + red[J.k + c] + red[2 * J.k + c] + red[3 * J.k + c];
+}
+
+constexpr int RL = 16;
+__device__ __forceinline__ void gemv_t_finish(const GemvTJob& J, int tid, float* red) {
+    const bool v4 = (J.k & 3) == 0;
+    for (int c0 = 0; c0 < J.k; c0 += 64) {
+        if (v4) {
+            const int c = c0 + 4 * (tid & 15), rl = tid >> 4;
+            f32x4 acc = {0.f, 0.f, 0.f, 0.f};
+            if (c < J.k) {
+#pragma unroll 8
+                for (int b = rl; b < J.nblocks; b += RL) acc += *reinterpret_cast<const f32x4*>(J.partial + (size_t)b * J.k + c);
+            }
+#pragma unroll
+            for (int e = 0; e < 4; ++e) red[rl * 65 + 4 * (tid & 15) + e] = acc[e];
+        } else {
+            const int c = c0 + (tid & 63);
+#pragma unroll
+            for (int j = 0; j < 4; ++j) {
+                const int rl = (tid >> 6) + 4 * j;
+                float acc = 0.f;
+                if (c < J.k)
+                    for (int b = rl; b < J.nblocks; b += RL) acc += J.partial[(size_t)b * J.k + c];
+                red[rl * 65 + (tid & 63)] = acc;
+            }
+        }
+        __syncthreads();
+        if (tid < 64 && c0 + tid < J.k) {
+            float s = 0.f;
+#pragma unroll
+            for (int i = 0; i < RL; ++i) s += red[i * 65 + tid];
+            if (J.post) s *= lrelu_grad(J.post[c0 + tid]);
+            if (J.out0) J.out0[c0 + tid] = s;
+            if (J.out1) J.out1[c0 + tid] = s;
+        }
+        __syncthreads();
+    }
 }
 
 template <int QMAX>
@@ -316,9 +355,22 @@
             for (int j = 0; j < CJ; ++j) if (c0 + 256 * j < J.k) J.partial[(size_t)lb * J.k + c0 + 256 * j] = s[j];
         }
     }
-}
-
-constexpr int RL = 16;
+    if (!J.ticket) return;
+    __shared__ unsigned last_s;
+    __builtin_amdgcn_fence(__ATOMIC_RELEASE, "agent");
+    __syncthreads();
+    if (tid == 0) {
+        const unsigned t = __hip_atomic_fetch_add(J.ticket, 1u, __ATOMIC_RELAXED, __HIP_MEMORY_SCOPE_AGENT);
+        const bool last = t == (unsigned)J.nblocks - 1u;
+        if (last) __hip_atomic_store(J.ticket, 0u, __ATOMIC_RELAXED, __HIP_MEMORY_SCOPE_AGENT);
+        last_s = last ? 1u : 0u;
+    }
+    __syncthreads();
+    if (!last_s) return;
+    __builtin_amdgcn_fence(__ATOMIC_ACQUIRE, "agent");
+    gemv_t_finish(J, tid, red);
+}
+
 __device__ __forceinline__ float col_reduce_finish(float acc, float (*red)[65]) {
     const int c = threadIdx.x & 63, rl = threadIdx.x >> 6;
     red[rl][c] = acc;
@@ -390,6 +442,7 @@
 }
 
 
+int g_tune_vjp_fold = 0;
 int g_tune_vjp_blocks = 512;
 int g_tune_hyper_tail = 0;
 struct TailHead { const float* partial; const float* post; const float* w1; float* g_b1; float* g_w1; int k, nblocks, dzo; };
@@ -680,7 +733,7 @@
 
 namespace {
 struct BwdWs { size_t partial[CAPHN_MAX_HEADS]; int nblocks[CAPHN_MAX_HEADS]; size_t dz[CAPHN_MAX_HEADS];
-               size_t dzb2, dzb0, bar, total; };
+               size_t dzb2, dzb0, bar, tick, total; };
 constexpr int VJP_BLOCKS_MAX = 4096;
 inline BwdWs bwd_ws(const caphn_hyper_desc* d) {
     BwdWs w; size_t o = 0;
@@ -696,6 +749,7 @@
     w.dzb0 = o; o += caphn_align_up(d_mid(d), 4);
     o = caphn_align_up(o, 32);
     w.bar = o; o += 32;
+    w.tick = o; o += 32;
     w.total = o;
     return w;
 }
@@ -706,10 +760,20 @@
     return bwd_ws(d).total * sizeof(float);
 }
 
+int caphn_hyper_backward_prepare(const caphn_hyper_desc* d, void* ws_, hipStream_t s) {
+    if (!desc_ok(d) || !ws_) return CAPHN_EINVAL;
+    return caphn_zero_f32(static_cast<float*>(ws_) + bwd_ws(d).tick, 32, s);
+}
 extern "C" int caphn_hyper_backward(const caphn_hyper_desc* d, const float* dtheta, const float* acts,
                                     const caphn_hyper_grads* g, void* ws_, caphn_stream_t stream) {
     if (!desc_ok(d) || !dtheta || !acts || !g || !ws_) return CAPHN_EINVAL;
-    hipStream_t s = static_cast<hipStream_t>(stream);
+    const int rc = caphn_hyper_backward_prepare(d, ws_, static_cast<hipStream_t>(stream));
+    if (rc != CAPHN_OK) return rc;
+    return caphn_hyper_backward_run(d, dtheta, acts, g, ws_, static_cast<hipStream_t>(stream));
+}
+int caphn_hyper_backward_run(const caphn_hyper_desc* d, const float* dtheta, const float* acts,
+                             const caphn_hyper_grads* g, void* ws_, hipStream_t s) {
+    if (!desc_ok(d) || !dtheta || !acts || !g || !ws_) return CAPHN_EINVAL;
     const ActsLayout L = acts_layout(d);
     const BwdWs W = bwd_ws(d);
     float* ws = static_cast<float*>(ws_);
@@ -728,6 +792,7 @@
             J.W = d->w2[i]; J.d = dtheta + toff[i]; J.partial = ws + W.partial[i];
             J.rows = d->w[i]; J.k = d->k[i]; J.vec = (J.k % 4 == 0) && caphn_aligned16(J.W);
             J.block0 = b0; J.nblocks = W.nblocks[i]; b0 += J.nblocks;
+            J.ticket = nullptr; J.post = nullptr; J.out0 = nullptr; J.out1 = nullptr;
             kmax = std::max(kmax, J.k);
         }
         size_t vec_floats = std::max(d->he, d_mid(d));
@@ -736,7 +801,13 @@
         if (fused_tail) jobs.bar = reinterpret_cast<unsigned*>(ws + W.bar);
         int kv = 0;
         for (int i = 0; i < nh; ++i) if (jobs.j[i].vec && jobs.j[i].k <= 2048) kv = std::max(kv, jobs.j[i].k);
-        const size_t shm = sizeof(float) * 4 * (kv > 0 ? kv : 1);
+        const bool fold = g_tune_vjp_fold != 0 && !fused_tail;
+        if (fold)
+            for (int i = 0; i < nh; ++i) {
+                GemvTJob& J = jobs.j[i];
+                J.ticket = reinterpret_cast<unsigned*>(ws + W.tick) + i; J.post = acts + L.a[i]; J.out0 = ws + W.dz[i]; J.out1 = g->g_b1[i];
+            }
+        const size_t shm = sizeof(float) * std::max<size_t>(4 * (size_t)(kv > 0 ? kv : 1), fold ? RL * 65 : 0);
         if (kv <= 256) hipLaunchKernelGGL(gemv_t_partial_kernel<1>, dim3(b0), dim3(256), shm, s, jobs);
         else if (kv <= 512) hipLaunchKernelGGL(gemv_t_partial_kernel<2>, dim3(b0), dim3(256), shm, s, jobs);
         else if (kv <= 1024) hipLaunchKernelGGL(gemv_t_partial_kernel<4>, dim3(b0), dim3(256), shm, s, jobs);
@@ -772,6 +843,7 @@
                 }
             return caphn_launch_status();
         }
+        if (!fold) {
         ReduceJobs rj; rj.n = nh;
         for (int i = 0; i < nh; ++i) {
             ReduceJob& R = rj.j[i];
@@ -779,6 +851,7 @@
             R.k = d->k[i]; R.nblocks = W.nblocks[i];
         }
         hipLaunchKernelGGL(gemv_t_reduce_kernel, dim3((kmax + 63) / 64, nh), dim3(1024), 0, s, rj);
+        }
     }
     {
         SmallTArgs a; a.n = nh; a.k = d->he; a.post = acts + L.base; a.out0 = ws + W.dzb2; a.out1 = g->g_base_b2;
@@ -852,6 +925,7 @@
 extern int g_tune_sk_dhs, g_tune_sk_vocab_w;
 extern int g_tune_join_chain;
 extern int g_tune_gemm_kres;
+extern int g_tune_post_merge;
 extern int g_tune_gemm_waves;
 extern int g_tune_hops;
 extern int g_tune_vocab_order;
@@ -882,6 +956,8 @@
     if (key == 27) { g_tune_hyper_tail = value != 0; return CAPHN_OK; }
     if (key == 28) { g_tune_acts_fused = value != 0; return CAPHN_OK; }
     if (key == 36) { g_tune_gemm_kres = value != 0; return CAPHN_OK; }
+    if (key == 37) { g_tune_vjp_fold = value != 0; return CAPHN_OK; }
+    if (key == 38) { g_tune_post_merge = value != 0; return CAPHN_OK; }
     if (key == 35) { g_tune_join_chain = value != 0; return CAPHN_OK; }
     if (key == 33) { if (value < 0 || value > 64) return CAPHN_EINVAL; g_tune_sk_dhs = value; return CAPHN_OK; }
     if (key == 34) { if (value < 0 || value > 64) return CAPHN_EINVAL; g_tune_sk_vocab_w = value; return CAPHN_OK; }
diff --git a/hypernet-image-captioning_amd/csrc/misc.hip b/hypernet-image-captioning_amd/csrc/misc.hip
--- a/hypernet-image-captioning_amd/csrc/misc.hip
+++ b/hypernet-image-captioning_amd/csrc/misc.hip
@@ -218,8 +218,8 @@
     const int64_t id = idx[(size_t)r * istride];
     for (int e = threadIdx.x; e < E; e += 256) out[(size_t)r * ostride + e] = id < 0 ? 0.f : table[(size_t)id * E + e];
 }
-__global__ __launch_bounds__(256) void embed_scatter_det_kernel(int rows, int E, int V, const float* __restrict__ g, const int64_t* __restrict__ idx,
-                                                                float* __restrict__ tg) {
+__global__ __launch_bounds__(256) void embed_scatter_det_kernel(int rows, int E, int V, const float* __restrict__ g, int ldg,
+                                                                const int64_t* __restrict__ idx, float* __restrict__ tg) {
     const int v = blockIdx.x * 4 + (threadIdx.x >> 6), lane = threadIdx.x & 63;
     if (v >= V) return;
     bool any = false;
@@ -230,18 +230,18 @@
         while (ball) {
             const int b = __ffsll((long long)ball) - 1;
             ball &= ball - 1;
-            const float* src = g + (size_t)(r0 + b) * E;
+            const float* src = g + (size_t)(r0 + b) * ldg;
             for (int e = lane; e < E; e += 64) tg[(size_t)v * E + e] += src[e];
             any = true;
         }
     }
     (void)any;
 }
-__global__ __launch_bounds__(256) void embed_scatter_kernel(int rows, int E, const float* __restrict__ g, const int64_t* __restrict__ idx, float* __restrict__ tg) {
+__global__ __launch_bounds__(256) void embed_scatter_kernel(int rows, int E, const float* __restrict__ g, int ldg, const int64_t* __restrict__ idx, float* __restrict__ tg) {
     const int r = blockIdx.x;
     const int64_t id = idx[r];
     if (id < 0) return;
-    for (int e = threadIdx.x; e < E; e += 256) atomicAdd(&tg[(size_t)id * E + e], g[(size_t)r * E + e]);
+    for (int e = threadIdx.x; e < E; e += 256) atomicAdd(&tg[(size_t)id * E + e], g[(size_t)r * ldg + e]);
 }
 
 constexpr int SUMSQ_CHUNK = 256 * 4 * 8;
@@ -944,21 +944,23 @@
 }
 extern int g_tune_deterministic;
 int g_det_vocab = 0;
+int caphn_launch_embed_scatter(int rows, int E, int V, const float* g, int ldg, const int64_t* idx, float* table_grad, hipStream_t s) {
+    if (rows <= 0 || E <= 0 || V <= 0 || ldg < E || !g || !idx || !table_grad) return CAPHN_EINVAL;
+    if (g_tune_deterministic && rows > 1) {
+        hipLaunchKernelGGL(embed_scatter_det_kernel, dim3((V + 3) / 4), dim3(256), 0, s, rows, E, V, g, ldg, idx, table_grad);
+        return caphn_launch_status();
+    }
+    hipLaunchKernelGGL(embed_scatter_kernel, dim3(rows), dim3(256), 0, s, rows, E, g, ldg, idx, table_grad);
+    return caphn_launch_status();
+}
 extern "C" int caphn_embedding_scatter_add_v(int rows, int E, int V, const float* g, const int64_t* idx, float* table_grad,
                                              caphn_stream_t stream) {
-    if (rows <= 0 || E <= 0 || V <= 0 || !g || !idx || !table_grad) return CAPHN_EINVAL;
-    if (g_tune_deterministic && rows > 1) {
-        hipLaunchKernelGGL(embed_scatter_det_kernel, dim3((V + 3) / 4), dim3(256), 0, static_cast<hipStream_t>(stream), rows, E,
-                           V, g, idx, table_grad);
-        return caphn_launch_status();
-    }
-    hipLaunchKernelGGL(embed_scatter_kernel, dim3(rows), dim3(256), 0, static_cast<hipStream_t>(stream), rows, E, g, idx, table_grad);
-    return caphn_launch_status();
+    return caphn_launch_embed_scatter(rows, E, V, g, E, idx, table_grad, static_cast<hipStream_t>(stream));
 }
 extern "C" int caphn_embedding_scatter_add(int rows, int E, const float* g, const int64_t* idx, float* table_grad, caphn_stream_t stream) {
     if (rows <= 0 || E <= 0 || !g || !idx || !table_grad) return CAPHN_EINVAL;
     if (g_tune_deterministic && g_det_vocab > 0 && rows > 1) return caphn_embedding_scatter_add_v(rows, E, g_det_vocab, g, idx, table_grad, stream);
-    hipLaunchKernelGGL(embed_scatter_kernel, dim3(rows), dim3(256), 0, static_cast<hipStream_t>(stream), rows, E, g, idx, table_grad);
+    hipLaunchKernelGGL(embed_scatter_kernel, dim3(rows), dim3(256), 0, static_cast<hipStream_t>(stream), rows, E, g, E, idx, table_grad);
     return caphn_launch_status();
 }
 
diff --git a/hypernet-image-captioning_amd/csrc/recurrent_gru.hip b/hypernet-image-captioning_amd/csrc/recurrent_gru.hip
--- a/hypernet-image-captioning_amd/csrc/recurrent_gru.hip
+++ b/hypernet-image-captioning_amd/csrc/recurrent_gru.hip
@@ -497,7 +497,7 @@
         ctx[((size_t)b * T + t) * ldc + k] = s;
     }
 }
-__global__ void df_kernel(int P, int F, int T, const float* __restrict__ alphas, const float* __restrict__ dctx,
+__global__ void df_kernel(int P, int F, int T, const float* __restrict__ alphas, const float* __restrict__ dctx, int ldd,
                           const float* __restrict__ dmean, const float* __restrict__ dmean2, float* __restrict__ df) {
     const int b = blockIdx.x, p = blockIdx.y;
     const float invP = 1.0f / (float)P;
@@ -507,11 +507,11 @@
         for (; t + 8 <= T; t += 8) {
             float a[8], v[8];
 #pragma unroll
-            for (int u = 0; u < 8; ++u) { a[u] = alphas[((size_t)b * T + t + u) * P + p]; v[u] = dctx[((size_t)b * T + t + u) * F + k]; }
+            for (int u = 0; u < 8; ++u) { a[u] = alphas[((size_t)b * T + t + u) * P + p]; v[u] = dctx[((size_t)b * T + t + u) * ldd + k]; }
 #pragma unroll
             for (int u = 0; u < 8; ++u) s += a[u] * v[u];
         }
-        for (; t < T; ++t) s += alphas[((size_t)b * T + t) * P + p] * dctx[((size_t)b * T + t) * F + k];
+        for (; t < T; ++t) s += alphas[((size_t)b * T + t) * P + p] * dctx[((size_t)b * T + t) * ldd + k];
         df[((size_t)b * P + p) * F + k] = s;
     }
 }
@@ -634,9 +634,9 @@
     hipLaunchKernelGGL(ctx_kernel, dim3(B, T), dim3(F >= 192 ? 256 : 64), 0, s, P, F, T, alphas, f, ctx, ldc);
     return caphn_launch_status();
 }
-int caphn_launch_df(int B, int T, int P, int F, const float* alphas, const float* dctx, const float* dmean, float* df, hipStream_t s,
+int caphn_launch_df(int B, int T, int P, int F, const float* alphas, const float* dctx, int ldd, const float* dmean, float* df, hipStream_t s,
                     const float* dmean2) {
-    hipLaunchKernelGGL(df_kernel, dim3(B, P), dim3(F >= 192 ? 256 : 64), 0, s, P, F, T, alphas, dctx, dmean, dmean2, df);
+    hipLaunchKernelGGL(df_kernel, dim3(B, P), dim3(F >= 192 ? 256 : 64), 0, s, P, F, T, alphas, dctx, ldd, dmean, dmean2, df);
     return caphn_launch_status();
 }
 int caphn_launch_init_state(int B, int P, int F, int H, const float* f, const float* Wh, const float* bh, const float* Wc,
diff --git a/include/caphn.h b/include/caphn.h
--- a/include/caphn.h
+++ b/include/caphn.h
@@ -48,6 +48,8 @@
 int caphn_axpy_f32(size_t n, float alpha, const float* x, float* y, caphn_stream_t stream);
 int caphn_linear_wgrad_f32(int M, int N, int K, const float* dY, int ldy, const float* X, int ldx, float* dW, int ldw,
                            float* db, void* ws, caphn_stream_t stream);
+int caphn_linear_wgrad_panels_f32(int n, const int* M, int N, int K, const float* const* dY, const int* ldy, const float* X, int ldx,
+                                  float* const* dW, const int* ldw, float* const* db, int splitk, void* ws, caphn_stream_t stream);
 size_t caphn_colsum_workspace_bytes(int M, int N);
 int caphn_colsum_f32(int M, int N, const float* A, int lda, float* out, void* ws, caphn_stream_t stream);
 
```

After: 82400 images/s (median of 4 runs). About the same (+0.0%).
